# xxxupeng/stereo_toolbox

Hardware: AMD Instinct MI355X
Metric: stereo pairs/sec @ 540x960 D=192 (GwcNet_GC fwd+bwd) (higher is better)
Workload: dtype f32; 1 GPU; GwcNet_GC(maxdisp=192) train step: fwd+bwd+allreduce+Adam, 576x960 pairs (reference pad_to_2x shape), batch 1/GPU, fp32, synthetic randn inputs, deterministic filler weights; global_batch=1, parallelism=dp1, grad_sync=none (single rank: flat fp32 buffer packed, no collective), launch=eager, optimizer=torch.optim.Adam(fused=True)

## Files before the change

include/stx_hip.h:

```cpp
#ifndef STX_HIP_H
#define STX_HIP_H
#ifdef __cplusplus
extern "C" {
#endif

const char* stx_last_error(void);
const char* stx_build_info(void);
int stx_get_tuning(const char* name);
int stx_set_tuning(const char* name, int value);

int stx_cost_volume_fwd(const float* Lg, const float* Rg, int Cg, int G, const float* Lc, const float* Rc, int Cc,
                        const float* scale, float* vol, int B, int H, int W, int D, int mask_left, void* stream);
int stx_group_normalize_fwd(const float* x, float* y, int B, int C, int G, int HW, float out_scale, void* stream);
int stx_group_normalize_bwd(const float* x, const float* gy, float* gx, int B, int C, int G, int HW, float out_scale, void* stream);
int stx_cost_volume_bwd(const float* gvol, const float* Lg, const float* Rg, int Cg, int G, int Cc, float* gLg,
                        float* gRg, float* gLc, float* gRc, int B, int H, int W, int D, int mask_left, void* stream);

int stx_head_fwd(const float* cost, float* disp, float* stats, int B, int Dc, int Hc, int Wc, int D, int H, int W,
                 void* stream);
long long stx_head_bwd_workspace_floats(int B, int Dc, int H, int W);
int stx_head_bwd(const float* gdisp, const float* cost, const float* disp, const float* stats, float* gcost,
                 float* workspace, int B, int Dc, int Hc, int Wc, int D, int H, int W, void* stream);
int stx_head_fwd2(const float* cost, float* disp, float* stats, int B, int Dc, int Hc, int Wc, int D, int H, int W,
                  int align_corners, void* stream);
int stx_head_bwd2(const float* gdisp, const float* cost, const float* disp, const float* stats, float* gcost,
                  float* workspace, int B, int Dc, int Hc, int Wc, int D, int H, int W, int align_corners, void* stream);
int stx_softargmax_fwd(const float* x, float* out, int B, int D, int HW, void* stream);
int stx_argmax_fwd(const float* x, long long* out, int B, int D, int HW, void* stream);
int stx_unimodal_fwd(const float* x, float* out, int B, int D, int HW, void* stream);
int stx_dominant_modal_fwd(const float* x, float* out, int B, int D, int HW, void* stream);
int stx_modal_fwd(const float* x, float* out, float* aux, int B, int D, int HW, int kind, void* stream);
int stx_modal_bwd(const float* g, const float* out, const float* aux, float* gx, int B, int D, int HW, void* stream);
int stx_split_mode(const float* x, float* mode, unsigned char* mask, int B, int D, int HW, void* stream);
int stx_softmax_d_fwd(const float* x, float* y, int B, int D, int HW, void* stream);

long long stx_conv3d_packed_floats(int K, int N, int T);
int stx_conv3d_pack_weight(const float* w, float* wp, int A, int B, int T, int mode, void* stream);
int stx_conv3d_fwd_blocks(int Do, int Ho, int Wo);
long long stx_conv3d_fwd_stat_rows(int B, int Di, int Hi, int Wi, int Cin, int Cout, int ks, int stride);
int stx_conv3d_fwd(const float* x, const float* wp, float* out, const float* scale, const float* bias,
                   const float* residual, float* stats, int B, int Di, int Hi, int Wi, int Cin, int Cout, int ks,
                   int stride, int relu, void* stream);
int stx_deconv3d_fwd_blocks(int Di, int Hi, int Wi);
int stx_deconv3d_fwd(const float* x, const float* wp, float* out, const float* scale, const float* bias,
                     const float* residual, float* stats, int B, int Di, int Hi, int Wi, int Cin, int Cout, int Do,
                     int Ho, int Wo, int relu, void* stream);
long long stx_conv3d_wgrad_workspace_floats(int B, int Dc, int Hc, int Wc, int CF, int CC, int ks, int stride);
int stx_conv3d_wgrad(const float* fine, const float* coarse, float* dw, float* workspace, int B, int Df, int Hf, int Wf,
                     int CF, int Dc, int Hc, int Wc, int CC, int ks, int stride, void* stream);

int stx_conv3d_wgrad_bn_supported(int B, int D, int H, int W, int CF, int CC);
int stx_conv3d_wgrad_bn(const float* x, const float* gy, const float* z, const float* scale, const float* shift, const float* mean,
                        const float* invstd, const float* gamma, const float* sums, float inv_n, int act, float* dz, float* dw,
                        float* workspace, int B, int D, int H, int W, int CF, int CC, void* stream);

int stx_conv3d_axial_supported(int Cin, int Cout, int kd, int kh, int kw);
long long stx_conv3d_axial_packed_floats(int K, int N, int kd, int kh, int kw);
int stx_conv3d_axial_pack_weight(const float* w, float* wp, int A, int B, int kd, int kh, int kw, int mode, void* stream);
long long stx_conv3d_axial_fwd_stat_rows(int B, int D, int H, int W, int Cin, int Cout, int kd, int kh, int kw);
int stx_conv3d_axial_fwd(const float* x, const float* wp, float* out, const float* scale, const float* bias,
                         const float* residual, float* stats, int B, int D, int H, int W, int Cin, int Cout, int kd, int kh,
                         int kw, int act, void* stream);
long long stx_conv3d_axial_wgrad_workspace_floats(int B, int D, int H, int W, int CF, int CC, int kd, int kh, int kw);
int stx_conv3d_axial_wgrad(const float* x, const float* gz, float* dw, float* workspace, int B, int D, int H, int W, int CF,
                           int CC, int kd, int kh, int kw, void* stream);

int stx_convgru_supported(int hidden, int nx, int cx0, int cx1, int cx2, int ksize);
long long stx_convgru_packed_floats(int K, int N);
int stx_convgru_pack_weight(const float* w0, const float* w1, float* wp, int A, int Bd, int mode, void* stream);
int stx_convgru_gemm(const float* s0, int c0, int p0, const float* s1, int c1, int p1, const float* s2, int c2, int p2,
                     const float* s3, int c3, int p3, const float* wp, int N, int epi, int split, const float* bias0,
                     const float* bias1, const float* add0, int add0_pitch, const float* add1, int add1_pitch, const float* h,
                     int h_pitch, const float* z, float* out0, float* out1, float* out2, int out_pitch, int B, int H, int W,
                     void* stream);
int stx_convgru_gate_rows(long long P, int hidden);
int stx_convgru_gate_bwd(const float* g, int g_pitch, const float* z, const float* q, const float* h, int h_pitch, float* gq,
                         float* gz, float* rows, long long P, int hidden, void* stream);
int stx_convgru_reset_bwd(float* buf, int buf_pitch, const float* g, int g_pitch, const float* z, const float* r, const float* h,
                          int h_pitch, float* gr, float* rows, long long P, int hidden, void* stream);
int stx_convgru_row_sum(const float* rows, float* out, int nrows, int n, void* stream);
long long stx_convgru_wgrad_workspace_floats(int B, int H, int W, int K, int CC);
int stx_convgru_wgrad(const float* s0, int c0, int p0, const float* s1, int c1, int p1, const float* s2, int c2, int p2,
                      const float* s3, int c3, int p3, const float* g0, const float* g1, int CG, float* dw, float* workspace,
                      int B, int H, int W, void* stream);

int stx_conv2d_supported(int Cin, int Cout);
long long stx_conv2d_stat_rows(int groups);
int stx_conv2d_fwd(const float* x, const float* w, float* out, float* stats, int B, int H, int W, int Cin, int Cout, int dgrad,
                   int groups, void* stream);

int stx_conv3d_c1_fwd(const float* x, const float* w, const float* residual, float* out, int B, int D, int H, int W,
                      int Cin, void* stream);
long long stx_conv3d_c1_wgrad_workspace_floats(int Cin);
int stx_conv3d_c1_wgrad(const float* x, const float* gy, float* dw, float* workspace, int B, int D, int H, int W,
                        int Cin, void* stream);
int stx_conv3d_c1_dgrad(const float* gy, const float* w, float* gx, int B, int D, int H, int W, int Cin, void* stream);

int stx_mish_fwd(const float* x, float* y, long long n, void* stream);
int stx_mish_bwd(const float* gy, const float* x, float* gx, long long n, void* stream);
int stx_depth_to_space(const float* y, float* out, int B, int D, int H, int W, int C, int inverse, void* stream);
int stx_gate_fwd(const float* cv, const float* att, float* out, int B, int D, long long HW, int C, void* stream);
int stx_gate_bwd(const float* g, const float* cv, const float* att, float* gcv, float* gatt, int B, int D, long long HW,
                 int C, void* stream);

int stx_concat_channels(const float* in0, const float* in1, const float* in2, const float* in3, int C0, int C1, int C2, int C3,
                        float* out, long long nvox, void* stream);
int stx_split_channels(const float* in, float* out0, float* out1, float* out2, float* out3, int C0, int C1, int C2, int C3,
                       long long nvox, void* stream);
int stx_transpose(const float* in, float* out, int N, int rows, int cols, void* stream);

int stx_dwconv_hw_fwd(const float* x, const float* w, const int* dil, float* out, int B, int D, int H, int W, int C,
                      int flip, void* stream);
long long stx_dwconv_hw_wgrad_workspace_floats(int C);
int stx_dwconv_hw_wgrad(const float* x, const float* gy, const int* dil, float* dw, float* workspace, int B, int D,
                        int H, int W, int C, void* stream);
int stx_cost_volume_scale_bwd(const float* gvol, const float* Lc, const float* Rc, float* gscale, int B, int Cc, int H,
                              int W, int D, int mask_left, void* stream);
int stx_scale_channels(const float* x, const float* s, float* out, long long nvox, int C, void* stream);
int stx_ac_volume_bwd(const float* gvol, const float* Lc, const float* Rc, const float* prob, float* gL, float* gR,
                      float* gprob, int B, int Cc, int H, int W, int D, int mask_left, void* stream);

int stx_bn_reduce_blocks(void);
int stx_bn_stats_rows(long long nvox, int C);
int stx_bn_stats(const float* z, float* partials, long long nvox, int C, int groups, void* stream);
int stx_bn_finalize(const float* partials, int nrows, int C, double count, const float* gamma, const float* beta,
                    float* running_mean, float* running_var, float momentum, float eps, float* scale, float* shift,
                    float* mean, float* invstd, void* stream);
int stx_bn_finalize_groups(const float* partials, int nrows, int C, double count, const float* gamma, const float* beta,
                           float* running_mean, float* running_var, float momentum, float eps, float* out, int groups,
                           void* stream);
int stx_bn_apply(const float* z1, const float* scale1, const float* shift1, const float* z2, const float* scale2,
                 const float* shift2, float* out, long long nvox, int C, int relu, int groups, void* stream);
int stx_bn_bwd_reduce(const float* gy, const float* y, const float* z1, const float* mean1, const float* invstd1,
                      const float* z2, const float* mean2, const float* invstd2, float* partials, float* sums,
                      long long nvox, int C, int relu, void* stream);
int stx_bn_bwd_apply(const float* gy, const float* y, const float* z1, const float* mean1, const float* invstd1,
                     const float* gamma1, const float* z2, const float* mean2, const float* invstd2,
                     const float* gamma2, const float* sums, float* dz1, float* dz2, float* gout, long long nvox, int C,
                     int relu, void* stream);
int stx_bn_bwd_reduce2(const float* gy, const float* y, const float* z1, const float* mean1, const float* invstd1,
                       const float* z2, const float* mean2, const float* invstd2, const float* scale1,
                       const float* shift1, const float* scale2, const float* shift2, float* partials, float* sums,
                       long long nvox, int C, int relu, int groups, void* stream);
int stx_bn_bwd_apply2(const float* gy, const float* y, const float* z1, const float* mean1, const float* invstd1,
                      const float* gamma1, const float* z2, const float* mean2, const float* invstd2,
                      const float* gamma2, const float* scale1, const float* shift1, const float* scale2,
                      const float* shift2, const float* sums, float* dz1, float* dz2, float* gout, long long nvox,
                      int C, int relu, int groups, void* stream);

int stx_pad_normalize_u8(const unsigned char* img, float* out, int B, int H, int W, int Hp, int Wp, int top,
                         const float* mean3, const float* std3, void* stream);

int stx_sampled_volume_fwd(const float* Lg, const float* Rg, int Cg, int G, const float* Lc, const float* Rc, int Cc,
                           const float* samples, float* vol, int B, int H, int W, int S, int CTp, void* stream);
int stx_sampled_volume_bwd(const float* gvol, const float* Lg, const float* Rg, int Cg, int G, int Cc,
                           const float* samples, float* gLg, float* gRg, float* gLc, float* gRc, int B, int H, int W,
                           int S, int CTp, void* stream);

int stx_warp_fwd(const float* x, const float* disp, float* out, int B, int C, int H, int W, void* stream);
int stx_warp_bwd(const float* gout, const float* x, const float* disp, float* gx, float* gdisp, int B, int C, int H, int W,
                 void* stream);
int stx_corr_volume_fwd(const float* ref, const float* tgt, float* vol, int B, int C, int H, int W, int maxdisp, int groups,
                        void* stream);
int stx_corr_volume_bwd(const float* gvol, const float* ref, const float* tgt, float* gref, float* gtgt, int B, int C, int H,
                        int W, int maxdisp, int groups, void* stream);
int stx_disparity_variance_fwd(const float* x, const float* disp, const float* samples, float* out, int B, int D, int HW,
                               void* stream);
int stx_disparity_variance_bwd(const float* g, const float* x, const float* disp, const float* samples, float* gx, float* gdisp,
                               float* gsamples, int B, int D, int HW, void* stream);

long long stx_geo_pyramid_floats(long long rows, int len, int C, int levels);
int stx_geo_corr_fwd(const float* fmap1, const float* fmap2, float* cpyr, int B, int C, int H, int W1, int W2, int levels,
                     void* stream);
int stx_geo_corr_bwd(const float* gcpyr, const float* fmap1, const float* fmap2, float* gfmap1, float* gfmap2, int B, int C, int H,
                     int W1, int W2, int levels, void* stream);
int stx_geo_pyramid_fwd(const float* vol, float* gpyr, int B, int D, int H, int W, int C, int levels, void* stream);
int stx_geo_pyramid_bwd(const float* ggpyr, float* gvol, int B, int D, int H, int W, int C, int levels, void* stream);
int stx_geo_lookup_fwd(const float* gpyr, const float* cpyr, const float* disp, const float* coords, float* out, int B, int H,
                       int W, int D, int C, int W2, int levels, int radius, void* stream);
int stx_geo_lookup_bwd(const float* gout, const float* disp, const float* coords, float* ggpyr, float* gcpyr, int B, int H, int W,
                       int D, int C, int W2, int levels, int radius, void* stream);
int stx_context_upsample_fwd(const float* disp_low, const float* up_weights, float* out, int B, int h, int w, void* stream);
int stx_context_upsample_bwd(const float* g, const float* disp_low, const float* up_weights, float* gdisp, float* gweights, int B,
                             int h, int w, void* stream);

long long stx_corr1d_pyramid_floats(long long rows, int W2, int levels);
int stx_corr1d_pyramid_fwd(const float* fmap1, const float* fmap2, float* cpyr, int B, int C, int H, int W1, int W2, int levels,
                           float scale, void* stream);
int stx_corr1d_pyramid_bwd(const float* gcpyr, const float* fmap1, const float* fmap2, float* gfmap1, float* gfmap2, int B, int C,
                           int H, int W1, int W2, int levels, float scale, void* stream);
int stx_corr1d_lookup_fwd(const float* cpyr, const float* base, const float* disp, const float* jobs, int njobs, float* out, int B,
                          int H, int W1, int W2, int levels, void* stream);
int stx_corr1d_lookup_bwd(const float* gout, const float* base, const float* disp, const float* jobs, int njobs, float* gcpyr,
                          int B, int H, int W1, int W2, int levels, void* stream);

int stx_allpairs_estimates_fwd(const float* vol, int which, float* disp_l, float* conf_l, float* disp_r, float* conf_r, float* stats,
                               int B, int H, int W1, int W2, void* stream);
int stx_allpairs_estimates_bwd(const float* g_disp_l, const float* g_conf_l, const float* g_disp_r, const float* g_conf_r,
                               const float* vol, const float* stats, float* gvol, int B, int H, int W1, int W2, void* stream);
int stx_corr1d_volume_pyramid_fwd(const float* vol, const float* tdisp, const float* tconf, float atten, float* cpyr, int B, int H,
                                  int W1, int W2, int levels, void* stream);
int stx_corr1d_volume_pyramid_bwd(const float* gcpyr, const float* tdisp, const float* tconf, float atten, float* gvol, int B, int H,
                                  int W1, int W2, int levels, void* stream);
int stx_truncate_mask_fwd(const float* disp, const float* conf, int has_th, float conf_th, float atten, float* mask, int B, int H,
                          int W, void* stream);

int stx_generate_masks_fwd(const float* mde, void* masks, int B, int N, int H, int W, void* stream);
int stx_masked_volume_fwd(const float* vol, const float* mde_l, const float* mde_r, float* out, int B, int N, int H, int W2, int W3,
                          void* stream);
int stx_masked_volume_bwd(const float* g, const float* mde_l, const float* mde_r, float* gvol, int B, int N, int H, int W2, int W3,
                          void* stream);
int stx_softlrc_fwd(const float* disp2, const float* disp3, float lrc_th, float* out2, float* out3, int B, int H, int W,
                    void* stream);
long long stx_softlrc_bwd_workspace_floats(int B, int H, int W);
int stx_softlrc_bwd(const float* g2, const float* g3, const float* disp2, const float* disp3, float lrc_th, void* workspace,
                    float* gdisp2, float* gdisp3, int B, int H, int W, void* stream);
int stx_weighted_lsq_fwd(const float* mde, const float* disp, const float* conf, float min_quantile, float max_quantile, float* scale,
                         float* shift, void* stats, int B, long long n, void* stream);
int stx_weighted_lsq_bwd(const float* g_scale, const float* g_shift, const float* mde, const float* disp, const float* conf,
                         const void* stats, float* g_mde, float* g_disp, float* g_conf, int B, long long n, void* stream);
int stx_mirror_detector_fwd(const float* stereo_disp, const float* mono_disp, const float* stereo_conf, const float* mono_conf,
                            float conf_th, float step_gain, float* out, long long n, void* stream);
int stx_mirror_detector_bwd(const float* g_out, const float* stereo_disp, const float* mono_disp, const float* stereo_conf,
                            const float* mono_conf, float conf_th, float step_gain, float* g_stereo_disp, float* g_mono_disp,
                            float* g_stereo_conf, float* g_mono_conf, long long n, void* stream);

int stx_photo_warp_fwd(const float* right, const float* disp, float* warped, float* valid, int B, int C, int H, int W, void* stream);
int stx_photo_warp_bwd(const float* gwarped, const float* right, const float* disp, float* gdisp, int B, int C, int H, int W,
                       void* stream);
int stx_ssim_fwd(const float* x, const float* y, float* out, int B, int C, int H, int W, int window, void* stream);
long long stx_ssim_bwd_workspace_floats(int B, int C, int H, int W);
int stx_ssim_bwd(const float* g_out, const float* x, const float* y, float* gx, float* gy, float* workspace, int B, int C, int H, int W,
                 int window, void* stream);
int stx_photometric_fwd(const float* left, const float* right, const float* disp, double ssim_weight, int enable_mask, float* loss,
                        int B, int C, int H, int W, void* stream);
long long stx_photometric_bwd_workspace_floats(int B, int C, int H, int W);
int stx_photometric_bwd(const float* gloss, const float* left, const float* right, const float* disp, double ssim_weight,
                        int enable_mask, float* gdisp, float* workspace, int B, int C, int H, int W, void* stream);
int stx_auto_mask_fwd(const float* left, const float* right, const float* disp, int denorm, unsigned char* mask, int B, int C, int H,
                      int W, void* stream);
long long stx_smoothness_workspace_floats(int B, int H, int W);
int stx_smoothness_fwd(const float* disp, const float* img, float* out, float* stats, float* workspace, int B, int C, int H, int W,
                       void* stream);
int stx_smoothness_bwd(const float* gout, const float* disp, const float* img, const float* stats, float* gdisp, int B, int C, int H,
                       int W, void* stream);

int stx_sttr_head_fwd(const float* attn, const float* phi, int mode, int iters, float log_one, float log_bin, float log_2w,
                      const unsigned char* occ_mask, const float* target, float* disp, float* occ, float* norm, int* arg,
                      float* gt_response, float* bin_left, float* bin_right, double* us, double* vs, int N, int H, int W, void* stream);
int stx_sttr_head_bwd(const float* g_disp, const float* g_occ, const float* g_gt, const float* g_bin_left, const float* g_bin_right,
                      const float* attn, const float* phi, int mode, int iters, float log_one, float log_bin, float log_2w,
                      const float* target, const float* disp, const float* norm, const int* arg, const double* us, const double* vs,
                      float* g_attn, double* phi_partials, float* g_phi, int N, int H, int W, void* stream);
int stx_sttr_transport_fwd(const float* attn, const float* phi, int mode, int iters, float log_one, float log_bin, float log_2w,
                           float* P, double* us, double* vs, int N, int H, int W, void* stream);
int stx_sttr_transport_bwd(const float* G, const float* attn, const float* phi, int mode, int iters, float log_one, float log_bin,
                           float log_2w, const double* us, const double* vs, float* g_attn, double* phi_partials, float* g_phi, int N,
                           int H, int W, void* stream);

int stx_sttr_attn_fwd(const float* q, const float* k, const float* v, const float* Qr, const float* Kr, int causal, float* o,
                      float* raw, float* avg, float* stats, int W, int B, int E, int head_dim, void* stream);
int stx_sttr_attn_bwd(const float* dO, const float* dRaw, const float* q, const float* k, const float* v, const float* Qr,
                      const float* Kr, const float* o, const float* stats, int causal, float* dq, float* dk, float* dv, float* dQr,
                      float* dKr, float* scratch, long long scratch_floats, int nb, int W, int B, int E, int head_dim, void* stream);

int stx_disp_attention_supported(int L, int C, int nhead, int F, int layers);
int stx_disp_attention_fwd(const float* x, const float* pe, const float* const* params, float* y, float* saved, const long long* seed,
                           float p, float eps, int N, int L, int C, int nhead, int F, int layers, int hw, long long sb, long long sp,
                           long long st, void* stream);
long long stx_disp_attention_bwd_workspace_floats(int N, int L, int C, int F);
int stx_disp_attention_bwd(const float* gy, const float* saved, const float* const* params, float* const* gparams, float* gx, float* gbuf,
                           float* workspace, long long workspace_floats, const long long* seed, float p, float eps, int N, int L, int C,
                           int nhead, int F, int layers, int hw, long long sb, long long sp, long long st, void* stream);
int stx_disp_attention_masks(const long long* seed, float p, unsigned char* masks, int N, int L, int C, int F, int layers, void* stream);

int stx_convex_upsample_fwd(const float* flow, const float* mask, float* out, int N, int D, int H, int W, int mask_channels, int f,
                            float scale, void* stream);
long long stx_convex_upsample_bwd_workspace_floats(int N, int D, int H, int W);
int stx_convex_upsample_bwd(const float* g, const float* flow, const float* mask, float* gflow, float* gmask, float* workspace, int N,
                            int D, int H, int W, int mask_channels, int f, float scale, void* stream);
int stx_softmax_context_upsample_fwd(const float* disp_low, const float* logits, float* out, int B, int h, int w, float scale,
                                     void* stream);
int stx_softmax_context_upsample_bwd(const float* g, const float* disp_low, const float* logits, float* gdisp, float* glogits,
                                     float* workspace, int B, int h, int w, float scale, void* stream);
int stx_sequence_loss_max_predictions(void);
long long stx_sequence_loss_workspace_floats(long long n);
int stx_sequence_loss_fwd(const float* const* preds, const double* weights, int K, const float* gt, float maxdisp, float* loss,
                          int* count, float* workspace, long long n, void* stream);
int stx_sequence_loss_bwd(const float* gloss, const float* const* preds, const double* weights, int K, const float* gt, float maxdisp,
                          const int* count, float* const* gpreds, long long n, void* stream);

int stx_monster_flaw_fwd(const float* left, const float* right, const float* disp_a, const float* disp_b, int zeros_pad, float* out_a,
                         float* out_b, float* valid, int B, int C, int H, int W, void* stream);
int stx_monster_flaw_bwd(const float* g_a, const float* g_b, const float* right, const float* disp_a, const float* disp_b, int zeros_pad,
                         float* g_left, float* g_right, float* g_disp_a, float* g_disp_b, int B, int C, int H, int W, void* stream);
int stx_monster_scale_shift(const float* mono, const float* gt, const unsigned char* mask, long long k, float* out, void* stats, int B,
                            long long n, void* stream);
int stx_monster_apply_scale_shift(const float* x, const float* scale_shift, int with_shift, float* out, int B, long long n,
                                  void* stream);

#ifdef __cplusplus
}
#endif
#endif
```

stereo_toolbox_amd/_capi.py:

```python
import ctypes
import os
import threading

import torch

_P = ctypes.c_void_p
_I = ctypes.c_int
_F = ctypes.c_float
_L = ctypes.c_longlong

SIGNATURES = {
    "stx_get_tuning": [ctypes.c_char_p],
    "stx_set_tuning": [ctypes.c_char_p, _I],
    "stx_cost_volume_fwd": [_P, _P, _I, _I, _P, _P, _I, _P, _P, _I, _I, _I, _I, _I, _P],
    "stx_cost_volume_bwd": [_P, _P, _P, _I, _I, _I, _P, _P, _P, _P, _I, _I, _I, _I, _I, _P],
    "stx_group_normalize_fwd": [_P, _P, _I, _I, _I, _I, _F, _P],
    "stx_group_normalize_bwd": [_P, _P, _P, _I, _I, _I, _I, _F, _P],
    "stx_head_fwd": [_P, _P, _P, _I, _I, _I, _I, _I, _I, _I, _P],
    "stx_head_bwd_workspace_floats": [_I, _I, _I, _I],
    "stx_head_bwd": [_P, _P, _P, _P, _P, _P, _I, _I, _I, _I, _I, _I, _I, _P],
    "stx_head_fwd2": [_P, _P, _P, _I, _I, _I, _I, _I, _I, _I, _I, _P],
    "stx_head_bwd2": [_P, _P, _P, _P, _P, _P, _I, _I, _I, _I, _I, _I, _I, _I, _P],
    "stx_softargmax_fwd": [_P, _P, _I, _I, _I, _P],
    "stx_argmax_fwd": [_P, _P, _I, _I, _I, _P],
    "stx_softmax_d_fwd": [_P, _P, _I, _I, _I, _P],
    "stx_unimodal_fwd": [_P, _P, _I, _I, _I, _P],
    "stx_dominant_modal_fwd": [_P, _P, _I, _I, _I, _P],
    "stx_modal_fwd": [_P, _P, _P, _I, _I, _I, _I, _P],
    "stx_modal_bwd": [_P, _P, _P, _P, _I, _I, _I, _P],
    "stx_split_mode": [_P, _P, _P, _I, _I, _I, _P],
    "stx_conv3d_packed_floats": [_I, _I, _I],
    "stx_conv3d_pack_weight": [_P, _P, _I, _I, _I, _I, _P],
    "stx_conv3d_fwd_blocks": [_I, _I, _I],
    "stx_conv3d_fwd_stat_rows": [_I, _I, _I, _I, _I, _I, _I, _I],
    "stx_deconv3d_fwd_blocks": [_I, _I, _I],
    "stx_conv3d_fwd": [_P, _P, _P, _P, _P, _P, _P, _I, _I, _I, _I, _I, _I, _I, _I, _I, _P],
    "stx_deconv3d_fwd": [_P, _P, _P, _P, _P, _P, _P, _I, _I, _I, _I, _I, _I, _I, _I, _I, _I, _P],
    "stx_conv3d_wgrad_workspace_floats": [_I, _I, _I, _I, _I, _I, _I, _I],
    "stx_conv3d_wgrad": [_P, _P, _P, _P, _I, _I, _I, _I, _I, _I, _I, _I, _I, _I, _I, _P],
    "stx_conv3d_wgrad_bn_supported": [_I, _I, _I, _I, _I, _I],
    "stx_conv3d_wgrad_bn": [_P] * 9 + [_F, _I, _P, _P, _P, _I, _I, _I, _I, _I, _I, _P],
    "stx_conv3d_axial_supported": [_I, _I, _I, _I, _I],
    "stx_conv3d_axial_packed_floats": [_I, _I, _I, _I, _I],
    "stx_conv3d_axial_pack_weight": [_P, _P, _I, _I, _I, _I, _I, _I, _P],
    "stx_conv3d_axial_fwd_stat_rows": [_I] * 9,
    "stx_conv3d_axial_fwd": [_P] * 7 + [_I] * 10 + [_P],
    "stx_conv3d_axial_wgrad_workspace_floats": [_I] * 9,
    "stx_conv3d_axial_wgrad": [_P, _P, _P, _P] + [_I] * 9 + [_P],
    "stx_convgru_supported": [_I] * 6,
    "stx_convgru_packed_floats": [_I, _I],
    "stx_convgru_pack_weight": [_P, _P, _P, _I, _I, _I, _P],
    "stx_convgru_gemm": [_P, _I, _I] * 4 + [_P, _I, _I, _I, _P, _P, _P, _I, _P, _I, _P, _I, _P, _P, _P, _P, _I, _I, _I, _I, _P],
    "stx_convgru_gate_rows": [_L, _I],
    "stx_convgru_gate_bwd": [_P, _I, _P, _P, _P, _I, _P, _P, _P, _L, _I, _P],
    "stx_convgru_reset_bwd": [_P, _I, _P, _I, _P, _P, _P, _I, _P, _P, _L, _I, _P],
    "stx_convgru_row_sum": [_P, _P, _I, _I, _P],
    "stx_convgru_wgrad_workspace_floats": [_I] * 5,
    "stx_convgru_wgrad": [_P, _I, _I] * 4 + [_P, _P, _I, _P, _P, _I, _I, _I, _P],
    "stx_conv2d_supported": [_I, _I],
    "stx_conv2d_stat_rows": [_I],
    "stx_conv2d_fwd": [_P, _P, _P, _P, _I, _I, _I, _I, _I, _I, _I, _P],
    "stx_conv3d_c1_fwd": [_P, _P, _P, _P, _I, _I, _I, _I, _I, _P],
    "stx_conv3d_c1_wgrad_workspace_floats": [_I],
    "stx_conv3d_c1_wgrad": [_P, _P, _P, _P, _I, _I, _I, _I, _I, _P],
    "stx_conv3d_c1_dgrad": [_P, _P, _P, _I, _I, _I, _I, _I, _P],
    "stx_mish_fwd": [_P, _P, _L, _P],
    "stx_mish_bwd": [_P, _P, _P, _L, _P],
    "stx_depth_to_space": [_P, _P, _I, _I, _I, _I, _I, _I, _P],
    "stx_gate_fwd": [_P, _P, _P, _I, _I, _L, _I, _P],
    "stx_gate_bwd": [_P, _P, _P, _P, _P, _I, _I, _L, _I, _P],
    "stx_concat_channels": [_P, _P, _P, _P, _I, _I, _I, _I, _P, _L, _P],
    "stx_split_channels": [_P, _P, _P, _P, _P, _I, _I, _I, _I, _L, _P],
    "stx_transpose": [_P, _P, _I, _I, _I, _P],
    "stx_dwconv_hw_fwd": [_P, _P, _P, _P, _I, _I, _I, _I, _I, _I, _P],
    "stx_dwconv_hw_wgrad_workspace_floats": [_I],
    "stx_dwconv_hw_wgrad": [_P, _P, _P, _P, _P, _I, _I, _I, _I, _I, _P],
    "stx_cost_volume_scale_bwd": [_P, _P, _P, _P, _I, _I, _I, _I, _I, _I, _P],
    "stx_scale_channels": [_P, _P, _P, _L, _I, _P],
    "stx_ac_volume_bwd": [_P, _P, _P, _P, _P, _P, _P, _I, _I, _I, _I, _I, _I, _P],
    "stx_pad_normalize_u8": [_P, _P, _I, _I, _I, _I, _I, _I, _P, _P, _P],
    "stx_warp_fwd": [_P, _P, _P, _I, _I, _I, _I, _P],
    "stx_warp_bwd": [_P, _P, _P, _P, _P, _I, _I, _I, _I, _P],
    "stx_corr_volume_fwd": [_P, _P, _P, _I, _I, _I, _I, _I, _I, _P],
    "stx_corr_volume_bwd": [_P, _P, _P, _P, _P, _I, _I, _I, _I, _I, _I, _P],
    "stx_disparity_variance_fwd": [_P, _P, _P, _P, _I, _I, _I, _P],
    "stx_disparity_variance_bwd": [_P, _P, _P, _P, _P, _P, _P, _I, _I, _I, _P],
    "stx_sampled_volume_fwd": [_P, _P, _I, _I, _P, _P, _I, _P, _P, _I, _I, _I, _I, _I, _P],
    "stx_sampled_volume_bwd": [_P, _P, _P, _I, _I, _I, _P, _P, _P, _P, _P, _I, _I, _I, _I, _I, _P],
    "stx_geo_pyramid_floats": [_L, _I, _I, _I],
    "stx_geo_corr_fwd": [_P, _P, _P, _I, _I, _I, _I, _I, _I, _P],
    "stx_geo_corr_bwd": [_P, _P, _P, _P, _P, _I, _I, _I, _I, _I, _I, _P],
    "stx_geo_pyramid_fwd": [_P, _P, _I, _I, _I, _I, _I, _I, _P],
    "stx_geo_pyramid_bwd": [_P, _P, _I, _I, _I, _I, _I, _I, _P],
    "stx_geo_lookup_fwd": [_P, _P, _P, _P, _P, _I, _I, _I, _I, _I, _I, _I, _I, _P],
    "stx_geo_lookup_bwd": [_P, _P, _P, _P, _P, _I, _I, _I, _I, _I, _I, _I, _I, _P],
    "stx_context_upsample_fwd": [_P, _P, _P, _I, _I, _I, _P],
    "stx_context_upsample_bwd": [_P, _P, _P, _P, _P, _I, _I, _I, _P],
    "stx_corr1d_pyramid_floats": [_L, _I, _I],
    "stx_corr1d_pyramid_fwd": [_P, _P, _P, _I, _I, _I, _I, _I, _I, _F, _P],
    "stx_corr1d_pyramid_bwd": [_P, _P, _P, _P, _P, _I, _I, _I, _I, _I, _I, _F, _P],
    "stx_corr1d_lookup_fwd": [_P, _P, _P, _P, _I, _P, _I, _I, _I, _I, _I, _P],
    "stx_corr1d_lookup_bwd": [_P, _P, _P, _P, _I, _P, _I, _I, _I, _I, _I, _P],
    "stx_allpairs_estimates_fwd": [_P, _I, _P, _P, _P, _P, _P, _I, _I, _I, _I, _P],
    "stx_allpairs_estimates_bwd": [_P, _P, _P, _P, _P, _P, _P, _I, _I, _I, _I, _P],
    "stx_corr1d_volume_pyramid_fwd": [_P, _P, _P, _F, _P, _I, _I, _I, _I, _I, _P],
    "stx_corr1d_volume_pyramid_bwd": [_P, _P, _P, _F, _P, _I, _I, _I, _I, _I, _P],
    "stx_truncate_mask_fwd": [_P, _P, _I, _F, _F, _P, _I, _I, _I, _P],
    "stx_generate_masks_fwd": [_P, _P, _I, _I, _I, _I, _P],
    "stx_masked_volume_fwd": [_P, _P, _P, _P, _I, _I, _I, _I, _I, _P],
    "stx_masked_volume_bwd": [_P, _P, _P, _P, _I, _I, _I, _I, _I, _P],
    "stx_softlrc_fwd": [_P, _P, _F, _P, _P, _I, _I, _I, _P],
    "stx_softlrc_bwd_workspace_floats": [_I, _I, _I],
    "stx_softlrc_bwd": [_P, _P, _P, _P, _F, _P, _P, _P, _I, _I, _I, _P],
    "stx_weighted_lsq_fwd": [_P, _P, _P, _F, _F, _P, _P, _P, _I, _L, _P],
    "stx_weighted_lsq_bwd": [_P, _P, _P, _P, _P, _P, _P, _P, _P, _I, _L, _P],
    "stx_mirror_detector_fwd": [_P, _P, _P, _P, _F, _F, _P, _L, _P],
    "stx_mirror_detector_bwd": [_P, _P, _P, _P, _P, _F, _F, _P, _P, _P, _P, _L, _P],
    "stx_photo_warp_fwd": [_P, _P, _P, _P, _I, _I, _I, _I, _P],
    "stx_photo_warp_bwd": [_P, _P, _P, _P, _I, _I, _I, _I, _P],
    "stx_ssim_fwd": [_P, _P, _P, _I, _I, _I, _I, _I, _P],
    "stx_ssim_bwd_workspace_floats": [_I, _I, _I, _I],
    "stx_ssim_bwd": [_P, _P, _P, _P, _P, _P, _I, _I, _I, _I, _I, _P],
    "stx_photometric_fwd": [_P, _P, _P, ctypes.c_double, _I, _P, _I, _I, _I, _I, _P],
    "stx_photometric_bwd_workspace_floats": [_I, _I, _I, _I],
    "stx_photometric_bwd": [_P, _P, _P, _P, ctypes.c_double, _I, _P, _P, _I, _I, _I, _I, _P],
    "stx_auto_mask_fwd": [_P, _P, _P, _I, _P, _I, _I, _I, _I, _P],
    "stx_smoothness_workspace_floats": [_I, _I, _I],
    "stx_smoothness_fwd": [_P, _P, _P, _P, _P, _I, _I, _I, _I, _P],
    "stx_smoothness_bwd": [_P, _P, _P, _P, _P, _I, _I, _I, _I, _P],
    "stx_sttr_head_fwd": [_P, _P, _I, _I, _F, _F, _F] + [_P] * 11 + [_I, _I, _I, _P],
    "stx_sttr_head_bwd": [_P] * 7 + [_I, _I, _F, _F, _F] + [_P] * 9 + [_I, _I, _I, _P],
    "stx_sttr_transport_fwd": [_P, _P, _I, _I, _F, _F, _F, _P, _P, _P, _I, _I, _I, _P],
    "stx_sttr_transport_bwd": [_P, _P, _P, _I, _I, _F, _F, _F, _P, _P, _P, _P, _P, _I, _I, _I, _P],
    "stx_sttr_attn_fwd": [_P] * 5 + [_I] + [_P] * 4 + [_I, _I, _I, _I, _P],
    "stx_sttr_attn_bwd": [_P] * 9 + [_I] + [_P] * 6 + [_L, _I, _I, _I, _I, _I, _P],
    "stx_disp_attention_supported": [_I] * 5,
    "stx_disp_attention_fwd": [_P] * 6 + [_F, _F] + [_I] * 7 + [_L, _L, _L, _P],
    "stx_disp_attention_bwd_workspace_floats": [_I] * 4,
    "stx_disp_attention_bwd": [_P] * 7 + [_L, _P, _F, _F] + [_I] * 7 + [_L, _L, _L, _P],
    "stx_disp_attention_masks": [_P, _F, _P, _I, _I, _I, _I, _I, _P],
    "stx_convex_upsample_fwd": [_P, _P, _P, _I, _I, _I, _I, _I, _I, _F, _P],
    "stx_convex_upsample_bwd_workspace_floats": [_I, _I, _I, _I],
    "stx_convex_upsample_bwd": [_P, _P, _P, _P, _P, _P, _I, _I, _I, _I, _I, _I, _F, _P],
    "stx_softmax_context_upsample_fwd": [_P, _P, _P, _I, _I, _I, _F, _P],
    "stx_softmax_context_upsample_bwd": [_P, _P, _P, _P, _P, _P, _I, _I, _I, _F, _P],
    "stx_sequence_loss_max_predictions": [],
    "stx_sequence_loss_workspace_floats": [_L],
    "stx_sequence_loss_fwd": [_P, _P, _I, _P, _F, _P, _P, _P, _L, _P],
    "stx_sequence_loss_bwd": [_P, _P, _P, _I, _P, _F, _P, _P, _L, _P],
    "stx_monster_flaw_fwd": [_P, _P, _P, _P, _I, _P, _P, _P, _I, _I, _I, _I, _P],
    "stx_monster_flaw_bwd": [_P, _P, _P, _P, _P, _I, _P, _P, _P, _P, _I, _I, _I, _I, _P],
    "stx_monster_scale_shift": [_P, _P, _P, _L, _P, _P, _I, _L, _P],
    "stx_monster_apply_scale_shift": [_P, _P, _I, _P, _I, _L, _P],
    "stx_bn_reduce_blocks": [],
    "stx_bn_stats_rows": [_L, _I],
    "stx_bn_stats": [_P, _P, _L, _I, _I, _P],
    "stx_bn_finalize": [_P, _I, _I, ctypes.c_double, _P, _P, _P, _P, _F, _F, _P, _P, _P, _P, _P],
    "stx_bn_finalize_groups": [_P, _I, _I, ctypes.c_double, _P, _P, _P, _P, _F, _F, _P, _I, _P],
    "stx_bn_apply": [_P, _P, _P, _P, _P, _P, _P, _L, _I, _I, _I, _P],
    "stx_bn_bwd_reduce": [_P, _P, _P, _P, _P, _P, _P, _P, _P, _P, _L, _I, _I, _P],
    "stx_bn_bwd_apply": [_P, _P, _P, _P, _P, _P, _P, _P, _P, _P, _P, _P, _P, _P, _L, _I, _I, _P],
    "stx_bn_bwd_reduce2": [_P] * 14 + [_L, _I, _I, _I, _P],
    "stx_bn_bwd_apply2": [_P] * 18 + [_L, _I, _I, _I, _P],
}
_RET_CHARP = ("stx_last_error", "stx_build_info")


class StxError(RuntimeError):
    pass


class StxLib:

    def __init__(self, path):
        if not os.path.exists(path):
            raise StxError(
                f"HIP library not found: {path}. Build it with `python -m stereo_toolbox_amd.build` "
                "(hipcc, gfx950). There is no CPU fallback for the cost-volume hot path.")
        self.path = path
        self._dll = ctypes.CDLL(path)
        for name in _RET_CHARP:
            fn = getattr(self._dll, name)
            fn.restype = ctypes.c_char_p
            fn.argtypes = []
        self._fns = {}
        for name, argtypes in SIGNATURES.items():
            fn = getattr(self._dll, name, None)
            if fn is None:
                continue
            fn.restype = ctypes.c_longlong if name.endswith(("_floats", "_stat_rows")) else _I
            fn.argtypes = argtypes
            self._fns[name] = fn

    def has(self, name):
        return name in self._fns

    def build_info(self):
        return self._dll.stx_build_info().decode()

    def get_tuning(self, name):
        return self._fns["stx_get_tuning"](name.encode())

    def set_tuning(self, name, value):
        old = self.get_tuning(name)
        if old < 0 or self._fns["stx_set_tuning"](name.encode(), int(value)) != 0:
            raise StxError(f"unknown tuning switch {name}")
        return old

    def raw(self, name):
        return self._fns[name]

    def call(self, name, *args):
        fn = self._fns.get(name)
        if fn is None:
            raise StxError(f"{self.path} does not export {name}")
        rc = fn(*args)
        if rc != 0:
            raise StxError(f"{name} failed ({rc}): {self._dll.stx_last_error().decode()}")


_LIB = None
_LOCK = threading.Lock()
LIB_PATH = os.environ.get("STX_HIP_LIB") or os.path.join(os.path.dirname(os.path.abspath(__file__)), "lib", "libstx_hip.so")


def get_lib():
    global _LIB
    if _LIB is None:
        with _LOCK:
            if _LIB is None:
                _LIB = StxLib(LIB_PATH)
    return _LIB
```

stereo_toolbox_amd/aggregation.py:

```python
import os
import threading

import torch
import torch.nn as nn

from . import ops


def _is_transposed(conv):
    return isinstance(conv, nn.ConvTranspose3d)


def _conv_cfg(conv):
    ks = conv.kernel_size[0]
    stride = conv.stride[0]
    if _is_transposed(conv):
        k3 = ks == 3 and stride == 2 and conv.padding[0] == 1 and conv.output_padding[0] == 1
        k4 = ks == 4 and stride == 2 and conv.padding[0] == 1 and conv.output_padding[0] == 0
        if not (k3 or k4) or len(set(conv.kernel_size)) != 1 or len(set(conv.stride)) != 1:
            raise ops.StxError("only ConvTranspose3d(k=3, s=2, p=1, op=1) and ConvTranspose3d(k=4, s=2, p=1) are on the hot path")
    else:
        if not ((ks == 3 and conv.padding[0] == 1 and stride in (1, 2)) or (ks == 1 and conv.padding[0] == 0 and stride == 1)):
            raise ops.StxError(f"unsupported Conv3d k={ks} s={stride} p={conv.padding}")
    if conv.bias is not None or conv.groups != 1:
        raise ops.StxError("hot-path convolutions are bias-free and dense")
    return ks, stride


def _fold(bn):
    key = (bn.weight._version, bn.bias._version, bn.running_mean._version, bn.running_var._version,
           bn.weight.data_ptr(), bn.bias.data_ptr(), bn.running_mean.data_ptr(), bn.running_var.data_ptr())
    hit = bn.__dict__.get("_stx_fold") if ops._CACHE_ENABLED else None
    if hit is not None and hit[0] == key:
        return hit[1], hit[2]
    with torch.no_grad():
        scale = (bn.weight * torch.rsqrt(bn.running_var + bn.eps)).contiguous()
        bias = (bn.bias - bn.running_mean * scale).contiguous()
    if ops._CACHE_ENABLED:
        bn.__dict__["_stx_fold"] = (key, scale, bias)
    return scale, bias


def _needs_grad(*tensors_and_modules):
    if not torch.is_grad_enabled():
        return False
    for t in tensors_and_modules:
        if t is None:
            continue
        if isinstance(t, torch.Tensor):
            if t.requires_grad:
                return True
        else:
            if any(p.requires_grad for p in t.parameters()):
                return True
    return False


def _infer_conv(x, conv, scale, bias, residual, relu):
    ks, stride = _conv_cfg(conv)
    if _is_transposed(conv) and ks == 4:
        if residual is not None:
            raise ops.StxError("ConvTranspose3d(k4) with a fused residual is not wired (no model uses it)")
        return ops.deconv4_forward(x, conv.weight.detach(), scale, bias, int(relu), owner=conv.weight)
    if _is_transposed(conv):
        wp = ops.pack_weight(conv.weight.detach(), 2, owner=conv.weight)
        return ops.deconv3d_forward(x, wp, conv.weight.shape[1], scale=scale, bias=bias, residual=residual, relu=relu)[0]
    if ops._is_c1(conv.weight, ks, stride, False) and scale is None and bias is None and not relu:
        return ops.conv3d_c1_forward(x, conv.weight.detach().contiguous(), residual)
    if x.shape[-1] != conv.weight.shape[1]:
        if x.shape[-1] != (conv.weight.shape[1] + 7) // 8 * 8:
            raise ops.StxError(f"conv: input has {x.shape[-1]} channels, weight expects {conv.weight.shape[1]}")
        wpad = ops.pad_weight_channels(conv.weight.detach(), x.shape[-1])
        return ops.conv3d_forward(x, ops.pack_weight(wpad, 0), conv.weight.shape[0], ks, stride, scale, bias, residual, relu)[0]
    if x.shape[-1] % 8 != 0:
        xp, wpad = ops.pad_input_channels(x, conv.weight.detach())
        return ops.conv3d_forward(xp, ops.pack_weight(wpad, 0), conv.weight.shape[0], ks, stride, scale, bias, residual, relu)[0]
    wp = ops.pack_weight(conv.weight.detach(), 0, owner=conv.weight)
    return ops.conv3d_forward(x, wp, conv.weight.shape[0], ks, stride, scale, bias, residual, relu)[0]


class deferred_bn_counters:
    _tls = threading.local()

    @staticmethod
    def _state():
        st = deferred_bn_counters._tls
        if not hasattr(st, "active"):
            st.active, st.pending = 0, []
        return st

    def __enter__(self):
        self._state().active += 1
        ops.bn_defer_reset_if_stale()
        return self

    def __exit__(self, *exc):
        st = self._state()
        st.active -= 1
        if st.active == 0 and st.pending:
            pend, st.pending = st.pending, []
            by_dev = {}
            for t in pend:
                d = by_dev.setdefault(t.device, {})
                ent = d.setdefault(id(t), [t, 0])
                ent[1] += 1
            for d in by_dev.values():
                torch._foreach_add_([e[0] for e in d.values()], [e[1] for e in d.values()])
        return False


def _bn_state(bn, partials, count, steps=1):
    training = bn.training
    sync = None
    if training and isinstance(bn, nn.SyncBatchNorm):
        import torch.distributed as dist
        if dist.is_available() and dist.is_initialized() and dist.get_world_size(bn.process_group) > 1:
            sync = (bn.process_group, dist.get_world_size(bn.process_group))
    if training:
        bn.__dict__.pop("_stx_fold", None)
    if training and bn.track_running_stats and bn.num_batches_tracked is not None:
        st = deferred_bn_counters._state()
        if st.active and bn.momentum is not None:
            st.pending.extend([bn.num_batches_tracked] * steps)
        else:
            bn.num_batches_tracked.add_(steps)
    if bn.momentum is not None:
        momentum = bn.momentum
    elif training and bn.track_running_stats and bn.num_batches_tracked is not None:
        momentum = 1.0 / float(bn.num_batches_tracked.item())
    else:
        momentum = 0.0
    return {"training": training, "partials": partials, "count": count, "running_mean": bn.running_mean,
            "running_var": bn.running_var, "momentum": momentum, "eps": bn.eps, "sync": sync}


def _raw_conv(x, conv, want):
    ks, stride = _conv_cfg(conv)
    if _is_transposed(conv) and ks == 4:
        return ops.deconv4_raw(x, conv.weight, want)
    return ops.ConvRawFn.apply(x, conv.weight, ks, stride, _is_transposed(conv), want)


@ops.fp32_region
def shared_input_convs(x, blocks):
    cfgs, ws = [], []
    for seq in blocks:
        conv, bn = seq[0], seq[1]
        if _is_transposed(conv) or not bn.training or conv.weight.shape[1] != x.shape[-1] or conv.weight.shape[1] % 8 \
                or conv.weight.shape[0] % 8:
            return None
        ks, stride = _conv_cfg(conv)
        cfgs.append((ks, stride, True))
        ws.append(conv.weight)
    if not _needs_grad(x, *[m for seq in blocks for m in (seq[0], seq[1])]):
        return None
    outs = ops.SharedInputConvsFn.apply(x, tuple(cfgs), *ws)
    return [(outs[2 * k], outs[2 * k + 1]) for k in range(len(blocks))]


@ops.fp32_region
def conv_block(x, conv, bn=None, relu=False, second=None, residual=None, mish=False, leaky=False, raw=None, second_raw=None):
    if (mish and relu) or (leaky and (relu or mish)):
        raise ops.StxError("conv_block: relu, mish and leaky are mutually exclusive")
    if second is not None and residual is not None:
        raise ops.StxError("conv_block: `second` and `residual` are mutually exclusive")
    mods = [conv, bn] + ([second[1], second[2]] if second is not None else [])
    grad = (raw is not None or second_raw is not None
            or _needs_grad(x, residual, *(m for m in mods if m is not None), *([second[0]] if second else [])))
    train_bn = (bn is not None and bn.training) or (second is not None and second[2].training)
    if mish and (grad or train_bn) and (bn is None or residual is not None):
        return ops.mish(conv_block(x, conv, bn, relu=False, second=second, residual=residual))
    if mish:
        relu = 2
    if leaky:
        relu = 3

    if not grad and not train_bn:
        if second is not None:
            s2, b2 = _fold(second[2])
            residual = _infer_conv(second[0], second[1], s2, b2, None, False)
        if bn is not None:
            s1, b1 = _fold(bn)
        else:
            s1 = b1 = None
        return _infer_conv(x, conv, s1, b1, residual, relu)

    want = bn is not None and bn.training
    z1, part1 = raw if raw is not None else _raw_conv(x, conv, want)
    if bn is None:
        y = z1
        if residual is not None:
            y = y + residual
        if relu == 3:
            return torch.nn.functional.leaky_relu(y, 0.01)
        return torch.relu(y) if relu else y
    count1 = z1.numel() // z1.shape[-1]
    st1 = _bn_state(bn, part1 if want else None, count1)
    if second is not None:
        x2, conv2, bn2 = second
        want2 = bn2.training
        z2, part2 = second_raw if second_raw is not None else _raw_conv(x2, conv2, want2)
        st2 = _bn_state(bn2, part2 if want2 else None, z2.numel() // z2.shape[-1])
        return ops.BnActFn.apply(z1, bn.weight, bn.bias, z2, bn2.weight, bn2.bias, None, relu, st1, st2)
    defer = (residual is None and want and relu in (0, 1, False, True) and not _is_transposed(conv) and _conv_cfg(conv) == (3, 1)
             and conv.weight.shape[0] % 32 == 0 and conv.weight.shape[1] % 32 == 0 and not st1.get("sync")
             and os.environ.get("STX_BN_BWD_IN_WGRAD", "1") != "0")
    if defer:
        ops.bn_defer_reset_if_stale()
    return ops.BnActFn.apply(z1, bn.weight, bn.bias, None, None, None, residual, relu, st1, None, 1, defer)


def _axial_cfg(conv):
    if not isinstance(conv, nn.Conv3d) or _is_transposed(conv):
        raise ops.StxError("axial_conv_block: expected an nn.Conv3d")
    kernel = ops._axial_kernel(conv.weight, "axial_conv_block")
    if tuple(conv.stride) != (1, 1, 1) or tuple(conv.dilation) != (1, 1, 1) or conv.groups != 1:
        raise ops.StxError(f"axial_conv_block: stride {tuple(conv.stride)} dilation {tuple(conv.dilation)} groups {conv.groups}: "
                           "only dense stride-1 convolutions are served")
    if tuple(conv.padding) != tuple(k // 2 for k in kernel) or conv.padding_mode != "zeros":
        raise ops.StxError(f"axial_conv_block: padding {conv.padding} ({conv.padding_mode}) is not the 'same' zero padding of kernel {kernel}")
    return kernel


def _fold_with_bias(conv, bn):
    scale, shift = _fold(bn)
    if conv.bias is None:
        return scale, shift
    hit = conv.__dict__.get("_stx_fold") if ops._CACHE_ENABLED else None
    key = (conv.bias._version, conv.bias.data_ptr())
    if hit is not None and hit[0] == key and hit[1] is shift:
        return scale, hit[2]
    with torch.no_grad():
        shift_b = torch.addcmul(shift, conv.bias, scale).contiguous()
    if ops._CACHE_ENABLED:
        conv.__dict__["_stx_fold"] = (key, shift, shift_b)
    return scale, shift_b


@ops.fp32_region
def axial_conv_block(x, conv, bn):
    kernel = _axial_cfg(conv)
    if not isinstance(bn, nn.modules.batchnorm._BatchNorm):
        raise ops.StxError(f"axial_conv_block: {type(bn).__name__} is not a BatchNorm")
    if not _needs_grad(x, conv, bn) and not bn.training:
        scale, shift = _fold_with_bias(conv, bn)
        xk, wk, _ = ops._axial_prepare(x, conv.weight.detach(), "axial_conv_block")
        wp = ops.pack_weight_axial(wk, 0, owner=conv.weight if wk.shape == conv.weight.shape else None)
        return ops.conv3d_axial_forward(xk, wp, conv.weight.shape[0], kernel, scale, shift, None, 1)[0]
    want = bn.training
    z, part = ops.AxialConvRawFn.apply(x, conv.weight, want)
    if conv.bias is not None:
        z = ops.ZeroGradBiasFn.apply(z, conv.bias) if want else z + conv.bias
    st = _bn_state(bn, part if want else None, z.numel() // z.shape[-1])
    y = ops.BnActFn.apply(z, bn.weight, bn.bias, None, None, None, None, 1, st, None)
    if want and conv.bias is not None and bn.track_running_stats and bn.running_mean is not None:
        with torch.no_grad():
            bn.running_mean.add_(conv.bias.detach(), alpha=float(st["momentum"]))
    return y


@ops.fp32_region
def convbn_block(x, seq, relu=False, second=None, residual=None, mish=False, raw=None, second_raw=None):
    sec = None
    if second is not None:
        sec = (second[0], second[1][0], second[1][1])
    return conv_block(x, seq[0], seq[1], relu=relu, second=sec, residual=residual, mish=mish, raw=raw, second_raw=second_raw)
```

stereo_toolbox_amd/csrc/conv_c1.hip:

```cpp
#include "stx_common.h"
#include <stdlib.h>

namespace {

constexpr int C1_THREADS = 256;
constexpr int C1_TD = 2, C1_TH = 4, C1_TW = 32;
constexpr int C1_ED = C1_TD + 2, C1_EH = C1_TH + 2, C1_EW = C1_TW + 2;
constexpr int C1_CK = 16, C1_VS = C1_CK + 4;

struct C1Args {
    const float* x;
    const float* w;
    const float* gy;
    const float* res;
    float* out;
    int B, D, H, W, Cin;
    int nDt, nHt, nWt, ntiles;
};

__device__ __forceinline__ void c1_stage(const C1Args& a, float* tile, int b, int d0, int h0, int w0, int c0, int tid) {
    for (int idx = tid; idx < C1_ED * C1_EH * C1_EW * (C1_CK / 4); idx += C1_THREADS) {
        const int v = idx / (C1_CK / 4), f = idx - v * (C1_CK / 4);
        const int wx = v % C1_EW, hy = (v / C1_EW) % C1_EH, dz = v / (C1_EW * C1_EH);
        const int gd = d0 - 1 + dz, gh = h0 - 1 + hy, gw = w0 - 1 + wx;
        float4 val = make_float4(0.f, 0.f, 0.f, 0.f);
        if (gd >= 0 && gd < a.D && gh >= 0 && gh < a.H && gw >= 0 && gw < a.W)
            val = stx_ld4(a.x + ((((size_t)b * a.D + gd) * a.H + gh) * a.W + gw) * a.Cin + c0 + 4 * f);
        stx_st4(tile + v * C1_VS + 4 * f, val);
    }
}

__global__ __launch_bounds__(C1_THREADS) void conv_c1_fwd_kernel(C1Args a) {
    STX_DYN_SMEM(smem);
    float* tile = reinterpret_cast<float*>(smem);
    const int tid = threadIdx.x;
    int r = blockIdx.x;
    const int wt = r % a.nWt; r /= a.nWt;
    const int ht = r % a.nHt; r /= a.nHt;
    const int dt = r % a.nDt;
    const int b = r / a.nDt;
    const int d0 = dt * C1_TD, h0 = ht * C1_TH, w0 = wt * C1_TW;
    const int lw = tid % C1_TW, lh = (tid / C1_TW) % C1_TH, ld = tid / (C1_TW * C1_TH);
    const int base = ((ld * C1_EH + lh) * C1_EW + lw) * C1_VS;
    float acc = 0.f;
    for (int c0 = 0; c0 < a.Cin; c0 += C1_CK) {
        __syncthreads();
        c1_stage(a, tile, b, d0, h0, w0, c0, tid);
        __syncthreads();
        for (int tap = 0; tap < 27; ++tap) {
            const int kd = tap / 9, kh = (tap / 3) % 3, kw = tap % 3;
            const float* p = tile + base + ((kd * C1_EH + kh) * C1_EW + kw) * C1_VS;
#pragma unroll
            for (int f = 0; f < C1_CK / 4; ++f) {
                const float4 v = stx_ld4(p + 4 * f);
                const float* wp = a.w + (size_t)(c0 + 4 * f) * 27 + tap;
                acc = fmaf(v.x, wp[0], acc);
                acc = fmaf(v.y, wp[27], acc);
                acc = fmaf(v.z, wp[54], acc);
                acc = fmaf(v.w, wp[81], acc);
            }
        }
    }
    const int od = d0 + ld, oh = h0 + lh, ow = w0 + lw;
    if (od < a.D && oh < a.H && ow < a.W) {
        const size_t o = (((size_t)b * a.D + od) * a.H + oh) * a.W + ow;
        a.out[o] = a.res ? acc + a.res[o] : acc;
    }
}

__global__ __launch_bounds__(C1_THREADS) void conv_c1_wgrad_kernel(C1Args a) {
    STX_DYN_SMEM(smem);
    float* tile = reinterpret_cast<float*>(smem);
    float* gys = tile + C1_ED * C1_EH * C1_EW * C1_VS;
    const int tid = threadIdx.x;
    const int cl = tid & 15, tg = tid >> 4;
    const int nchunk = a.Cin / C1_CK;
    float acc[4][2];
#pragma unroll
    for (int i = 0; i < 4; ++i) { acc[i][0] = 0.f; acc[i][1] = 0.f; }
    const int tapA = tg, tapB = tg + 16;
    const int offA = (((tapA / 9) * C1_EH + (tapA / 3) % 3) * C1_EW + tapA % 3) * C1_VS + cl;
    const int tB = tapB < 27 ? tapB : 0;
    const int offB = (((tB / 9) * C1_EH + (tB / 3) % 3) * C1_EW + tB % 3) * C1_VS + cl;

    for (int t = blockIdx.x; t < a.ntiles; t += gridDim.x) {
        int r = t;
        const int wt = r % a.nWt; r /= a.nWt;
        const int ht = r % a.nHt; r /= a.nHt;
        const int dt = r % a.nDt;
        const int b = r / a.nDt;
        const int d0 = dt * C1_TD, h0 = ht * C1_TH, w0 = wt * C1_TW;
#pragma unroll
        for (int ck = 0; ck < 4; ++ck) {
            if (ck < nchunk) {
                __syncthreads();
                c1_stage(a, tile, b, d0, h0, w0, ck * C1_CK, tid);
                if (ck == 0) {
                    const int lw = tid % C1_TW, lh = (tid / C1_TW) % C1_TH, ld = tid / (C1_TW * C1_TH);
                    const int od = d0 + ld, oh = h0 + lh, ow = w0 + lw;
                    gys[tid] = (od < a.D && oh < a.H && ow < a.W)
                                   ? a.gy[(((size_t)b * a.D + od) * a.H + oh) * a.W + ow] : 0.f;
                }
                __syncthreads();
                float sA = 0.f, sB = 0.f;
                for (int v = 0; v < C1_TD * C1_TH * C1_TW; ++v) {
                    const int lw = v % C1_TW, lh = (v / C1_TW) % C1_TH, ld = v / (C1_TW * C1_TH);
                    const int vb = ((ld * C1_EH + lh) * C1_EW + lw) * C1_VS;
                    const float g = gys[v];
                    sA = fmaf(tile[vb + offA], g, sA);
                    sB = fmaf(tile[vb + offB], g, sB);
                }
                acc[ck][0] += sA;
                acc[ck][1] += sB;
            }
        }
    }
    float* dst = a.out + (size_t)blockIdx.x * a.Cin * 27;
#pragma unroll
    for (int ck = 0; ck < 4; ++ck) {
        if (ck < nchunk) {
            dst[(ck * C1_CK + cl) * 27 + tapA] = acc[ck][0];
            if (tapB < 27) dst[(ck * C1_CK + cl) * 27 + tapB] = acc[ck][1];
        }
    }
}

__global__ __launch_bounds__(C1_THREADS) void c1_colsum_kernel(const float* __restrict__ partials, int nrows, int M,
                                                               float* __restrict__ sums) {
    __shared__ double red[C1_THREADS];
    const int m = blockIdx.x, tid = threadIdx.x;
    double s = 0.0;
    for (int r = tid; r < nrows; r += C1_THREADS) s += (double)partials[(size_t)r * M + m];
    red[tid] = s;
    __syncthreads();
    for (int k = C1_THREADS / 2; k > 0; k >>= 1) {
        if (tid < k) red[tid] += red[tid + k];
        __syncthreads();
    }
    if (tid == 0) sums[m] = (float)red[0];
}

constexpr size_t C1_TILE_BYTES = (size_t)C1_ED * C1_EH * C1_EW * C1_VS * 4;
constexpr int C1_WGRAD_BLOCKS = 512;


constexpr int C1D_TH = 4, C1D_TW = 32;
constexpr int C1D_EH = C1D_TH + 2, C1D_EW = C1D_TW + 2;

__global__ __launch_bounds__(C1_THREADS) void conv_c1_dgrad_kernel(const float* __restrict__ gy,
                                                                   const float* __restrict__ w, float* __restrict__ gx,
                                                                   int B, int D, int H, int W, int Cin, int nHt, int nWt) {
    __shared__ float gys[3 * C1D_EH * C1D_EW];
    __shared__ float ws[27 * 64];
    const int tid = threadIdx.x;
    int r = blockIdx.x;
    const int wt = r % nWt; r /= nWt;
    const int ht = r % nHt; r /= nHt;
    const int d = r % D;
    const int b = r / D;
    const int h0 = ht * C1D_TH, w0 = wt * C1D_TW;
    for (int idx = tid; idx < 3 * C1D_EH * C1D_EW; idx += C1_THREADS) {
        const int wx = idx % C1D_EW, hy = (idx / C1D_EW) % C1D_EH, dz = idx / (C1D_EW * C1D_EH);
        const int gd = d - 1 + dz, gh = h0 - 1 + hy, gw = w0 - 1 + wx;
        gys[idx] = (gd >= 0 && gd < D && gh >= 0 && gh < H && gw >= 0 && gw < W)
                       ? gy[(((size_t)b * D + gd) * H + gh) * W + gw] : 0.f;
    }
    for (int idx = tid; idx < 27 * Cin; idx += C1_THREADS) {
        const int c = idx % Cin, tap = idx / Cin;
        ws[tap * Cin + c] = w[(size_t)c * 27 + tap];
    }
    __syncthreads();
    const int CQ = Cin >> 2;
    for (int item = tid; item < CQ * (C1D_TH * C1D_TW / 4); item += C1_THREADS) {
        const int q = item % CQ, grp = item / CQ;
        const int lw = (grp % (C1D_TW / 4)) * 4, lh = grp / (C1D_TW / 4);
        float4 acc[4];
#pragma unroll
        for (int j = 0; j < 4; ++j) acc[j] = make_float4(0.f, 0.f, 0.f, 0.f);
#pragma unroll
        for (int kd = 0; kd < 3; ++kd)
#pragma unroll
            for (int kh = 0; kh < 3; ++kh) {
                const float* gp = gys + (((2 - kd) * C1D_EH) + (lh + 2 - kh)) * C1D_EW + lw;
                float g6[6];
#pragma unroll
                for (int j = 0; j < 6; ++j) g6[j] = gp[j];
#pragma unroll
                for (int kw = 0; kw < 3; ++kw) {
                    const float4 wv = stx_ld4(ws + ((kd * 3 + kh) * 3 + kw) * Cin + 4 * q);
#pragma unroll
                    for (int j = 0; j < 4; ++j) {
                        const float g = g6[j + 2 - kw];
                        acc[j].x = fmaf(g, wv.x, acc[j].x);
                        acc[j].y = fmaf(g, wv.y, acc[j].y);
                        acc[j].z = fmaf(g, wv.z, acc[j].z);
                        acc[j].w = fmaf(g, wv.w, acc[j].w);
                    }
                }
            }
        const int oh = h0 + lh;
        if (oh < H) {
            float* o = gx + ((((size_t)b * D + d) * H + oh) * W + w0 + lw) * Cin + 4 * q;
#pragma unroll
            for (int j = 0; j < 4; ++j)
                if (w0 + lw + j < W) stx_st4(o + (size_t)j * Cin, acc[j]);
        }
    }
}


__global__ __launch_bounds__(C1_THREADS) void conv_c1_dgrad_mfma_kernel(const float* __restrict__ gy,
                                                                        const float* __restrict__ w, float* __restrict__ gx,
                                                                        int B, int D, int H, int W, int nHt, int nWt, int ntiles) {
    __shared__ float gys[3 * C1D_EH * C1D_EW];
    const int tid = threadIdx.x, lane = tid & 63, wave = tid >> 6;
    const int i = lane & 31, half = lane >> 5;
    float wreg[14];
    int aoff[14];
#pragma unroll
    for (int j = 0; j < 14; ++j) {
        const int tap = 2 * j + half;
        const int tp = tap < 27 ? tap : 26;
        const int kd = tp / 9, kh = (tp / 3) % 3, kw = tp % 3;
        wreg[j] = tap < 27 ? w[(size_t)i * 27 + tap] : 0.f;
        aoff[j] = ((2 - kd) * C1D_EH + (wave + 2 - kh)) * C1D_EW + i + 2 - kw;
    }
    const unsigned plane_bytes = (unsigned)H * (unsigned)W * 128u;
    for (int tile = blockIdx.x; tile < ntiles; tile += gridDim.x) {
        int r_ = tile;
        const int wt = r_ % nWt; r_ /= nWt;
        const int ht = r_ % nHt; r_ /= nHt;
        const int d = r_ % D;
        const int b = r_ / D;
        const int h0 = ht * C1D_TH, w0 = wt * C1D_TW;
        __syncthreads();
        for (int idx = tid; idx < 3 * C1D_EH * C1D_EW; idx += C1_THREADS) {
            const int wx = idx % C1D_EW, hy = (idx / C1D_EW) % C1D_EH, dz = idx / (C1D_EW * C1D_EH);
            const int gd = d - 1 + dz, gh = h0 - 1 + hy, gw = w0 - 1 + wx;
            gys[idx] = (gd >= 0 && gd < D && gh >= 0 && gh < H && gw >= 0 && gw < W)
                           ? gy[(((size_t)b * D + gd) * H + gh) * W + gw] : 0.f;
        }
        __syncthreads();
        f32x16 acc;
#pragma unroll
        for (int r = 0; r < 16; ++r) acc[r] = 0.f;
        float av[14];
#pragma unroll
        for (int j = 0; j < 14; ++j) av[j] = gys[aoff[j]];
#pragma unroll
        for (int j = 0; j < 14; ++j) acc = __builtin_amdgcn_mfma_f32_32x32x2f32(av[j], wreg[j], acc, 0, 0, 0);
        const int oh = h0 + wave;
        const stx_bufrsrc ors = stx_make_rsrc(gx + ((size_t)b * D + d) * H * W * 32, plane_bytes);
        const unsigned vbase = (unsigned)((((oh < H ? oh : 0) * W + w0 + 4 * half) * 32 + i) * 4);
#pragma unroll
        for (int r = 0; r < 16; ++r) {
            const int m = (r & 3) + 8 * (r >> 2);
            const bool ok = oh < H && w0 + 4 * half + m < W;
            stx_buf_st1(ors, ok ? vbase : STX_BUF_OOB, (unsigned)(m * 128), acc[r]);
        }
    }
}


constexpr int C1M_TD = 2, C1M_TH = 8, C1M_TW = 32;
constexpr int C1M_ED = C1M_TD + 2, C1M_EH = C1M_TH + 2, C1M_EW = C1M_TW + 2;
constexpr int C1M_BLOCKS = 1024;

__global__ __launch_bounds__(C1_THREADS) void conv_c1_wgrad_mfma_kernel(const float* __restrict__ x,
                                                                        const float* __restrict__ gy,
                                                                        float* __restrict__ slab, int B, int D, int H,
                                                                        int W, int Cin, int nDt, int nHt, int nWt,
                                                                        int ntiles) {
    __shared__ float gys[C1M_ED * C1M_EH * C1M_EW];
    __shared__ float red[4][1024];
    const int tid = threadIdx.x, lane = tid & 63, wave = tid >> 6;
    const int i = lane & 31, half = lane >> 5;
    const int cb = blockIdx.y;
    const int kd = i / 9, kh = (i / 3) % 3, kw = i % 3;
    const int toff = (i < 27) ? ((2 - kd) * C1M_EH + (2 - kh)) * C1M_EW + (2 - kw) + half : half;
    f32x16 acc;
#pragma unroll
    for (int r = 0; r < 16; ++r) acc[r] = 0.f;
    for (int t = blockIdx.x; t < ntiles; t += gridDim.x) {
        int r = t;
        const int wt = r % nWt; r /= nWt;
        const int ht = r % nHt; r /= nHt;
        const int dt = r % nDt;
        const int b = r / nDt;
        const int d0 = dt * C1M_TD, h0 = ht * C1M_TH, w0 = wt * C1M_TW;
        __syncthreads();
        for (int idx = tid; idx < C1M_ED * C1M_EH * C1M_EW; idx += C1_THREADS) {
            const int wx = idx % C1M_EW, hy = (idx / C1M_EW) % C1M_EH, dz = idx / (C1M_EW * C1M_EH);
            const int gd = d0 - 1 + dz, gh = h0 - 1 + hy, gw = w0 - 1 + wx;
            gys[idx] = (gd >= 0 && gd < D && gh >= 0 && gh < H && gw >= 0 && gw < W)
                           ? gy[(((size_t)b * D + gd) * H + gh) * W + gw] : 0.f;
        }
        __syncthreads();
#pragma unroll 1
        for (int k = 0; k < 4; ++k) {
            const int row = wave * 4 + k;
            const int ld = row / C1M_TH, lh = row % C1M_TH;
            const int gd = d0 + ld, gh = h0 + lh;
            const bool rowok = gd < D && gh < H;
            const float* xr = x + ((((size_t)b * D + gd) * H + gh) * W + w0 + half) * Cin + cb * 32 + i;
            float av[16];
#pragma unroll
            for (int p = 0; p < 16; ++p)
                av[p] = (rowok && w0 + 2 * p + half < W) ? xr[(size_t)(2 * p) * Cin] : 0.f;
            const float* gp = gys + (ld * C1M_EH + lh) * C1M_EW + toff;
#pragma unroll
            for (int p = 0; p < 16; ++p) {
                float bv = gp[2 * p];
                bv = (i < 27) ? bv : 0.f;
                acc = __builtin_amdgcn_mfma_f32_32x32x2f32(av[p], bv, acc, 0, 0, 0);
            }
        }
    }
#pragma unroll
    for (int r = 0; r < 16; ++r) red[wave][((r & 3) + 8 * (r >> 2) + 4 * half) * 32 + i] = acc[r];
    __syncthreads();
    float* dst = slab + ((size_t)cb * gridDim.x + blockIdx.x) * 1024;
    for (int idx = tid; idx < 1024; idx += C1_THREADS)
        dst[idx] = (red[0][idx] + red[1][idx]) + (red[2][idx] + red[3][idx]);
}

__global__ __launch_bounds__(C1_THREADS) void c1m_reduce_kernel(const float* __restrict__ slab, int nrows,
                                                                float* __restrict__ dw) {
    __shared__ double red[C1_THREADS];
    const int m = blockIdx.x, tid = threadIdx.x;
    const int tap = m % 27, cfull = m / 27, cb = cfull >> 5, c = cfull & 31;
    const float* p = slab + (size_t)cb * nrows * 1024 + c * 32 + tap;
    double s = 0.0;
    for (int r = tid; r < nrows; r += C1_THREADS) s += (double)p[(size_t)r * 1024];
    red[tid] = s;
    __syncthreads();
    for (int k = C1_THREADS / 2; k > 0; k >>= 1) {
        if (tid < k) red[tid] += red[tid + k];
        __syncthreads();
    }
    if (tid == 0) dw[m] = (float)red[0];
}


constexpr int C1F_TH = 8, C1F_TW = 32;
constexpr int C1F_EH = C1F_TH + 2, C1F_EW = C1F_TW + 2, C1F_NV = C1F_EH * C1F_EW;
constexpr int C1F_MT = (C1F_NV + 31) / 32;
constexpr int C1F_WGS = 512;

__global__ __launch_bounds__(C1_THREADS) void conv_c1_fwd_mfma_kernel(const float* __restrict__ x,
                                                                      const float* __restrict__ w,
                                                                      const float* __restrict__ res,
                                                                      float* __restrict__ out, int B, int D, int H, int W,
                                                                      int nHt, int nWt, int ncols) {
    STX_DYN_SMEM(smem);
    float* Ps = reinterpret_cast<float*>(smem);
    const int tid = threadIdx.x, lane = tid & 63, wave = __builtin_amdgcn_readfirstlane(tid >> 6);
    const int i = lane & 31, half = lane >> 5;
    float wreg[16];
#pragma unroll
    for (int s_ = 0; s_ < 16; ++s_) wreg[s_] = (i < 27) ? w[(size_t)(16 * half + s_) * 27 + i] : 0.f;
    const int lh = tid / C1F_TW, lw = tid % C1F_TW;

    constexpr int MTW = (C1F_MT + 3) / 4;
    const long long units = (long long)ncols * D;
    int u = __builtin_amdgcn_readfirstlane((int)(units * blockIdx.x / gridDim.x));
    const int u_end = __builtin_amdgcn_readfirstlane((int)(units * (blockIdx.x + 1) / gridDim.x));
    const unsigned plane_bytes = (unsigned)H * (unsigned)W * 32u * 4u;
    while (u < u_end) {
        const int col = u / D;
        const int d_lo = u - col * D;
        const int left = u_end - u;
        const int d_hi = (D - d_lo < left) ? D : d_lo + left;
        u += d_hi - d_lo;
        const int wt = col % nWt, ht = (col / nWt) % nHt, b = col / (nWt * nHt);
        const int h0 = ht * C1F_TH, w0 = wt * C1F_TW;
        const int oh = h0 + lh, ow = w0 + lw;
        const bool ook = oh < H && ow < W;
        unsigned voff[MTW];
#pragma unroll
        for (int t = 0; t < MTW; ++t) {
            const int hv = (wave + 4 * t) * 32 + i;
            const int hy = hv / C1F_EW, wx = hv - hy * C1F_EW;
            const int gh = h0 - 1 + hy, gw = w0 - 1 + wx;
            const bool ok = wave + 4 * t < C1F_MT && hv < C1F_NV && gh >= 0 && gh < H && gw >= 0 && gw < W;
            voff[t] = ok ? (unsigned)(((gh * W + gw) * 32 + 16 * half) * 4) : STX_BUF_OOB;
        }
        float4 nxt[MTW][4];
        auto load_plane = [&](int p) {
            const bool in = p >= 0 && p < D && p <= d_hi;
            const stx_bufrsrc rs = stx_make_rsrc(x + ((size_t)b * D + (in ? p : 0)) * H * W * 32, in ? plane_bytes : 0u);
#pragma unroll
            for (int t = 0; t < MTW; ++t)
#pragma unroll
                for (int q = 0; q < 4; ++q) nxt[t][q] = stx_buf_ld4(rs, voff[t], 16u * q);
        };
        float accA = 0.f, accB = 0.f;
        load_plane(d_lo - 1);
        __syncthreads();
        for (int p = d_lo - 1; p <= d_hi; ++p) {
            float* Pb = Ps + ((p + 2) & 1) * (C1F_NV * 27);
            const bool pin = p >= 0 && p < D;
            float4 cur[MTW][4];
#pragma unroll
            for (int t = 0; t < MTW; ++t)
#pragma unroll
                for (int q = 0; q < 4; ++q) cur[t][q] = nxt[t][q];
            load_plane(p + 1);
            if (pin) {
#pragma unroll
                for (int t = 0; t < MTW; ++t) {
                    const int m = wave + 4 * t;
                    if (m < C1F_MT) {
                        f32x16 acc;
#pragma unroll
                        for (int r = 0; r < 16; ++r) acc[r] = 0.f;
#pragma unroll
                        for (int q = 0; q < 4; ++q) {
                            acc = __builtin_amdgcn_mfma_f32_32x32x2f32(cur[t][q].x, wreg[4 * q + 0], acc, 0, 0, 0);
                            acc = __builtin_amdgcn_mfma_f32_32x32x2f32(cur[t][q].y, wreg[4 * q + 1], acc, 0, 0, 0);
                            acc = __builtin_amdgcn_mfma_f32_32x32x2f32(cur[t][q].z, wreg[4 * q + 2], acc, 0, 0, 0);
                            acc = __builtin_amdgcn_mfma_f32_32x32x2f32(cur[t][q].w, wreg[4 * q + 3], acc, 0, 0, 0);
                        }
                        if (i < 27) {
#pragma unroll
                            for (int r = 0; r < 16; ++r) {
                                const int v = m * 32 + (r & 3) + 8 * (r >> 2) + 4 * half;
                                if (v < C1F_NV) Pb[v * 27 + i] = acc[r];
                            }
                        }
                    }
                }
            }
            __syncthreads();
            float s0 = 0.f, s1 = 0.f, s2 = 0.f;
            if (pin) {
#pragma unroll
                for (int kh = 0; kh < 3; ++kh)
#pragma unroll
                    for (int kw = 0; kw < 3; ++kw) {
                        const float* pp = Pb + ((lh + kh) * C1F_EW + lw + kw) * 27 + kh * 3 + kw;
                        s0 += pp[0];
                        s1 += pp[9];
                        s2 += pp[18];
                    }
            }
            const float done = accA + s2;
            const int od = p - 1;
            if (od >= d_lo && od < d_hi && ook) {
                const size_t o = (((size_t)b * D + od) * H + oh) * W + ow;
                out[o] = res ? done + res[o] : done;
            }
            accA = accB + s1;
            accB = s0;
        }
    }
}

}

extern "C" int stx_conv3d_c1_fwd(const float* x, const float* w, const float* residual, float* out, int B, int D,
                                 int H, int W, int Cin, void* stream) {
    stx_begin();
    STX_REQUIRE(x && w && out && B > 0 && D > 0 && H > 0 && W > 0, "conv3d_c1_fwd: bad shape");
    STX_REQUIRE(Cin % C1_CK == 0, "conv3d_c1_fwd: Cin=%d must be a multiple of %d", Cin, C1_CK);
    if (Cin == 32 && (long long)H * W * 128 < (1ll << 31)) {
        const int nHt = stx_cdiv(H, C1F_TH), nWt = stx_cdiv(W, C1F_TW);
        const long long ncols = (long long)B * nHt * nWt, units = ncols * D;
        STX_REQUIRE(units < (1ll << 31), "conv3d_c1_fwd: volume too large");
        long long g = C1F_WGS;
        if (g > units / 4) g = units / 4 > 0 ? units / 4 : 1;
        const size_t lds = (size_t)2 * C1F_NV * 27 * 4;
        if (int rc = stx_lds_require((const void*)conv_c1_fwd_mfma_kernel, lds, "conv3d_c1_fwd(mfma)")) return rc;
        hipLaunchKernelGGL(conv_c1_fwd_mfma_kernel, dim3((unsigned)g), dim3(C1_THREADS), lds, (hipStream_t)stream, x, w,
                           residual, out, B, D, H, W, nHt, nWt, (int)ncols);
        return stx_check_launch("conv3d_c1_fwd(mfma)");
    }
    C1Args a;
    a.x = x; a.w = w; a.gy = nullptr; a.res = residual; a.out = out;
    a.B = B; a.D = D; a.H = H; a.W = W; a.Cin = Cin;
    a.nDt = stx_cdiv(D, C1_TD); a.nHt = stx_cdiv(H, C1_TH); a.nWt = stx_cdiv(W, C1_TW);
    a.ntiles = B * a.nDt * a.nHt * a.nWt;
    if (int rc = stx_lds_require((const void*)conv_c1_fwd_kernel, C1_TILE_BYTES, "conv3d_c1_fwd")) return rc;
    hipLaunchKernelGGL(conv_c1_fwd_kernel, dim3(a.ntiles), dim3(C1_THREADS), C1_TILE_BYTES, (hipStream_t)stream, a);
    return stx_check_launch("conv3d_c1_fwd");
}

extern "C" long long stx_conv3d_c1_wgrad_workspace_floats(int Cin) {
    const long long valu = (long long)C1_WGRAD_BLOCKS * Cin * 27;
    const long long mfma = (long long)C1M_BLOCKS * 1024 * ((Cin + 31) / 32);
    return valu > mfma ? valu : mfma;
}

extern "C" int stx_conv3d_c1_wgrad(const float* x, const float* gy, float* dw, float* workspace, int B, int D, int H,
                                   int W, int Cin, void* stream) {
    stx_begin();
    STX_REQUIRE(x && gy && dw && workspace && B > 0, "conv3d_c1_wgrad: null operand");
    STX_REQUIRE(Cin % C1_CK == 0 && Cin <= 4 * C1_CK, "conv3d_c1_wgrad: Cin=%d must be 16..64 in steps of 16", Cin);
    if (Cin % 32 == 0) {
        const int nDt = stx_cdiv(D, C1M_TD), nHt = stx_cdiv(H, C1M_TH), nWt = stx_cdiv(W, C1M_TW);
        const long long nt = (long long)B * nDt * nHt * nWt;
        STX_REQUIRE(nt < (1ll << 31), "conv3d_c1_wgrad: volume too large");
        const int nblk = nt < C1M_BLOCKS ? (int)nt : C1M_BLOCKS;
        hipStream_t st = (hipStream_t)stream;
        hipLaunchKernelGGL(conv_c1_wgrad_mfma_kernel, dim3(nblk, Cin / 32), dim3(C1_THREADS), 0, st, x, gy, workspace, B,
                           D, H, W, Cin, nDt, nHt, nWt, (int)nt);
        int rc = stx_check_launch("conv3d_c1_wgrad(mfma)");
        if (rc) return rc;
        hipLaunchKernelGGL(c1m_reduce_kernel, dim3(Cin * 27), dim3(C1_THREADS), 0, st, workspace, nblk, dw);
        return stx_check_launch("conv3d_c1_wgrad(reduce)");
    }
    C1Args a;
    a.x = x; a.w = nullptr; a.gy = gy; a.res = nullptr; a.out = workspace;
    a.B = B; a.D = D; a.H = H; a.W = W; a.Cin = Cin;
    a.nDt = stx_cdiv(D, C1_TD); a.nHt = stx_cdiv(H, C1_TH); a.nWt = stx_cdiv(W, C1_TW);
    a.ntiles = B * a.nDt * a.nHt * a.nWt;
    const int nblk = a.ntiles < C1_WGRAD_BLOCKS ? a.ntiles : C1_WGRAD_BLOCKS;
    const size_t lds = C1_TILE_BYTES + 256 * 4;
    hipStream_t st = (hipStream_t)stream;
    if (int rc = stx_lds_require((const void*)conv_c1_wgrad_kernel, lds, "conv3d_c1_wgrad")) return rc;
    hipLaunchKernelGGL(conv_c1_wgrad_kernel, dim3(nblk), dim3(C1_THREADS), lds, st, a);
    if (int rc = stx_check_launch("conv3d_c1_wgrad")) return rc;
    hipLaunchKernelGGL(c1_colsum_kernel, dim3(Cin * 27), dim3(C1_THREADS), 0, st, workspace, nblk, Cin * 27, dw);
    return stx_check_launch("conv3d_c1_colsum");
}

extern "C" int stx_conv3d_c1_dgrad(const float* gy, const float* w, float* gx, int B, int D, int H, int W, int Cin,
                                   void* stream) {
    stx_begin();
    STX_REQUIRE(gy && w && gx && B > 0 && D > 0 && H > 0 && W > 0, "conv3d_c1_dgrad: bad shape");
    STX_REQUIRE(Cin % 4 == 0 && Cin <= 64, "conv3d_c1_dgrad: Cin=%d must be a multiple of 4, <= 64", Cin);
    const int nHt = stx_cdiv(H, C1D_TH), nWt = stx_cdiv(W, C1D_TW);
    const long long nt = (long long)B * D * nHt * nWt;
    if (Cin == 32 && (long long)H * W * 128 < (1ll << 31) && nt < (1ll << 31)) {
        const long long g = nt < 256 * 8 ? nt : 256 * 8;
        hipLaunchKernelGGL(conv_c1_dgrad_mfma_kernel, dim3((unsigned)g), dim3(C1_THREADS), 0, (hipStream_t)stream, gy, w, gx, B, D,
                           H, W, nHt, nWt, (int)nt);
        return stx_check_launch("conv3d_c1_dgrad(mfma)");
    }
    hipLaunchKernelGGL(conv_c1_dgrad_kernel, dim3((unsigned)((size_t)B * D * nHt * nWt)), dim3(C1_THREADS), 0,
                       (hipStream_t)stream, gy, w, gx, B, D, H, W, Cin, nHt, nWt);
    return stx_check_launch("conv3d_c1_dgrad");
}
```

stereo_toolbox_amd/models/GwcNet/gwcnet.py:

```python
import torch
import torch.nn as nn

from ... import ops
from ...aggregation import conv_block, convbn_block, deferred_bn_counters, shared_input_convs
from ..features2d import ResTrunk, cat_features, channels_last_weights_, convbn, init_reference_style, run_head2d, run_pair
from .submodule import convbn_3d


class feature_extraction(ResTrunk):
    fused_everywhere = True

    def __init__(self, concat_feature=False, concat_feature_channel=12):
        super().__init__()
        self.concat_feature = concat_feature
        if concat_feature:
            self.lastconv = nn.Sequential(convbn(320, 128, 3, 1, 1, 1), nn.ReLU(inplace=True),
                                          nn.Conv2d(128, concat_feature_channel, 1, bias=False))

    def forward(self, x):
        gwc = cat_features(self.trunk(x))
        if not self.concat_feature:
            return {"gwc_feature": gwc}
        return {"gwc_feature": gwc, "concat_feature": run_head2d(self.lastconv, gwc)}


class hourglass(nn.Module):

    def __init__(self, c):
        super().__init__()
        self.conv1 = nn.Sequential(convbn_3d(c, c * 2, 3, 2, 1), nn.ReLU(inplace=True))
        self.conv2 = nn.Sequential(convbn_3d(c * 2, c * 2, 3, 1, 1), nn.ReLU(inplace=True))
        self.conv3 = nn.Sequential(convbn_3d(c * 2, c * 4, 3, 2, 1), nn.ReLU(inplace=True))
        self.conv4 = nn.Sequential(convbn_3d(c * 4, c * 4, 3, 1, 1), nn.ReLU(inplace=True))
        self.conv5 = nn.Sequential(nn.ConvTranspose3d(c * 4, c * 2, 3, padding=1, output_padding=1, stride=2, bias=False),
                                   nn.BatchNorm3d(c * 2))
        self.conv6 = nn.Sequential(nn.ConvTranspose3d(c * 2, c, 3, padding=1, output_padding=1, stride=2, bias=False),
                                   nn.BatchNorm3d(c))
        self.redir1 = convbn_3d(c, c, kernel_size=1, stride=1, pad=0)
        self.redir2 = convbn_3d(c * 2, c * 2, kernel_size=1, stride=1, pad=0)

    def forward(self, x, mid=None, also=None):
        rx = shared_input_convs(x, [self.conv1[0], self.redir1] + ([also] if also is not None else []))
        rx = rx or [None, None, None]
        c1 = convbn_block(x, self.conv1[0], relu=True, raw=rx[0])
        c2 = convbn_block(c1, self.conv2[0], relu=True)
        r2 = shared_input_convs(c2, [self.conv3[0], self.redir2]) or [None, None]
        c3 = convbn_block(c2, self.conv3[0], relu=True, raw=r2[0])
        c4 = convbn_block(c3, self.conv4[0], relu=True)
        if mid is not None:
            c4 = mid(c4)
        c5 = convbn_block(c4, self.conv5, relu=True, second=(c2, self.redir2), second_raw=r2[1])
        out = convbn_block(c5, self.conv6, relu=True, second=(x, self.redir1), second_raw=rx[1])
        return (out, rx[2]) if also is not None else out


def classifier(c):
    return nn.Sequential(convbn_3d(c, c, 3, 1, 1), nn.ReLU(inplace=True),
                         nn.Conv3d(c, 1, kernel_size=3, padding=1, stride=1, bias=False))


def run_classifier(seq, x, add=None, raw=None):
    h = convbn_block(x, seq[0], relu=True, raw=raw)
    cost = conv_block(h, seq[2], residual=None if add is None else add.unsqueeze(-1))
    return cost.squeeze(-1)


class GwcNet(nn.Module):
    def __init__(self, maxdisp, use_concat_volume=False):
        super().__init__()
        self.maxdisp = maxdisp
        self.use_concat_volume = use_concat_volume
        self.num_groups = 40
        if use_concat_volume:
            self.concat_channels = 12
            self.feature_extraction = feature_extraction(True, self.concat_channels)
        else:
            self.concat_channels = 0
            self.feature_extraction = feature_extraction(False)
        self.dres0 = nn.Sequential(convbn_3d(self.num_groups + self.concat_channels * 2, 32, 3, 1, 1),
                                   nn.ReLU(inplace=True), convbn_3d(32, 32, 3, 1, 1), nn.ReLU(inplace=True))
        self.dres1 = nn.Sequential(convbn_3d(32, 32, 3, 1, 1), nn.ReLU(inplace=True), convbn_3d(32, 32, 3, 1, 1))
        self.dres2 = hourglass(32)
        self.dres3 = hourglass(32)
        self.dres4 = hourglass(32)
        self.classif0 = classifier(32)
        self.classif1 = classifier(32)
        self.classif2 = classifier(32)
        self.classif3 = classifier(32)
        init_reference_style(self)
        channels_last_weights_(self.feature_extraction)

    def forward(self, left, right):
        with deferred_bn_counters():
            fl, fr = run_pair(self.feature_extraction, left, right, self.training)
            return self.aggregate(fl, fr, left.shape[2], left.shape[3])

    @ops.fp32_region
    def aggregate(self, fl, fr, H, W):
        vol = ops.cost_volume(fl["gwc_feature"], fr["gwc_feature"], fl.get("concat_feature"),
                              fr.get("concat_feature"), self.maxdisp // 4, self.num_groups, mask_left=True)
        cost0 = convbn_block(vol, self.dres0[0], relu=True)
        cost0 = convbn_block(cost0, self.dres0[2], relu=True)
        t = convbn_block(cost0, self.dres1[0], relu=True)
        cost0 = convbn_block(t, self.dres1[2], relu=False, residual=cost0)
        if self.training:
            out1, r0 = self.dres2(cost0, also=self.classif0[0])
            out2, r1 = self.dres3(out1, also=self.classif1[0])
            out3, r2 = self.dres4(out2, also=self.classif2[0])
            return [ops.regression_head(run_classifier(c, o, raw=r), self.maxdisp, H, W)
                    for c, o, r in ((self.classif0, cost0, r0), (self.classif1, out1, r1), (self.classif2, out2, r2),
                                    (self.classif3, out3, None))]
        out1 = self.dres2(cost0)
        out2 = self.dres3(out1)
        out3 = self.dres4(out2)
        return ops.regression_head(run_classifier(self.classif3, out3), self.maxdisp, H, W)


def GwcNet_G(d=192):
    return GwcNet(d, use_concat_volume=False)


def GwcNet_GC(d=192):
    return GwcNet(d, use_concat_volume=True)
```

stereo_toolbox_amd/models/PSMNet/stackhourglass.py:

```python
import torch.nn as nn

from ... import ops
from ...aggregation import conv_block, convbn_block, deferred_bn_counters
from ..features2d import channels_last_weights_, init_reference_style, run_pair
from .submodule import convbn_3d, feature_extraction


class hourglass(nn.Module):

    def __init__(self, inplanes):
        super().__init__()
        c = inplanes
        self.conv1 = nn.Sequential(convbn_3d(c, c * 2, kernel_size=3, stride=2, pad=1), nn.ReLU(inplace=True))
        self.conv2 = convbn_3d(c * 2, c * 2, kernel_size=3, stride=1, pad=1)
        self.conv3 = nn.Sequential(convbn_3d(c * 2, c * 2, kernel_size=3, stride=2, pad=1), nn.ReLU(inplace=True))
        self.conv4 = nn.Sequential(convbn_3d(c * 2, c * 2, kernel_size=3, stride=1, pad=1), nn.ReLU(inplace=True))
        self.conv5 = nn.Sequential(nn.ConvTranspose3d(c * 2, c * 2, kernel_size=3, padding=1, output_padding=1,
                                                      stride=2, bias=False), nn.BatchNorm3d(c * 2))
        self.conv6 = nn.Sequential(nn.ConvTranspose3d(c * 2, c, kernel_size=3, padding=1, output_padding=1,
                                                      stride=2, bias=False), nn.BatchNorm3d(c))

    def forward(self, x, presqu, postsqu, skip=None):
        out = convbn_block(x, self.conv1[0], relu=True)
        pre = convbn_block(out, self.conv2, relu=True, residual=postsqu)
        out = convbn_block(pre, self.conv3[0], relu=True)
        out = convbn_block(out, self.conv4[0], relu=True)
        post = convbn_block(out, self.conv5, relu=True, residual=presqu if presqu is not None else pre)
        out = convbn_block(post, self.conv6, relu=False, residual=skip)
        return out, pre, post


def _classifier():
    return nn.Sequential(convbn_3d(32, 32, 3, 1, 1), nn.ReLU(inplace=True),
                         nn.Conv3d(32, 1, kernel_size=3, padding=1, stride=1, bias=False))


def _run_classifier(seq, x, add=None):
    h = convbn_block(x, seq[0], relu=True)
    cost = conv_block(h, seq[2], residual=None if add is None else add.unsqueeze(-1))
    return cost.squeeze(-1)


class PSMNet(nn.Module):
    def __init__(self, maxdisp=192):
        super().__init__()
        self.maxdisp = maxdisp
        self.feature_extraction = feature_extraction()
        self.dres0 = nn.Sequential(convbn_3d(64, 32, 3, 1, 1), nn.ReLU(inplace=True),
                                   convbn_3d(32, 32, 3, 1, 1), nn.ReLU(inplace=True))
        self.dres1 = nn.Sequential(convbn_3d(32, 32, 3, 1, 1), nn.ReLU(inplace=True), convbn_3d(32, 32, 3, 1, 1))
        self.dres2 = hourglass(32)
        self.dres3 = hourglass(32)
        self.dres4 = hourglass(32)
        self.classif1 = _classifier()
        self.classif2 = _classifier()
        self.classif3 = _classifier()
        init_reference_style(self)
        channels_last_weights_(self.feature_extraction)

    def forward(self, left, right):
        with deferred_bn_counters():
            fl, fr = run_pair(self.feature_extraction, left, right, self.training)
            return self.aggregate(fl, fr, left.shape[2], left.shape[3])

    @ops.fp32_region
    def aggregate(self, fl, fr, H, W):
        cost = ops.cost_volume(None, None, fl, fr, self.maxdisp // 4, 0, mask_left=True)
        cost0 = convbn_block(cost, self.dres0[0], relu=True)
        cost0 = convbn_block(cost0, self.dres0[2], relu=True)
        t = convbn_block(cost0, self.dres1[0], relu=True)
        cost0 = convbn_block(t, self.dres1[2], relu=False, residual=cost0)
        out1, pre1, post1 = self.dres2(cost0, None, None, skip=cost0)
        out2, pre2, post2 = self.dres3(out1, pre1, post1, skip=cost0)
        out3, pre3, post3 = self.dres4(out2, pre1, post2, skip=cost0)
        cost1 = _run_classifier(self.classif1, out1)
        cost2 = _run_classifier(self.classif2, out2, add=cost1)
        cost3 = _run_classifier(self.classif3, out3, add=cost2)
        pred3 = ops.regression_head(cost3, self.maxdisp, H, W).unsqueeze(1)
        if self.training:
            pred1 = ops.regression_head(cost1, self.maxdisp, H, W).unsqueeze(1)
            pred2 = ops.regression_head(cost2, self.maxdisp, H, W).unsqueeze(1)
            return [pred1, pred2, pred3]
        return pred3
```

stereo_toolbox_amd/ops.py:

```python
import ctypes

import torch

from ._capi import StxError, get_lib

_P = ctypes.c_void_p


class _DevPtr(ctypes.c_void_p):
    """A device pointer that remembers the device of the tensor it came from: _call() reads the launch device off its
    own arguments, so nothing survives between launches (an exception between building the arguments and the launch
    cannot leak state into the next one)."""


def _stream(dev=None):
    return _P(torch.cuda.current_stream(dev).cuda_stream)


def _p(t):
    if t is None:
        return None
    p = _DevPtr(t.data_ptr())
    p.dev = t.device
    return p


def on_device(t):
    return t.is_cuda


def _chk(t, name, dims=None):
    if t is None:
        return
    if not t.is_cuda:
        raise StxError(f"{name}: expected a ROCm device tensor, got {t.device} -- the cost-volume hot path has "
                       "no CPU fallback (the CPU oracle lives in oracle/ and is test-only)")
    if t.dtype != torch.float32:
        raise StxError(f"{name}: expected float32, got {t.dtype}")
    if not t.is_contiguous():
        raise StxError(f"{name}: expected a dense contiguous tensor, strides {t.stride()}")
    if dims is not None and t.dim() != dims:
        raise StxError(f"{name}: expected {dims} dims, got shape {tuple(t.shape)}")


def _call(name, *args):
    dev = None
    for a in args:
        if isinstance(a, _DevPtr):
            if dev is None:
                dev = a.dev
            elif a.dev != dev:
                raise StxError(f"{name}: operands live on different devices ({dev} and {a.dev})")
    if dev is not None and dev.type == "cuda" and dev.index != torch.cuda.current_device():
        with torch.cuda.device(dev):
            get_lib().call(name, *args, _stream(dev))
    else:
        get_lib().call(name, *args, _stream(dev))


_LOW = (torch.float16, torch.bfloat16)


def _to_fp32(v):
    if isinstance(v, torch.Tensor):
        return v.float() if v.dtype in _LOW else v
    if isinstance(v, dict):
        return {k: _to_fp32(x) for k, x in v.items()}
    if isinstance(v, (list, tuple)):
        return type(v)(_to_fp32(x) for x in v)
    return v


def autocast_active():
    return torch.is_autocast_enabled("cuda") or torch.is_autocast_enabled("cpu")


def fp32_region(fn):
    import functools

    @functools.wraps(fn)
    def wrapped(*args, **kwargs):
        if not autocast_active():
            return fn(*args, **kwargs)
        with torch.autocast("cuda", enabled=False), torch.autocast("cpu", enabled=False):
            return fn(*_to_fp32(args), **_to_fp32(kwargs))
    return wrapped


def to_ncdhw(x):
    return x.permute(0, 4, 1, 2, 3)


def to_ndhwc(x):
    return x.permute(0, 2, 3, 4, 1).contiguous()


class _Workspace:

    def __init__(self):
        self.bufs = {}

    def get(self, tag, nfloats, device):
        sid = torch.cuda.current_stream(device).cuda_stream if device.type == "cuda" else 0
        key = (device.index, sid, tag)
        b = self.bufs.get(key)
        if b is None or b.numel() < nfloats:
            b = torch.empty(int(nfloats), dtype=torch.float32, device=device)
            self.bufs[key] = b
        return b


_WS = _Workspace()


_CACHE_ENABLED = True


def set_weight_cache(enabled):
    global _CACHE_ENABLED
    _CACHE_ENABLED = bool(enabled)


def invalidate_caches(model):
    for m in model.modules():
        m.__dict__.pop("_stx_fold", None)
    for p in model.parameters():
        p.__dict__.pop("_stx_packed", None)


def pack_weight(w, mode, owner=None):
    _chk(w, "weight", 5)
    if owner is not None and _CACHE_ENABLED:
        cache = owner.__dict__.setdefault("_stx_packed", {})
        hit = cache.get(mode)
        if hit is not None and hit[0] == (owner._version, owner.data_ptr()):
            return hit[1]
    A, Bd = w.shape[0], w.shape[1]
    T = w.shape[2] * w.shape[3] * w.shape[4]
    K, N = (Bd, A) if mode == 0 else (A, Bd)
    n = get_lib().raw("stx_conv3d_packed_floats")(K, N, T)
    wp = torch.empty(n, dtype=torch.float32, device=w.device)
    _call("stx_conv3d_pack_weight", _p(w), _p(wp), A, Bd, T, mode)
    if owner is not None and _CACHE_ENABLED:
        cache[mode] = ((owner._version, owner.data_ptr()), wp)
    return wp


def _pad_channels(t, C):
    if t.shape[-1] == C:
        return t
    out = t.new_zeros(*t.shape[:-1], C)
    out[..., : t.shape[-1]] = t
    return out


def pad_input_channels(x, w):
    Cin = x.shape[-1]
    Cp = (Cin + 7) // 8 * 8
    if Cp == Cin:
        return x, w
    wp = w.new_zeros(w.shape[0], Cp, *w.shape[2:])
    wp[:, :Cin] = w
    return _pad_channels(x, Cp), wp


def pad_weight_channels(w, Cp):
    if w.shape[1] == Cp:
        return w
    wp = w.new_zeros(w.shape[0], Cp, *w.shape[2:])
    wp[:, : w.shape[1]] = w
    return wp


def conv_out_dims(D, H, W, ks, stride):
    pad = ks // 2
    return tuple((d + 2 * pad - ks) // stride + 1 for d in (D, H, W))


def conv3d_forward(x, wp, Cout, ks, stride, scale=None, bias=None, residual=None, relu=False, want_stats=False):
    _chk(x, "x", 5)
    B, D, H, W, Cin = x.shape
    Do, Ho, Wo = conv_out_dims(D, H, W, ks, stride)
    out = torch.empty(B, Do, Ho, Wo, Cout, dtype=torch.float32, device=x.device)
    stats = None
    if want_stats:
        rows = get_lib().raw("stx_conv3d_fwd_stat_rows")(B, D, H, W, Cin, Cout, ks, stride)
        stats = torch.empty(rows, 2, Cout, dtype=torch.float32, device=x.device)
    _call("stx_conv3d_fwd", _p(x), _p(wp), _p(out), _p(scale), _p(bias), _p(residual), _p(stats), B, D, H, W, Cin,
          Cout, ks, stride, int(relu))
    return out, stats


def deconv3d_forward(x, wp, Cout, out_dims=None, scale=None, bias=None, residual=None, relu=False, want_stats=False):
    _chk(x, "x", 5)
    B, D, H, W, Cin = x.shape
    Do, Ho, Wo = out_dims if out_dims is not None else (2 * D, 2 * H, 2 * W)
    if Cout > 64:
        if Cout % 64 != 0:
            raise StxError(f"deconv3d_forward: Cout={Cout} > 64 must be a multiple of 64")
        nt = Cout // 32
        wv = wp.view(-1, Cin // 8, nt, 256)
        outs, sts = [], []
        for h in range(Cout // 64):
            sl = slice(64 * h, 64 * h + 64)
            o, st_ = deconv3d_forward(x, wv[:, :, 2 * h:2 * h + 2].contiguous(), 64, (Do, Ho, Wo),
                                      None if scale is None else scale[sl].contiguous(),
                                      None if bias is None else bias[sl].contiguous(),
                                      None if residual is None else residual[..., sl].contiguous(), relu, want_stats)
            outs.append(o)
            sts.append(st_)
        return torch.cat(outs, -1), (torch.cat(sts, -1) if want_stats else None)
    out = torch.empty(B, Do, Ho, Wo, Cout, dtype=torch.float32, device=x.device)
    stats = None
    if want_stats:
        nb = get_lib().raw("stx_deconv3d_fwd_blocks")(D, H, W)
        stats = torch.empty(B * nb, 2, Cout, dtype=torch.float32, device=x.device)
    _call("stx_deconv3d_fwd", _p(x), _p(wp), _p(out), _p(scale), _p(bias), _p(residual), _p(stats), B, D, H, W, Cin,
          Cout, Do, Ho, Wo, int(relu))
    return out, stats


def conv3d_wgrad(fine, coarse, ks, stride):
    B, Df, Hf, Wf, CF = fine.shape
    _, Dc, Hc, Wc, CC = coarse.shape
    n = get_lib().raw("stx_conv3d_wgrad_workspace_floats")(B, Dc, Hc, Wc, CF, CC, ks, stride)
    ws = _WS.get("wgrad", n, fine.device)
    dw = torch.empty(CC, CF, ks ** 3, dtype=torch.float32, device=fine.device)
    _call("stx_conv3d_wgrad", _p(fine), _p(coarse), _p(dw), _p(ws), B, Df, Hf, Wf, CF, Dc, Hc, Wc, CC, ks, stride)
    return dw


def conv3d_wgrad_bn(x, gy, pend):
    B, D, H, W, CF = x.shape
    CC = gy.shape[-1]
    n = get_lib().raw("stx_conv3d_wgrad_workspace_floats")(B, D, H, W, CF, CC, 3, 1)
    ws = _WS.get("wgrad", n, x.device)
    dw = torch.empty(CC, CF, 27, dtype=torch.float32, device=x.device)
    dz = torch.empty_like(gy)
    _call("stx_conv3d_wgrad_bn", _p(x), _p(gy), _p(pend.z), _p(pend.scale), _p(pend.shift), _p(pend.mean), _p(pend.invstd),
          _p(pend.gamma), _p(pend.sums), float(pend.inv_n), int(pend.act), _p(dz), _p(dw), _p(ws), B, D, H, W, CF, CC)
    return dw, dz


class _PendingBn:
    __slots__ = ("g", "z", "scale", "shift", "mean", "invstd", "gamma", "sums", "inv_n", "act")

    def materialize(self):
        C = self.z.shape[-1]
        nvox = self.z.numel() // C
        dz = torch.empty_like(self.z)
        _call("stx_bn_bwd_apply2", _p(self.g), None, _p(self.z), _p(self.mean), _p(self.invstd), _p(self.gamma), None, None,
              None, None, _p(self.scale), _p(self.shift), None, None, _p(self.sums), _p(dz), None, None, nvox, C, int(self.act), 1)
        return dz


_BN_DEFER = {"outstanding": 0, "armed": False}


def _bn_defer_check():
    n, _BN_DEFER["outstanding"], _BN_DEFER["armed"] = _BN_DEFER["outstanding"], 0, False
    if n:
        raise StxError(f"{n} deferred BatchNorm-backward record(s) were not consumed by their convolution's backward node: "
                       "the gradients of this backward pass are wrong (set STX_BN_BWD_IN_WGRAD=0 and report)")


def _defer_pending_bn(g, pend):
    g._stx_pending_bn = pend
    _BN_DEFER["outstanding"] += 1
    if not _BN_DEFER["armed"]:
        _BN_DEFER["armed"] = True
        torch.autograd.Variable._execution_engine.queue_callback(_bn_defer_check)


def bn_defer_reset_if_stale():
    if not _BN_DEFER["armed"]:
        return
    task_id = getattr(torch._C, "_current_graph_task_id", None)
    if task_id is None or task_id() == -1:
        _BN_DEFER["outstanding"], _BN_DEFER["armed"] = 0, False


def _take_pending_bn(g):
    pend = getattr(g, "_stx_pending_bn", None) if g is not None else None
    if pend is not None:
        del g._stx_pending_bn
        _BN_DEFER["outstanding"] -= 1
        if pend.g is not g:
            raise StxError("deferred BatchNorm backward: record attached to a different gradient tensor")
    return pend


def _is_c1(w, ks, stride, transposed):
    return (not transposed) and ks == 3 and stride == 1 and w.shape[0] == 1 and w.shape[1] % 16 == 0 and w.shape[1] <= 64


def conv3d_c1_forward(x, w, residual=None):
    _chk(x, "x", 5)
    _chk(w, "weight", 5)
    B, D, H, W, Cin = x.shape
    out = torch.empty(B, D, H, W, 1, dtype=torch.float32, device=x.device)
    _call("stx_conv3d_c1_fwd", _p(x), _p(w), _p(residual), _p(out), B, D, H, W, Cin)
    return out


def conv3d_c1_wgrad(x, gy):
    B, D, H, W, Cin = x.shape
    ws = _WS.get("c1wgrad", get_lib().raw("stx_conv3d_c1_wgrad_workspace_floats")(Cin), x.device)
    dw = torch.empty(1, Cin, 3, 3, 3, dtype=torch.float32, device=x.device)
    _call("stx_conv3d_c1_wgrad", _p(x), _p(gy), _p(dw), _p(ws), B, D, H, W, Cin)
    return dw


def conv3d_c1_dgrad(gy, w, Cin):
    B, D, H, W, _ = gy.shape
    gx = torch.empty(B, D, H, W, Cin, dtype=torch.float32, device=gy.device)
    _call("stx_conv3d_c1_dgrad", _p(gy), _p(w), _p(gx), B, D, H, W, Cin)
    return gx


class ConvRawFn(torch.autograd.Function):

    @staticmethod
    def forward(ctx, x, w, ks, stride, transposed, want_stats):
        _chk(x, "x", 5)
        ctx.cin_true = None
        ctx.x_prepadded = False
        if not transposed and x.shape[-1] != w.shape[1]:
            if x.shape[-1] != (w.shape[1] + 7) // 8 * 8:
                raise StxError(f"conv: input has {x.shape[-1]} channels, weight expects {w.shape[1]}")
            ctx.cin_true, ctx.x_prepadded = w.shape[1], True
            w = pad_weight_channels(w, x.shape[-1])
        elif not transposed and x.shape[-1] % 8 != 0:
            ctx.cin_true = x.shape[-1]
            x, w = pad_input_channels(x, w)
        if _is_c1(w, ks, stride, transposed) and not want_stats:
            z, stats = conv3d_c1_forward(x, w.contiguous()), None
        elif transposed:
            Cout = w.shape[1]
            z, stats = deconv3d_forward(x, pack_weight(w, 2), Cout, want_stats=want_stats)
        else:
            Cout = w.shape[0]
            z, stats = conv3d_forward(x, pack_weight(w, 0), Cout, ks, stride, want_stats=want_stats)
        ctx.save_for_backward(x, w)
        ctx.cfg = (ks, stride, transposed)
        if stats is None:
            stats = x.new_empty(0)
        ctx.mark_non_differentiable(stats)
        return z, stats

    @staticmethod
    def backward(ctx, gz, _gstats):
        x, w = ctx.saved_tensors
        ks, stride, transposed = ctx.cfg
        pend = _take_pending_bn(gz)
        gx = gw = None
        B, D, H, W, Cin = x.shape
        if pend is not None:
            if (ctx.needs_input_grad[1] and not transposed and ks == 3 and stride == 1 and ctx.cin_true is None
                    and get_lib().raw("stx_conv3d_wgrad_bn_supported")(B, D, H, W, Cin, w.shape[0])):
                gw_pre, gz = conv3d_wgrad_bn(x, gz, pend)
                gw_pre = gw_pre.reshape(w.shape)
            else:
                gw_pre, gz = None, pend.materialize()
        else:
            gw_pre = None
        gz = gz.contiguous()
        if transposed:
            Ci, Co = w.shape[0], w.shape[1]
            if ctx.needs_input_grad[0]:
                gx, _ = conv3d_forward(gz, pack_weight(w, 0), Ci, 3, 2)
            if ctx.needs_input_grad[1]:
                gz_w = gz if Co % 32 == 0 else _pad_channels(gz, (Co + 31) // 32 * 32)
                x_w = x if Ci % 32 == 0 else _pad_channels(x, (Ci + 31) // 32 * 32)
                gw = conv3d_wgrad(gz_w, x_w, 3, 2)[:Ci, :Co].reshape(w.shape)
        else:
            Co, Ci = w.shape[0], w.shape[1]
            c1 = _is_c1(w, ks, stride, transposed)
            gz_k, w_k = gz, w
            if Co % 8 != 0 and not c1:
                Cp = (Co + 7) // 8 * 8
                gz_k = _pad_channels(gz, Cp)
                w_k = w.new_zeros(Cp, *w.shape[1:])
                w_k[:Co] = w
            if ctx.needs_input_grad[0]:
                if c1:
                    gx = conv3d_c1_dgrad(gz, w.contiguous(), Ci)
                elif stride == 1 and Ci > 128:
                    parts = []
                    for lo in range(0, Ci, 128):
                        hi = min(Ci, lo + 128)
                        g, _ = conv3d_forward(gz_k, pack_weight(w_k[:, lo:hi].contiguous(), 1), hi - lo, ks, 1)
                        parts.append(g)
                    gx = torch.cat(parts, -1)
                elif stride == 1:
                    gx, _ = conv3d_forward(gz_k, pack_weight(w_k, 1), Ci, ks, 1)
                else:
                    if Co % 32:
                        Cp = (Co + 31) // 32 * 32
                        gz_k = _pad_channels(gz, Cp)
                        w_k = w.new_zeros(Cp, *w.shape[1:])
                        w_k[:Co] = w
                    gx, _ = deconv3d_forward(gz_k, pack_weight(w_k, 2), Ci, out_dims=(D, H, W))
            if gw_pre is not None:
                gw = gw_pre
            elif ctx.needs_input_grad[1]:
                if c1:
                    gw = conv3d_c1_wgrad(x, gz)
                else:
                    gz_w = gz if Co % 32 == 0 else _pad_channels(gz, (Co + 31) // 32 * 32)
                    x_w = x if Ci % 32 == 0 else _pad_channels(x, (Ci + 31) // 32 * 32)
                    gw = conv3d_wgrad(x_w, gz_w, ks, stride)[:Co, :Ci].reshape(w.shape)
        if ctx.cin_true is not None:
            if gx is not None and not ctx.x_prepadded:
                gx = gx[..., :ctx.cin_true].contiguous()
            if gw is not None:
                gw = gw[:, :ctx.cin_true].contiguous()
        return gx, gw, None, None, None, None


AXIAL_MAX_CHANNELS = 192
AXIAL_MAX_TAPS = 17


def _axial_kernel(w, who):
    if w.dim() != 5:
        raise StxError(f"{who}: expected a weight [Cout, Cin, kd, kh, kw], got shape {tuple(w.shape)}")
    kd, kh, kw = (int(k) for k in w.shape[2:])
    planar = (kd, kh, kw) == (1, 3, 3)
    axial = kh == 1 and kw == 1 and kd % 2 == 1 and 3 <= kd <= AXIAL_MAX_TAPS
    if not (planar or axial):
        raise StxError(f"{who}: kernel {(kd, kh, kw)} is not served -- (1,3,3) or (kd,1,1) with kd odd, 3 <= kd <= {AXIAL_MAX_TAPS}")
    if w.shape[0] > AXIAL_MAX_CHANNELS or w.shape[1] > AXIAL_MAX_CHANNELS:
        raise StxError(f"{who}: {w.shape[1]} -> {w.shape[0]} channels, at most {AXIAL_MAX_CHANNELS} are served")
    return kd, kh, kw


def pack_weight_axial(w, mode, owner=None):
    _chk(w, "weight", 5)
    kd, kh, kw = _axial_kernel(w, "pack_weight_axial")
    if owner is not None and _CACHE_ENABLED:
        cache = owner.__dict__.setdefault("_stx_packed", {})
        hit = cache.get(("axial", mode))
        if hit is not None and hit[0] == (owner._version, owner.data_ptr()):
            return hit[1]
    A, Bd = w.shape[0], w.shape[1]
    K, N = (Bd, A) if mode == 0 else (A, Bd)
    n = get_lib().raw("stx_conv3d_axial_packed_floats")(K, N, kd, kh, kw)
    if n <= 0:
        raise StxError(f"pack_weight_axial: GEMM-K {K} (a multiple of 4), N {N}, kernel {(kd, kh, kw)} unsupported")
    wp = torch.empty(n, dtype=torch.float32, device=w.device)
    _call("stx_conv3d_axial_pack_weight", _p(w), _p(wp), A, Bd, kd, kh, kw, mode)
    if owner is not None and _CACHE_ENABLED:
        cache[("axial", mode)] = ((owner._version, owner.data_ptr()), wp)
    return wp


def conv3d_axial_forward(x, wp, Cout, kernel, scale=None, bias=None, residual=None, act=0, want_stats=False):
    _chk(x, "x", 5)
    B, D, H, W, Cin = x.shape
    kd, kh, kw = kernel
    out = torch.empty(B, D, H, W, Cout, dtype=torch.float32, device=x.device)
    stats = None
    if want_stats:
        rows = get_lib().raw("stx_conv3d_axial_fwd_stat_rows")(B, D, H, W, Cin, Cout, kd, kh, kw)
        stats = torch.empty(rows, 2, Cout, dtype=torch.float32, device=x.device)
    _call("stx_conv3d_axial_fwd", _p(x), _p(wp), _p(out), _p(scale), _p(bias), _p(residual), _p(stats), B, D, H, W, Cin, Cout,
          kd, kh, kw, int(act))
    return out, stats


def conv3d_axial_wgrad(x, gz, kernel):
    B, D, H, W, CF = x.shape
    CC = gz.shape[-1]
    kd, kh, kw = kernel
    n = get_lib().raw("stx_conv3d_axial_wgrad_workspace_floats")(B, D, H, W, CF, CC, kd, kh, kw)
    if n <= 0:
        raise StxError(f"conv3d_axial_wgrad: {CF} x {CC} channels, kernel {kernel} unsupported")
    ws = _WS.get("axwgrad", n, x.device)
    dw = torch.empty(CC, CF, kd * kh * kw, dtype=torch.float32, device=x.device)
    _call("stx_conv3d_axial_wgrad", _p(x), _p(gz), _p(dw), _p(ws), B, D, H, W, CF, CC, kd, kh, kw)
    return dw


def _pad4(C):
    return (C + 3) // 4 * 4


def _axial_prepare(x, w, who):
    _chk(x, "x", 5)
    _chk(w, "weight", 5)
    kernel = _axial_kernel(w, who)
    if x.shape[-1] != w.shape[1]:
        raise StxError(f"{who}: input has {x.shape[-1]} channels, weight expects {w.shape[1]}")
    Cp = _pad4(w.shape[1])
    if Cp != w.shape[1]:
        x, w = _pad_channels(x, Cp), pad_weight_channels(w, Cp)
    return x, w, kernel


def _axial_backward(x, w, kernel, gz, cin_true, need_x, need_w):
    gz = gz.contiguous()
    Co, Ci = w.shape[0], w.shape[1]
    gz_k, w_k = gz, w
    if Co % 4:
        Cp = _pad4(Co)
        gz_k = _pad_channels(gz, Cp)
        w_k = w.new_zeros(Cp, *w.shape[1:])
        w_k[:Co] = w
    gx = gw = None
    if need_x:
        gx, _ = conv3d_axial_forward(gz_k, pack_weight_axial(w_k, 1), Ci, kernel)
        if Ci != cin_true:
            gx = gx[..., :cin_true].contiguous()
    if need_w:
        gw = conv3d_axial_wgrad(x, gz_k, kernel)[:Co, :cin_true].reshape(Co, cin_true, *kernel)
        if not gw.is_contiguous():
            gw = gw.contiguous()
    return gx, gw


class AxialConvRawFn(torch.autograd.Function):

    @staticmethod
    def forward(ctx, x, w, want_stats):
        ctx.cin_true = w.shape[1]
        x, w, kernel = _axial_prepare(x, w, "AxialConvRawFn")
        z, stats = conv3d_axial_forward(x, pack_weight_axial(w, 0), w.shape[0], kernel, want_stats=want_stats)
        ctx.save_for_backward(x, w)
        ctx.kernel = kernel
        if stats is None:
            stats = x.new_empty(0)
        ctx.mark_non_differentiable(stats)
        return z, stats

    @staticmethod
    def backward(ctx, gz, _gstats):
        x, w = ctx.saved_tensors
        gx, gw = _axial_backward(x, w, ctx.kernel, gz, ctx.cin_true, ctx.needs_input_grad[0], ctx.needs_input_grad[1])
        return gx, gw, None


class _AxialConvBiasFn(torch.autograd.Function):

    @staticmethod
    def forward(ctx, x, w, bias):
        ctx.cin_true = w.shape[1]
        x, w, kernel = _axial_prepare(x, w, "conv3d_axial")
        z, _ = conv3d_axial_forward(x, pack_weight_axial(w, 0), w.shape[0], kernel, bias=bias.contiguous())
        ctx.save_for_backward(x, w)
        ctx.kernel = kernel
        return z

    @staticmethod
    def backward(ctx, gz):
        x, w = ctx.saved_tensors
        gx, gw = _axial_backward(x, w, ctx.kernel, gz, ctx.cin_true, ctx.needs_input_grad[0], ctx.needs_input_grad[1])
        gb = gz.sum((0, 1, 2, 3)) if ctx.needs_input_grad[2] else None
        return gx, gw, gb


class ZeroGradBiasFn(torch.autograd.Function):

    @staticmethod
    def forward(ctx, z, bias):
        ctx.save_for_backward(bias)
        return z.view_as(z)

    @staticmethod
    def backward(ctx, gz):
        (bias,) = ctx.saved_tensors
        return gz, torch.zeros_like(bias)


@fp32_region
def conv3d_axial(x, weight, bias=None):
    _chk(x, "x", 5)
    _chk(weight, "weight", 5)
    _chk(bias, "bias", 1)
    _axial_kernel(weight, "conv3d_axial")
    if bias is not None and bias.shape[0] != weight.shape[0]:
        raise StxError(f"conv3d_axial: bias of {bias.shape[0]} for {weight.shape[0]} output channels")
    if torch.is_grad_enabled() and any(t is not None and t.requires_grad for t in (x, weight, bias)):
        if bias is None:
            return AxialConvRawFn.apply(x, weight, False)[0]
        return _AxialConvBiasFn.apply(x, weight, bias)
    xk, wk, kernel = _axial_prepare(x, weight.detach(), "conv3d_axial")
    return conv3d_axial_forward(xk, pack_weight_axial(wk, 0), weight.shape[0], kernel, bias=None if bias is None else bias.detach())[0]


CONVGRU_MAX_HIDDEN = 128
CONVGRU_MAX_K = 512
CONVGRU_MAX_X = 3
CONVGRU_PACKS = 0


def _cl_pitch(t):
    B, C, H, W = t.shape
    sb, sc, sh, sw = t.stride()
    if C > 1 and sc != 1:
        return None
    pitch = sw if W > 1 else (sh if H > 1 else (sb if B > 1 else C))
    if pitch < C or pitch % 4 or t.data_ptr() % 16:
        return None
    if (W > 1 and sw != pitch) or (H > 1 and sh != W * pitch) or (B > 1 and sb != H * W * pitch):
        return None
    return pitch


def _cl_source(t):
    pitch = _cl_pitch(t)
    if pitch is None:
        t = t.contiguous(memory_format=torch.channels_last)
        pitch = _cl_pitch(t)
        if pitch is None:
            t = t.permute(0, 2, 3, 1).contiguous().permute(0, 3, 1, 2)
            pitch = t.shape[1]
    return t, pitch


def _convgru_chk(t, name, like=None, channels=None):
    if t is None:
        return
    if not on_device(t):
        raise StxError(f"convgru: {name}: expected a ROCm device tensor, got {t.device} -- the cell has no CPU fallback")
    if t.dtype != torch.float32:
        raise StxError(f"convgru: {name}: expected float32, got {t.dtype}")
    if like is not None:
        if t.dim() != 4 or t.shape[0] != like.shape[0] or tuple(t.shape[2:]) != tuple(like.shape[2:]):
            raise StxError(f"convgru: {name} has shape {tuple(t.shape)}, h has {tuple(like.shape)} (batch, H and W must agree)")
        if channels is not None and t.shape[1] != channels:
            raise StxError(f"convgru: {name} has {t.shape[1]} channels, expected {channels}")


def _convgru_pack(w0, w1, mode):
    global CONVGRU_PACKS
    key = tuple(v for w in (w0, w1) if w is not None for v in (w._version, w.data_ptr()))
    tag = ("convgru", mode, w1 is not None)
    if _CACHE_ENABLED:
        cache = w0.__dict__.setdefault("_stx_packed", {})
        hit = cache.get(tag)
        if hit is not None and hit[0] == key:
            return hit[1]
    A, Bd = w0.shape[0], w0.shape[1]
    nw = 1 if w1 is None else 2
    K, N = (Bd, nw * A) if mode == 0 else (nw * A, Bd)
    n = get_lib().raw("stx_convgru_packed_floats")(K, N)
    if n <= 0:
        raise StxError(f"convgru: GEMM-K {K} (a multiple of 4, <= {CONVGRU_MAX_K}) x N {N} unsupported")
    wp = torch.empty(n, dtype=torch.float32, device=w0.device)
    w0c, w1c = w0.detach().contiguous(), None if w1 is None else w1.detach().contiguous()
    _call("stx_convgru_pack_weight", _p(w0c), _p(w1c), _p(wp), A, Bd, mode)
    CONVGRU_PACKS += 1
    if _CACHE_ENABLED:
        cache[tag] = (key, wp)
    return wp


def _src_args(srcs):
    out = []
    for t, pitch in srcs:
        out += [_p(t), t.shape[1], pitch]
    for _ in range(4 - len(srcs)):
        out += [None, 0, 0]
    return out


def convgru_gemm(srcs, wp, N, B, H, W, epi=0, split=0, bias0=None, bias1=None, add0=None, add1=None, h=None, z=None, out0=None,
                 out1=None, out2=None, out_pitch=0):
    a0, a0p = add0 if add0 is not None else (None, 0)
    a1, a1p = add1 if add1 is not None else (None, 0)
    ht, hp = h if h is not None else (None, 0)
    _call("stx_convgru_gemm", *_src_args(srcs), _p(wp), N, epi, split, _p(bias0), _p(bias1), _p(a0), a0p, _p(a1), a1p, _p(ht), hp,
          _p(z), _p(out0), _p(out1), _p(out2), out_pitch, B, H, W)


def _nchw(t):
    return t.permute(0, 3, 1, 2)


class ConvGRUFn(torch.autograd.Function):

    @staticmethod
    def forward(ctx, h, cz, cr, cq, wz, bz, wr, br, wq, bq, *xs):
        B, hidden, H, W = h.shape
        dev = h.device
        need = any(ctx.needs_input_grad)
        hs = _cl_source(h.detach())
        xsrc = [_cl_source(x.detach()) for x in xs]
        cs = [None if c is None else _cl_source(c.detach()) for c in (cz, cr, cq)]
        new = lambda: torch.empty(B, H, W, hidden, dtype=torch.float32, device=dev)
        z, rh, hn = new(), new(), new()
        r = new() if need else None
        q = new() if need else None
        bzc, brc, bqc = (None if b is None else b.detach().contiguous() for b in (bz, br, bq))
        convgru_gemm([hs] + xsrc, _convgru_pack(wz, wr, 0), 2 * hidden, B, H, W, epi=1, split=hidden, bias0=bzc, bias1=brc,
                     add0=cs[0], add1=cs[1], h=hs, out0=z, out1=rh, out2=r)
        convgru_gemm([(_nchw(rh), hidden)] + xsrc, _convgru_pack(wq, None, 0), hidden, B, H, W, epi=2, split=hidden, bias0=bqc,
                     add0=cs[2], h=hs, z=z, out0=hn, out1=q)
        if need:
            ctx.save_for_backward(hs[0], z, r, q, rh, wz, wr, wq, *[t for t, _ in xsrc])
            ctx.pitches = (hs[1], [p for _, p in xsrc])
            ctx.has_c = [c is not None for c in (cz, cr, cq)]
            ctx.has_b = [b is not None for b in (bz, br, bq)]
        return _nchw(hn)

    @staticmethod
    def backward(ctx, g):
        h, z, r, q, rh, wz, wr, wq, *xt = ctx.saved_tensors
        hp, xp = ctx.pitches
        B, hidden, H, W = h.shape
        dev = h.device
        P = B * H * W
        need = ctx.needs_input_grad
        need_x = any(need[10:])
        need_w = any(need[i] for i in (4, 6, 8))
        need_b = any(need[i] for i in (5, 7, 9)) and any(ctx.has_b)
        cx = [t.shape[1] for t in xt]
        K = hidden + sum(cx)
        Ndg = K if need_x else hidden
        gt, gp = _cl_source(g)
# ... 145 lines not shown
        if ctx.needs_input_grad[0]:
            rank = lambda k: (0 if ctx.cfgs[k][0] == 3 and ctx.cfgs[k][1] == 1 else (1 if ctx.cfgs[k][1] == 2 else 2))
            for k in sorted((k for k in range(len(ws)) if gzs[k] is not None), key=rank):
                (ks, stride, _), w, gz = ctx.cfgs[k], ws[k], gzs[k]
                if stride == 1:
                    gx, _ = conv3d_forward(gz, pack_weight(w, 1), Ci, ks, 1, residual=gx)
                else:
                    Co = w.shape[0]
                    gz_k, w_k = gz, w
                    if Co % 32:
                        Cp = (Co + 31) // 32 * 32
                        gz_k = _pad_channels(gz, Cp)
                        w_k = w.new_zeros(Cp, *w.shape[1:])
                        w_k[:Co] = w
                    gx, _ = deconv3d_forward(gz_k, pack_weight(w_k, 2), Ci, out_dims=(D, H, W), residual=gx)
        for k, (w, gz) in enumerate(zip(ws, gzs)):
            if gz is None or not ctx.needs_input_grad[2 + k] or gws[k] is not None:
                continue
            ks, stride, _ = ctx.cfgs[k]
            Co = w.shape[0]
            gz_w = gz if Co % 32 == 0 else _pad_channels(gz, (Co + 31) // 32 * 32)
            x_w = x if Ci % 32 == 0 else _pad_channels(x, (Ci + 31) // 32 * 32)
            gws[k] = conv3d_wgrad(x_w, gz_w, ks, stride)[:Co, :Ci].reshape(w.shape)
        return (gx, None, *gws)


_D4_SEL = ((3, 1, 4), (4, 2, 0))


def embed_deconv4_weight(w):
    Ci, Co = w.shape[0], w.shape[1]
    wz = torch.cat((w, w.new_zeros(Ci, Co, 1, 4, 4)), 2)
    wz = torch.cat((wz, wz.new_zeros(Ci, Co, 5, 1, 4)), 3)
    wz = torch.cat((wz, wz.new_zeros(Ci, Co, 5, 5, 1)), 4)
    parts = []
    for pd in (0, 1):
        for ph in (0, 1):
            for pw in (0, 1):
                sel = wz[:, :, list(_D4_SEL[pd])][:, :, :, list(_D4_SEL[ph])][:, :, :, :, list(_D4_SEL[pw])]
                parts.append(sel.transpose(0, 1))
    return torch.cat(parts, 0).contiguous()


class DepthToSpaceFn(torch.autograd.Function):

    @staticmethod
    def forward(ctx, y):
        y = y.contiguous()
        _chk(y, "y", 5)
        B, D, H, W, C8 = y.shape
        C = C8 // 8
        out = torch.empty(B, 2 * D, 2 * H, 2 * W, C, dtype=torch.float32, device=y.device)
        _call("stx_depth_to_space", _p(y), _p(out), B, D, H, W, C, 0)
        return out

    @staticmethod
    def backward(ctx, g):
        g = g.contiguous()
        B, D2, H2, W2, C = g.shape
        gy = torch.empty(B, D2 // 2, H2 // 2, W2 // 2, 8 * C, dtype=torch.float32, device=g.device)
        _call("stx_depth_to_space", _p(g), _p(gy), B, D2 // 2, H2 // 2, W2 // 2, C, 1)
        return gy


def _d4_chunks(Co):
    per = max(1, min(8, 128 // Co))
    return [(c0, min(8, c0 + per)) for c0 in range(0, 8, per)]


def deconv4_raw(x, w, want_stats):
    Co = w.shape[1]
    if Co % 4:
        raise StxError(f"ConvTranspose3d(k4): {Co} output channels (need a multiple of 4)")
    w3 = embed_deconv4_weight(w)
    ys = [ConvRawFn.apply(x, w3[c0 * Co:c1 * Co], 3, 1, False, False)[0] for c0, c1 in _d4_chunks(Co)]
    z = DepthToSpaceFn.apply(ys[0] if len(ys) == 1 else torch.cat(ys, -1))
    return z, (bn_stats(z.detach()) if want_stats else z.new_empty(0))


@fp32_region
def deconv4_forward(x, w, scale=None, bias=None, relu=0, owner=None):
    _chk(x, "x", 5)
    Co = w.shape[1]
    if Co % 4:
        raise StxError(f"ConvTranspose3d(k4): {Co} output channels (need a multiple of 4)")
    cache = owner.__dict__.setdefault("_stx_packed", {}) if (owner is not None and _CACHE_ENABLED) else None
    key = (owner._version, owner.data_ptr()) if owner is not None else None
    hit = cache.get("d4") if cache is not None else None
    if hit is not None and hit[0] == key:
        packed = hit[1]
    else:
        w3 = embed_deconv4_weight(w)
        packed = [pack_weight(w3[c0 * Co:c1 * Co].contiguous(), 0) for c0, c1 in _d4_chunks(Co)]
        if cache is not None:
            cache["d4"] = (key, packed)
    ys = []
    for (c0, c1), wp in zip(_d4_chunks(Co), packed):
        n = c1 - c0
        ys.append(conv3d_forward(x, wp, n * Co, 3, 1, None if scale is None else scale.repeat(n),
                                 None if bias is None else bias.repeat(n), None, relu)[0])
    B, D, H, W, _ = x.shape
    y = ys[0] if len(ys) == 1 else torch.cat(ys, -1)
    out = torch.empty(B, 2 * D, 2 * H, 2 * W, Co, dtype=torch.float32, device=x.device)
    _call("stx_depth_to_space", _p(y), _p(out), B, D, H, W, Co, 0)
    return out


class GateFn(torch.autograd.Function):

    @staticmethod
    def forward(ctx, cv, att):
        out = gate(cv.detach(), att.detach())
        ctx.save_for_backward(cv, att)
        return out

    @staticmethod
    def backward(ctx, g):
        cv, att = ctx.saved_tensors
        g = g.contiguous()
        B, D, H, W, C = cv.shape
        gcv = torch.empty_like(cv) if ctx.needs_input_grad[0] else None
        gatt = torch.empty_like(att) if ctx.needs_input_grad[1] else None
        if gcv is not None or gatt is not None:
            _call("stx_gate_bwd", _p(g), _p(cv), _p(att), _p(gcv), _p(gatt), B, D, H * W, C)
        return gcv, gatt


@fp32_region
def gate(cv, att):
    if torch.is_grad_enabled() and (cv.requires_grad or att.requires_grad):
        return GateFn.apply(cv.contiguous(), att.contiguous())
    cv, att = cv.contiguous(), att.contiguous()
    _chk(cv, "cv", 5)
    _chk(att, "att", 4)
    B, D, H, W, C = cv.shape
    if att.shape != (B, H, W, C) or C % 4:
        raise StxError(f"gate: volume {tuple(cv.shape)} vs gate {tuple(att.shape)} (need [B,H,W,C], C % 4 == 0)")
    out = torch.empty_like(cv)
    _call("stx_gate_fwd", _p(cv), _p(att), _p(out), B, D, H * W, C)
    return out


class ChannelMajorFn(torch.autograd.Function):

    @staticmethod
    def forward(ctx, x):
        B, C, H, W = x.shape
        out = torch.empty((B, C, H, W), dtype=x.dtype, device=x.device)
        _call("stx_transpose", _p(x.permute(0, 2, 3, 1)), _p(out), B, H * W, C)
        return out

    @staticmethod
    def backward(ctx, g):
        g = g.contiguous()
        B, C, H, W = g.shape
        gx = torch.empty((B, H, W, C), dtype=g.dtype, device=g.device)
        _call("stx_transpose", _p(g), _p(gx), B, C, H * W)
        return gx.permute(0, 3, 1, 2)


@fp32_region
def channel_major(x):
    if x.is_contiguous():
        return x
    if (x.dim() == 4 and x.dtype == torch.float32 and on_device(x) and x.is_contiguous(memory_format=torch.channels_last)
            and x.shape[1] % 4 == 0 and (x.shape[2] * x.shape[3]) % 4 == 0):
        return ChannelMajorFn.apply(x)
    return x.contiguous()


class CatChannelsFn(torch.autograd.Function):

    @staticmethod
    def forward(ctx, *parts):
        ctx.cs = [int(p.shape[-1]) for p in parts]
        nvox = parts[0].numel() // ctx.cs[0]
        out = parts[0].new_empty(*parts[0].shape[:-1], sum(ctx.cs))
        ptrs = [_p(p) for p in parts] + [None] * (4 - len(parts))
        cs = ctx.cs + [0] * (4 - len(parts))
        _call("stx_concat_channels", *ptrs, *cs, _p(out), nvox)
        return out

    @staticmethod
    def backward(ctx, g):
        g = g.contiguous()
        nvox = g.numel() // g.shape[-1]
        outs = [g.new_empty(*g.shape[:-1], c) if need else None for c, need in zip(ctx.cs, ctx.needs_input_grad)]
        if any(o is not None for o in outs):
            dst = [o if o is not None else g.new_empty(*g.shape[:-1], c) for o, c in zip(outs, ctx.cs)]
            ptrs = [_p(o) for o in dst] + [None] * (4 - len(dst))
            cs = ctx.cs + [0] * (4 - len(dst))
            _call("stx_split_channels", _p(g), *ptrs, *cs, nvox)
        return tuple(outs)


@fp32_region
def cat_channels(parts):
    parts = [p.contiguous() for p in parts]
    if not 2 <= len(parts) <= 4:
        raise StxError(f"cat_channels: {len(parts)} parts (2 to 4)")
    lead = parts[0].shape[:-1]
    for p in parts:
        if p.shape[:-1] != lead or p.shape[-1] % 4 or p.dtype != torch.float32 or p.device != parts[0].device:
            raise StxError(f"cat_channels: parts {[tuple(q.shape) for q in parts]} (equal leading shape, fp32, widths % 4 == 0)")
    return CatChannelsFn.apply(*parts)


def conv2d_supported(conv):
    return (conv.kernel_size == (3, 3) and conv.stride == (1, 1) and conv.padding == (1, 1) and conv.dilation == (1, 1)
            and conv.groups == 1 and conv.bias is None and conv.in_channels in (32, 64) and conv.out_channels in (32, 64))


def _ohwi(w):
    v = w.permute(0, 2, 3, 1)
    return v if v.is_contiguous() else v.contiguous()


def conv2d_forward(x, w, dgrad=False, groups=1, want_stats=False):
    _chk(x, "x", 4)
    wo = _ohwi(w)
    _chk(wo, "weight", 4)
    B, H, W, Cin = x.shape
    Co, Ci = w.shape[0], w.shape[1]
    Kin, Nout = (Co, Ci) if dgrad else (Ci, Co)
    if Cin != Kin or B % groups:
        raise StxError(f"conv2d: input {tuple(x.shape)} against weight {tuple(w.shape)} (dgrad={dgrad}, groups={groups})")
    out = torch.empty(B, H, W, Nout, dtype=torch.float32, device=x.device)
    part = None
    if want_stats:
        rows = int(get_lib().raw("stx_conv2d_stat_rows")(groups))
        part = torch.empty(rows, 2, Nout, dtype=torch.float32, device=x.device)
    _call("stx_conv2d_fwd", _p(x), _p(wo), _p(out), _p(part), B, H, W, Kin, Nout, int(dgrad), groups)
    if part is not None and groups > 1:
        part = part.view(groups, rows // groups, 2, Nout)
    return out, part


class Conv2dFn(torch.autograd.Function):

    @staticmethod
    def forward(ctx, x, w, groups):
        xl = x.permute(0, 2, 3, 1)
        if not xl.is_contiguous():
            xl = xl.contiguous()
        z, part = conv2d_forward(xl, w, False, groups, True)
        ctx.save_for_backward(x, w)
        ctx.mark_non_differentiable(part)
        return z, part

    @staticmethod
    def backward(ctx, gz, _gpart):
        x, w = ctx.saved_tensors
        gz = gz.contiguous()
        gx = gw = None
        if ctx.needs_input_grad[0]:
            gx = conv2d_forward(gz, w, True)[0].permute(0, 3, 1, 2)
        if ctx.needs_input_grad[1]:
            gw = torch.ops.aten.convolution_backward(gz.permute(0, 3, 1, 2), x, w, None, (1, 1), (1, 1), (1, 1), False, (0, 0), 1,
                                                     (False, True, False))[1]
        return gx, gw, None


def bn_finalize(partials, count, gamma, beta, running_mean, running_var, momentum, eps, groups=1):
    C = partials.shape[-1]
    out = torch.empty(4, groups, C, dtype=torch.float32, device=partials.device)
    _call("stx_bn_finalize_groups", _p(partials), partials.shape[-3], C, float(count), _p(gamma), _p(beta),
          _p(running_mean), _p(running_var), float(momentum), float(eps), _p(out), groups)
    return list(out.unbind(0)) if groups > 1 else list(out[:, 0].unbind(0))


@fp32_region
def bn_stats(z, groups=1):
    _chk(z, "z")
    C = z.shape[-1]
    nvox = z.numel() // C // groups
    if groups < 1 or z.shape[0] % groups:
        raise StxError(f"bn_stats: leading axis {z.shape[0]} does not split into {groups} groups")
    rows = get_lib().raw("stx_bn_stats_rows")(nvox, C)
    if rows <= 0:
        raise StxError(f"bn_stats: C={C} unsupported")
    part = torch.empty(groups, rows, 2, C, dtype=torch.float32, device=z.device)
    _call("stx_bn_stats", _p(z), _p(part), nvox, C, groups)
    return part if groups > 1 else part[0]


def _sync_bn_partials(partials, count, group, world):
    import torch.distributed as dist
    tot = partials.double().sum(0)
    dist.all_reduce(tot, group=group)
    hi = tot.float()
    lo = (tot - hi.double()).float()
    return torch.stack((hi, lo)).contiguous(), count * world


@fp32_region
def bn_apply(z1, scale1, shift1, z2=None, scale2=None, shift2=None, relu=False, groups=1):
    out = torch.empty_like(z1)
    C = z1.shape[-1]
    _call("stx_bn_apply", _p(z1), _p(scale1), _p(shift1), _p(z2), _p(scale2), _p(shift2), _p(out),
          z1.numel() // C // groups, C, int(relu), groups)
    return out


class BnActFn(torch.autograd.Function):

    @staticmethod
    def forward(ctx, z1, gamma1, beta1, z2, gamma2, beta2, residual, relu, bn1, bn2, groups=1, defer=False):
        G = int(groups)
        ctx.defer = bool(defer)

        def affine(gamma, beta, bn):
            if bn["training"]:
                partials, count = bn["partials"], bn["count"]
                if bn.get("sync"):
                    if G > 1:
                        raise StxError("BnActFn: SyncBatchNorm with groups is not wired (SyncBN runs the views separately)")
                    partials, count = _sync_bn_partials(partials, count, *bn["sync"])
                return bn_finalize(partials, count, gamma, beta, bn["running_mean"], bn["running_var"], bn["momentum"],
                                   bn["eps"], G)
            invstd = torch.rsqrt(bn["running_var"] + bn["eps"])
            scale = gamma * invstd
            res = (scale, beta - bn["running_mean"] * scale, bn["running_mean"].clone(), invstd)
            return res if G == 1 else [t.unsqueeze(0).expand(G, -1).contiguous() for t in res]

        relu = int(relu)
        if relu == 2 and residual is not None:
            raise StxError("BnActFn: Mish with a plain residual is not wired (no model of the family uses it)")
        if G < 1 or z1.shape[0] % G:
            raise StxError(f"BnActFn: leading axis {z1.shape[0]} does not split into {G} groups")
        sc1, sh1, m1, i1 = affine(gamma1, beta1, bn1)
        two = z2 is not None
        if two:
            sc2, sh2, m2, i2 = affine(gamma2, beta2, bn2)
            y = bn_apply(z1, sc1, sh1, z2, sc2, sh2, relu, G)
        else:
            sc2 = sh2 = m2 = i2 = None
            y = bn_apply(z1, sc1, sh1, residual, None, None, relu, G)
        ctx.relu, ctx.two, ctx.has_res, ctx.groups = relu, two, residual is not None, G
        ctx.train1 = bn1["training"]
        ctx.train2 = bn2["training"] if two else False
        ctx.sync = bn1.get("sync") or (bn2.get("sync") if two else None)
        ctx.remask = bool(relu) and residual is None
        keep_y = y if (relu and not ctx.remask) else None
        ctx.save_for_backward(z1, gamma1, m1, i1, z2, gamma2, m2, i2, keep_y, sc1 if ctx.remask else None,
                              sh1 if ctx.remask else None, sc2 if (ctx.remask and two) else None,
                              sh2 if (ctx.remask and two) else None)
        return y

    @staticmethod
    def backward(ctx, gy):
        z1, gamma1, m1, i1, z2, gamma2, m2, i2, y, sc1, sh1, sc2, sh2 = ctx.saved_tensors
        gy = gy.contiguous()
        G = ctx.groups
        C = z1.shape[-1]
        nvox = z1.numel() // C // G
        lib = get_lib()
        NB = lib.raw("stx_bn_reduce_blocks")()
        part = _WS.get("bnred", G * NB * 3 * C, z1.device)
        sums_all = torch.empty(G + (1 if G > 1 else 0), 3, C, dtype=torch.float32, device=z1.device)
        sums = sums_all[:G]
        _call("stx_bn_bwd_reduce2", _p(gy), _p(y), _p(z1), _p(m1), _p(i1), _p(z2) if ctx.two else None,
              _p(m2) if ctx.two else None, _p(i2) if ctx.two else None, _p(sc1), _p(sh1), _p(sc2), _p(sh2), _p(part),
              _p(sums_all), nvox, C, int(ctx.relu), G)
        if not ctx.needs_input_grad[0] and not ctx.two and not ctx.has_res:
            tot = sums_all[G] if G > 1 else sums_all[0]
            return (None, tot[1], tot[0], None, None, None, None, None, None, None, None, None)
        if (ctx.defer and not ctx.two and not ctx.has_res and ctx.relu in (0, 1) and ctx.train1 and not ctx.sync and G == 1
                and (not ctx.relu or ctx.remask)):
            alias = gy.view_as(gy)
            pend = _PendingBn()
            pend.g, pend.z, pend.scale, pend.shift, pend.mean, pend.invstd = alias, z1, sc1, sh1, m1, i1
            pend.gamma, pend.sums, pend.inv_n, pend.act = gamma1, sums, 1.0 / nvox, int(ctx.relu)
            if pend.scale is None:
                pend.scale = pend.shift = m1
            _defer_pending_bn(alias, pend)
            tot = sums_all[0]
            return (alias, tot[1], tot[0], None, None, None, None, None, None, None, None, None)
        dz1 = torch.empty_like(z1)
        dz2 = torch.empty_like(z2) if ctx.two else None
        gres = torch.empty_like(z1) if (ctx.has_res and ctx.relu) else None
        use = sums
        if ctx.sync:
            import torch.distributed as dist
            use = sums.clone()
            dist.all_reduce(use, group=ctx.sync[0])
            use /= ctx.sync[1]
        if not ctx.train1 or (ctx.two and not ctx.train2):
            use = torch.zeros_like(sums)
        _call("stx_bn_bwd_apply2", _p(gy), _p(y), _p(z1), _p(m1), _p(i1), _p(gamma1), _p(z2) if ctx.two else None,
              _p(m2) if ctx.two else None, _p(i2) if ctx.two else None, _p(gamma2) if ctx.two else None, _p(sc1), _p(sh1),
              _p(sc2), _p(sh2), _p(use), _p(dz1), _p(dz2), _p(gres), nvox, C, int(ctx.relu), G)
        if ctx.has_res and not ctx.relu:
            gres = gy
        tot = sums_all[G] if G > 1 else sums_all[0]
        return (dz1, tot[1], tot[0], dz2, tot[2] if ctx.two else None, tot[0].clone() if ctx.two else None, gres,
                None, None, None, None, None)


class MishFn(torch.autograd.Function):

    @staticmethod
    def forward(ctx, x):
        x = x.contiguous()
        _chk(x, "x")
        y = torch.empty_like(x)
        _call("stx_mish_fwd", _p(x), _p(y), x.numel())
        ctx.save_for_backward(x)
        return y

    @staticmethod
    def backward(ctx, gy):
        (x,) = ctx.saved_tensors
        gy = gy.contiguous()
        gx = torch.empty_like(x)
        _call("stx_mish_bwd", _p(gy), _p(x), _p(gx), x.numel())
        return gx


@fp32_region
def mish(x):
    if torch.is_grad_enabled() and x.requires_grad:
        return MishFn.apply(x)
    x = x.contiguous()
    _chk(x, "x")
    y = torch.empty_like(x)
    _call("stx_mish_fwd", _p(x), _p(y), x.numel())
    return y


def _cv_shapes(Lg, Lc, num_groups):
    ref = Lg if Lg is not None else Lc
    B, _, H, W = ref.shape
    Cg = Lg.shape[1] if Lg is not None else 0
    Cc = Lc.shape[1] if Lc is not None else 0
    G = num_groups if Lg is not None else 0
    return B, H, W, Cg, G, Cc


@fp32_region
def cost_volume_forward(Lg, Rg, Lc, Rc, maxdisp, num_groups, mask_left=True, scale=None):
    for n, t in (("ref gwc", Lg), ("tgt gwc", Rg), ("ref concat", Lc), ("tgt concat", Rc)):
        _chk(t, n, 4)
    B, H, W, Cg, G, Cc = _cv_shapes(Lg, Lc, num_groups)
    if G:
        assert Cg % G == 0
    vol = torch.empty(B, maxdisp, H, W, G + 2 * Cc, dtype=torch.float32, device=(Lg if Lg is not None else Lc).device)
    _call("stx_cost_volume_fwd", _p(Lg), _p(Rg), Cg, G, _p(Lc), _p(Rc), Cc, _p(scale), _p(vol), B, H, W, maxdisp,
          int(mask_left))
    return vol


class CostVolumeFn(torch.autograd.Function):

    @staticmethod
    def forward(ctx, Lg, Rg, Lc, Rc, maxdisp, num_groups, mask_left):
        ctx.save_for_backward(Lg, Rg)
        ctx.cfg = (maxdisp, num_groups, mask_left, None if Lc is None else Lc.shape)
        return cost_volume_forward(Lg, Rg, Lc, Rc, maxdisp, num_groups, mask_left)

    @staticmethod
    def backward(ctx, gvol):
        Lg, Rg = ctx.saved_tensors
        maxdisp, num_groups, mask_left, cshape = ctx.cfg
        gvol = gvol.contiguous()
        B, D, H, W, CT = gvol.shape
        Cg = Lg.shape[1] if Lg is not None else 0
        G = num_groups if Lg is not None else 0
        Cc = cshape[1] if cshape is not None else 0
        gLg = torch.empty_like(Lg) if G else None
        gRg = torch.empty_like(Rg) if G else None
        gLc = gvol.new_empty(cshape) if Cc else None
        gRc = gvol.new_empty(cshape) if Cc else None
        _call("stx_cost_volume_bwd", _p(gvol), _p(Lg), _p(Rg), Cg, G, Cc, _p(gLg), _p(gRg), _p(gLc), _p(gRc), B, H, W,
              D, int(mask_left))
        return gLg, gRg, gLc, gRc, None, None, None


class GroupNormalizeFn(torch.autograd.Function):

    @staticmethod
    def forward(ctx, x, num_groups, out_scale):
        x = x.contiguous()
        _chk(x, "x", 4)
        B, C, H, W = x.shape
        y = torch.empty_like(x)
        _call("stx_group_normalize_fwd", _p(x), _p(y), B, C, num_groups, H * W, float(out_scale))
        ctx.save_for_backward(x)
        ctx.cfg = (num_groups, float(out_scale))
        return y

    @staticmethod
    def backward(ctx, gy):
        (x,) = ctx.saved_tensors
        gy = gy.contiguous()
        B, C, H, W = x.shape
        gx = torch.empty_like(x)
        _call("stx_group_normalize_bwd", _p(x), _p(gy), _p(gx), B, C, ctx.cfg[0], H * W, ctx.cfg[1])
        return gx, None, None


@fp32_region
def group_normalize(x, num_groups, out_scale=1.0):
    assert x.dim() == 4 and x.shape[1] % num_groups == 0, f"C:{x.shape[1]}, num_groups:{num_groups}"
    return GroupNormalizeFn.apply(channel_major(x), num_groups, out_scale)


@fp32_region
def cost_volume(Lg, Rg, Lc, Rc, maxdisp, num_groups, mask_left=True, normalize=False):
    if normalize and Lg is not None:
        Lg = group_normalize(Lg, num_groups, float(Lg.shape[1] // num_groups))
        Rg = group_normalize(Rg, num_groups, 1.0)
    ts = [channel_major(t) if t is not None else None for t in (Lg, Rg, Lc, Rc)]
    if torch.is_grad_enabled() and any(t is not None and t.requires_grad for t in ts):
        return CostVolumeFn.apply(*ts, maxdisp, num_groups, mask_left)
    return cost_volume_forward(*ts, maxdisp, num_groups, mask_left)


class SampledVolumeFn(torch.autograd.Function):

    @staticmethod
    def forward(ctx, Lg, Rg, Lc, Rc, samples, num_groups):
        B, H, W, Cg, G, Cc = _cv_shapes(Lg, Lc, num_groups)
        S = samples.shape[1]
        CTp = (G + 2 * Cc + 1 + 7) // 8 * 8
        vol = torch.empty(B, S, H, W, CTp, dtype=torch.float32, device=samples.device)
        _call("stx_sampled_volume_fwd", _p(Lg), _p(Rg), Cg, G, _p(Lc), _p(Rc), Cc, _p(samples), _p(vol), B, H, W, S, CTp)
        ctx.save_for_backward(Lg, Rg, samples)
        ctx.cfg = (G, Cg, Cc, None if Lc is None else Lc.shape)
        return vol

    @staticmethod
    def backward(ctx, gvol):
        Lg, Rg, samples = ctx.saved_tensors
        G, Cg, Cc, cshape = ctx.cfg
        gvol = gvol.contiguous()
        B, S, H, W, CTp = gvol.shape
        gLg = torch.empty_like(Lg) if G else None
        gRg = torch.empty_like(Rg) if G else None
        gLc = gvol.new_empty(cshape) if Cc else None
        gRc = gvol.new_empty(cshape) if Cc else None
        _call("stx_sampled_volume_bwd", _p(gvol), _p(Lg), _p(Rg), Cg, G, Cc, _p(samples), _p(gLg), _p(gRg), _p(gLc),
              _p(gRc), B, H, W, S, CTp)
        return gLg, gRg, gLc, gRc, None, None


@fp32_region
def sampled_volume(Lg, Rg, Lc, Rc, samples, num_groups):
    ts = [channel_major(t) if t is not None else None for t in (Lg, Rg, Lc, Rc)]
    for n, t in (("ref gwc", ts[0]), ("tgt gwc", ts[1]), ("ref concat", ts[2]), ("tgt concat", ts[3])):
        _chk(t, n, 4)
    samples = samples.detach().contiguous()
    _chk(samples, "samples", 4)
    if ts[0] is not None:
        assert ts[0].shape[1] % num_groups == 0
    if torch.is_grad_enabled() and any(t is not None and t.requires_grad for t in ts):
        return SampledVolumeFn.apply(*ts, samples, num_groups)
    return SampledVolumeFn.forward(_NoCtx(), *ts, samples, num_groups)


class _NoCtx:

    def save_for_backward(self, *a):
        pass

    def mark_non_differentiable(self, *a):
        pass


class WarpFn(torch.autograd.Function):

    @staticmethod
    def forward(ctx, x, disp):
        B, C, H, W = x.shape
        out = torch.empty_like(x)
        _call("stx_warp_fwd", _p(x), _p(disp), _p(out), B, C, H, W)
        ctx.save_for_backward(x, disp)
        return out

    @staticmethod
    def backward(ctx, g):
        x, disp = ctx.saved_tensors
        B, C, H, W = x.shape
        g = g.contiguous()
        gx = torch.empty_like(x) if ctx.needs_input_grad[0] else None
        gd = torch.empty_like(disp) if ctx.needs_input_grad[1] else None
        _call("stx_warp_bwd", _p(g), _p(x), _p(disp), _p(gx), _p(gd), B, C, H, W)
        return gx, gd


@fp32_region
def warp(x, disp):
    x, disp = x.contiguous(), disp.contiguous()
    _chk(x, "x", 4)
    _chk(disp, "disp", 4)
    if disp.shape != (x.shape[0], 1, x.shape[2], x.shape[3]):
        raise StxError(f"warp: disp {tuple(disp.shape)} does not match x {tuple(x.shape)}")
    if torch.is_grad_enabled() and (x.requires_grad or disp.requires_grad):
        return WarpFn.apply(x, disp)
    return WarpFn.forward(_NoCtx(), x, disp)


class CorrVolumeFn(torch.autograd.Function):

    @staticmethod
    def forward(ctx, ref, tgt, maxdisp, groups):
        B, C, H, W = ref.shape
        vol = torch.empty(B, groups, 2 * maxdisp + 1, H, W, dtype=torch.float32, device=ref.device)
        _call("stx_corr_volume_fwd", _p(ref), _p(tgt), _p(vol), B, C, H, W, maxdisp, groups)
        ctx.save_for_backward(ref, tgt)
        ctx.cfg = (maxdisp, groups)
        return vol

    @staticmethod
    def backward(ctx, g):
        ref, tgt = ctx.saved_tensors
        B, C, H, W = ref.shape
        g = g.contiguous()
        gr = torch.empty_like(ref) if ctx.needs_input_grad[0] else None
        gt = torch.empty_like(tgt) if ctx.needs_input_grad[1] else None
        _call("stx_corr_volume_bwd", _p(g), _p(ref), _p(tgt), _p(gr), _p(gt), B, C, H, W, *ctx.cfg)
        return gr, gt, None, None


@fp32_region
def corr_volume(ref, tgt, maxdisp, groups):
    ref, tgt = ref.contiguous(), tgt.contiguous()
    _chk(ref, "ref", 4)
    _chk(tgt, "tgt", 4)
    if ref.shape != tgt.shape:
        raise StxError(f"corr_volume: ref {tuple(ref.shape)} vs tgt {tuple(tgt.shape)}")
    if torch.is_grad_enabled() and (ref.requires_grad or tgt.requires_grad):
        return CorrVolumeFn.apply(ref, tgt, int(maxdisp), int(groups))
    return CorrVolumeFn.forward(_NoCtx(), ref, tgt, int(maxdisp), int(groups))


class DisparityVarianceFn(torch.autograd.Function):

    @staticmethod
    def forward(ctx, x, disp, samples):
        B, D = x.shape[0], x.shape[1]
        HW = x.shape[2] * x.shape[3]
        out = torch.empty(B, 1, x.shape[2], x.shape[3], dtype=torch.float32, device=x.device)
        _call("stx_disparity_variance_fwd", _p(x), _p(disp), _p(samples), _p(out), B, D, HW)
        ctx.save_for_backward(x, disp, samples)
        return out

    @staticmethod
    def backward(ctx, g):
        x, disp, samples = ctx.saved_tensors
        B, D = x.shape[0], x.shape[1]
        HW = x.shape[2] * x.shape[3]
        g = g.contiguous()
        need = ctx.needs_input_grad
        gx = torch.empty_like(x) if need[0] else None
        gd = torch.empty_like(disp) if need[1] else None
        gs = torch.empty_like(samples) if (samples is not None and need[2]) else None
        if gx is None and gd is None and gs is None:
            return None, None, None
        _call("stx_disparity_variance_bwd", _p(g), _p(x), _p(disp), _p(samples), _p(gx), _p(gd), _p(gs), B, D, HW)
        return gx, gd, gs


@fp32_region
def disparity_variance(x, disp, samples=None):
    x, disp = x.contiguous(), disp.contiguous()
    _chk(x, "x", 4)
    _chk(disp, "disparity", 4)
    if disp.shape != (x.shape[0], 1, x.shape[2], x.shape[3]):
        raise StxError(f"disparity_variance: disparity {tuple(disp.shape)} does not match x {tuple(x.shape)}")
    if samples is not None:
        samples = samples.contiguous()
        _chk(samples, "samples", 4)
        if samples.shape != x.shape:
            raise StxError(f"disparity_variance: samples {tuple(samples.shape)} vs x {tuple(x.shape)}")
    if torch.is_grad_enabled() and any(t is not None and t.requires_grad for t in (x, disp, samples)):
        return DisparityVarianceFn.apply(x, disp, samples)
    return DisparityVarianceFn.forward(_NoCtx(), x, disp, samples)


class AcVolumeFn(torch.autograd.Function):

    @staticmethod
    def forward(ctx, Lc, Rc, prob, maxdisp):
        ctx.save_for_backward(Lc, Rc, prob)
        ctx.maxdisp = maxdisp
        return cost_volume_forward(None, None, Lc, Rc, maxdisp, 0, mask_left=False, scale=prob)

    @staticmethod
    def backward(ctx, gvol):
        Lc, Rc, prob = ctx.saved_tensors
        gvol = gvol.contiguous()
        B, D, H, W, CT = gvol.shape
        Cc = Lc.shape[1]
        gprob = torch.empty_like(prob)
        gL, gR = torch.empty_like(Lc), torch.empty_like(Rc)
        if D * W * 4 <= 150 * 1024:
            _call("stx_ac_volume_bwd", _p(gvol), _p(Lc), _p(Rc), _p(prob), _p(gL), _p(gR), _p(gprob), B, Cc, H, W, D, 0)
            return gL, gR, gprob, None
        _call("stx_cost_volume_scale_bwd", _p(gvol), _p(Lc), _p(Rc), _p(gprob), B, Cc, H, W, D, 0)
# ... 1783 lines not shown
```

Before: 0.1787 pairs/s.

## Fuse BN+ReLU into the Cout=1 classifier conv's input load, forward and wgrad

Adds BN-affine+ReLU-on-load variants of the single-output-channel 3D conv forward and weight-gradient MFMA kernels, plus a BnReluC1Fn autograd function and classifier_tail helper. The classifier's intermediate BN+ReLU activation no longer needs to be written out and re-read. The backward recomputes the activation inside the wgrad kernel and reuses the shared BN backward path. This adds template branches and per-element recompute, and depends on the model file (truncated here) routing its classifiers through classifier_tail.

```diff
diff --git a/include/stx_hip.h b/include/stx_hip.h
--- a/include/stx_hip.h
+++ b/include/stx_hip.h
@@ -95,6 +95,11 @@
 int stx_conv3d_c1_wgrad(const float* x, const float* gy, float* dw, float* workspace, int B, int D, int H, int W,
                         int Cin, void* stream);
 int stx_conv3d_c1_dgrad(const float* gy, const float* w, float* gx, int B, int D, int H, int W, int Cin, void* stream);
+int stx_conv3d_c1_bn_supported(int B, int D, int H, int W, int Cin);
+int stx_conv3d_c1_fwd_bn(const float* z, const float* scale, const float* shift, const float* w, const float* residual,
+                         float* out, int B, int D, int H, int W, int Cin, void* stream);
+int stx_conv3d_c1_wgrad_bn(const float* z, const float* scale, const float* shift, const float* gy, float* dw,
+                           float* workspace, int B, int D, int H, int W, int Cin, void* stream);
 
 int stx_mish_fwd(const float* x, float* y, long long n, void* stream);
 int stx_mish_bwd(const float* gy, const float* x, float* gx, long long n, void* stream);
diff --git a/stereo_toolbox_amd/_capi.py b/stereo_toolbox_amd/_capi.py
--- a/stereo_toolbox_amd/_capi.py
+++ b/stereo_toolbox_amd/_capi.py
@@ -64,6 +64,9 @@
     "stx_conv3d_c1_wgrad_workspace_floats": [_I],
     "stx_conv3d_c1_wgrad": [_P, _P, _P, _P, _I, _I, _I, _I, _I, _P],
     "stx_conv3d_c1_dgrad": [_P, _P, _P, _I, _I, _I, _I, _I, _P],
+    "stx_conv3d_c1_bn_supported": [_I, _I, _I, _I, _I],
+    "stx_conv3d_c1_fwd_bn": [_P, _P, _P, _P, _P, _P, _I, _I, _I, _I, _I, _P],
+    "stx_conv3d_c1_wgrad_bn": [_P, _P, _P, _P, _P, _P, _I, _I, _I, _I, _I, _P],
     "stx_mish_fwd": [_P, _P, _L, _P],
     "stx_mish_bwd": [_P, _P, _P, _L, _P],
     "stx_depth_to_space": [_P, _P, _I, _I, _I, _I, _I, _I, _P],
diff --git a/stereo_toolbox_amd/aggregation.py b/stereo_toolbox_amd/aggregation.py
--- a/stereo_toolbox_amd/aggregation.py
+++ b/stereo_toolbox_amd/aggregation.py
@@ -159,6 +159,17 @@
 
 
 @ops.fp32_region
+def skip_input_conv(x, seq):
+    conv, bn = seq[0], seq[1]
+    if (_is_transposed(conv) or not bn.training or _conv_cfg(conv) != (3, 1) or conv.weight.shape[1] != x.shape[-1]
+            or conv.weight.shape[1] % 8 or conv.weight.shape[0] % 8 or conv.weight.shape[1] > 128
+            or not x.requires_grad or not torch.is_grad_enabled()):
+        return None, x
+    z, part, x_skip = ops.ConvRawSkipFn.apply(x, conv.weight, True)
+    return (z, part), x_skip
+
+
+@ops.fp32_region
 def conv_block(x, conv, bn=None, relu=False, second=None, residual=None, mish=False, leaky=False, raw=None, second_raw=None):
     if (mish and relu) or (leaky and (relu or mish)):
         raise ops.StxError("conv_block: relu, mish and leaky are mutually exclusive")
@@ -202,12 +213,34 @@
         z2, part2 = second_raw if second_raw is not None else _raw_conv(x2, conv2, want2)
         st2 = _bn_state(bn2, part2 if want2 else None, z2.numel() // z2.shape[-1])
         return ops.BnActFn.apply(z1, bn.weight, bn.bias, z2, bn2.weight, bn2.bias, None, relu, st1, st2)
+    defer = _defers_bn_backward(conv, st1, want, relu, residual)
+    return ops.BnActFn.apply(z1, bn.weight, bn.bias, None, None, None, residual, relu, st1, None, 1, defer)
+
+
+def _defers_bn_backward(conv, st, want, relu, residual):
     defer = (residual is None and want and relu in (0, 1, False, True) and not _is_transposed(conv) and _conv_cfg(conv) == (3, 1)
-             and conv.weight.shape[0] % 32 == 0 and conv.weight.shape[1] % 32 == 0 and not st1.get("sync")
+             and conv.weight.shape[0] % 32 == 0 and conv.weight.shape[1] % 32 == 0 and not st.get("sync")
              and os.environ.get("STX_BN_BWD_IN_WGRAD", "1") != "0")
     if defer:
         ops.bn_defer_reset_if_stale()
-    return ops.BnActFn.apply(z1, bn.weight, bn.bias, None, None, None, residual, relu, st1, None, 1, defer)
+    return defer
+
+
+@ops.fp32_region
+def classifier_tail(x, seq, tail, add=None, raw=None):
+    conv, bn = seq[0], seq[1]
+    on_load = (os.environ.get("STX_C1_BN_ON_LOAD", "1") != "0" and bn.training and isinstance(tail, nn.Conv3d)
+               and not _is_transposed(conv) and _conv_cfg(conv) == (3, 1) and _conv_cfg(tail) == (3, 1)
+               and tuple(tail.weight.shape[:2]) == (1, conv.weight.shape[0])
+               and (raw is not None or _needs_grad(x, conv, bn, tail, add))
+               and ops.conv3d_c1_bn_supported(*x.shape[:4], conv.weight.shape[0]))
+    if not on_load:
+        h = conv_block(x, conv, bn, relu=True, raw=raw)
+        return conv_block(h, tail, residual=add)
+    z, part = raw if raw is not None else _raw_conv(x, conv, True)
+    st = _bn_state(bn, part, z.numel() // z.shape[-1])
+    defer = _defers_bn_backward(conv, st, True, True, None)
+    return ops.BnReluC1Fn.apply(z, bn.weight, bn.bias, tail.weight, add, st, defer)
 
 
 def _axial_cfg(conv):
diff --git a/stereo_toolbox_amd/csrc/conv_c1.hip b/stereo_toolbox_amd/csrc/conv_c1.hip
--- a/stereo_toolbox_amd/csrc/conv_c1.hip
+++ b/stereo_toolbox_amd/csrc/conv_c1.hip
@@ -266,11 +266,15 @@
 constexpr int C1M_ED = C1M_TD + 2, C1M_EH = C1M_TH + 2, C1M_EW = C1M_TW + 2;
 constexpr int C1M_BLOCKS = 1024;
 
+__device__ __forceinline__ float c1_bn_relu(float z, float sc, float sh) { return stx_act(fmaf(z, sc, sh), 1); }
+
+template <bool BN>
 __global__ __launch_bounds__(C1_THREADS) void conv_c1_wgrad_mfma_kernel(const float* __restrict__ x,
                                                                         const float* __restrict__ gy,
                                                                         float* __restrict__ slab, int B, int D, int H,
                                                                         int W, int Cin, int nDt, int nHt, int nWt,
-                                                                        int ntiles) {
+                                                                        int ntiles, const float* __restrict__ scale,
+                                                                        const float* __restrict__ shift) {
     __shared__ float gys[C1M_ED * C1M_EH * C1M_EW];
     __shared__ float red[4][1024];
     const int tid = threadIdx.x, lane = tid & 63, wave = tid >> 6;
@@ -281,6 +285,8 @@
     f32x16 acc;
 #pragma unroll
     for (int r = 0; r < 16; ++r) acc[r] = 0.f;
+    float sc = 0.f, sh = 0.f;
+    if constexpr (BN) { sc = scale[cb * 32 + i]; sh = shift[cb * 32 + i]; }
     for (int t = blockIdx.x; t < ntiles; t += gridDim.x) {
         int r = t;
         const int wt = r % nWt; r /= nWt;
@@ -307,6 +313,13 @@
 #pragma unroll
             for (int p = 0; p < 16; ++p)
                 av[p] = (rowok && w0 + 2 * p + half < W) ? xr[(size_t)(2 * p) * Cin] : 0.f;
+            if constexpr (BN) {
+#pragma unroll
+                for (int p = 0; p < 16; ++p) {
+                    const float t = c1_bn_relu(av[p], sc, sh);
+                    av[p] = (rowok && w0 + 2 * p + half < W) ? t : 0.f;
+                }
+            }
             const float* gp = gys + (ld * C1M_EH + lh) * C1M_EW + toff;
 #pragma unroll
             for (int p = 0; p < 16; ++p) {
@@ -347,11 +360,14 @@
 constexpr int C1F_MT = (C1F_NV + 31) / 32;
 constexpr int C1F_WGS = 512;
 
+template <bool BN>
 __global__ __launch_bounds__(C1_THREADS) void conv_c1_fwd_mfma_kernel(const float* __restrict__ x,
                                                                       const float* __restrict__ w,
                                                                       const float* __restrict__ res,
                                                                       float* __restrict__ out, int B, int D, int H, int W,
-                                                                      int nHt, int nWt, int ncols) {
+                                                                      int nHt, int nWt, int ncols,
+                                                                      const float* __restrict__ scale,
+                                                                      const float* __restrict__ shift) {
     STX_DYN_SMEM(smem);
     float* Ps = reinterpret_cast<float*>(smem);
     const int tid = threadIdx.x, lane = tid & 63, wave = __builtin_amdgcn_readfirstlane(tid >> 6);
@@ -359,6 +375,11 @@
     float wreg[16];
 #pragma unroll
     for (int s_ = 0; s_ < 16; ++s_) wreg[s_] = (i < 27) ? w[(size_t)(16 * half + s_) * 27 + i] : 0.f;
+    float4 bsc[BN ? 4 : 1], bsh[BN ? 4 : 1];
+    if constexpr (BN) {
+#pragma unroll
+        for (int q = 0; q < 4; ++q) { bsc[q] = stx_ld4(scale + 16 * half + 4 * q); bsh[q] = stx_ld4(shift + 16 * half + 4 * q); }
+    }
     const int lh = tid / C1F_TW, lw = tid % C1F_TW;
 
     constexpr int MTW = (C1F_MT + 3) / 4;
@@ -411,6 +432,16 @@
                 for (int t = 0; t < MTW; ++t) {
                     const int m = wave + 4 * t;
                     if (m < C1F_MT) {
+                        if constexpr (BN) {
+                            const bool vin = voff[t] != STX_BUF_OOB;
+#pragma unroll
+                            for (int q = 0; q < 4; ++q) {
+                                cur[t][q].x = vin ? c1_bn_relu(cur[t][q].x, bsc[q].x, bsh[q].x) : 0.f;
+                                cur[t][q].y = vin ? c1_bn_relu(cur[t][q].y, bsc[q].y, bsh[q].y) : 0.f;
+                                cur[t][q].z = vin ? c1_bn_relu(cur[t][q].z, bsc[q].z, bsh[q].z) : 0.f;
+                                cur[t][q].w = vin ? c1_bn_relu(cur[t][q].w, bsc[q].w, bsh[q].w) : 0.f;
+                            }
+                        }
                         f32x16 acc;
 #pragma unroll
                         for (int r = 0; r < 16; ++r) acc[r] = 0.f;
@@ -458,23 +489,32 @@
 
 }
 
+static bool c1_fwd_mfma_ok(int B, int D, int H, int W, int Cin) {
+    return Cin == 32 && B > 0 && D > 0 && H > 0 && W > 0 && (long long)H * W * 128 < (1ll << 31);
+}
+
+template <bool BN>
+static int c1_fwd_mfma_launch(const float* x, const float* w, const float* residual, float* out, int B, int D, int H, int W,
+                              const float* scale, const float* shift, void* stream, const char* what) {
+    const int nHt = stx_cdiv(H, C1F_TH), nWt = stx_cdiv(W, C1F_TW);
+    const long long ncols = (long long)B * nHt * nWt, units = ncols * D;
+    STX_REQUIRE(units < (1ll << 31), "%s: volume too large", what);
+    long long g = C1F_WGS;
+    if (g > units / 4) g = units / 4 > 0 ? units / 4 : 1;
+    const size_t lds = (size_t)2 * C1F_NV * 27 * 4;
+    if (int rc = stx_lds_require((const void*)conv_c1_fwd_mfma_kernel<BN>, lds, what)) return rc;
+    hipLaunchKernelGGL(conv_c1_fwd_mfma_kernel<BN>, dim3((unsigned)g), dim3(C1_THREADS), lds, (hipStream_t)stream, x, w,
+                       residual, out, B, D, H, W, nHt, nWt, (int)ncols, scale, shift);
+    return stx_check_launch(what);
+}
+
 extern "C" int stx_conv3d_c1_fwd(const float* x, const float* w, const float* residual, float* out, int B, int D,
                                  int H, int W, int Cin, void* stream) {
     stx_begin();
     STX_REQUIRE(x && w && out && B > 0 && D > 0 && H > 0 && W > 0, "conv3d_c1_fwd: bad shape");
     STX_REQUIRE(Cin % C1_CK == 0, "conv3d_c1_fwd: Cin=%d must be a multiple of %d", Cin, C1_CK);
-    if (Cin == 32 && (long long)H * W * 128 < (1ll << 31)) {
-        const int nHt = stx_cdiv(H, C1F_TH), nWt = stx_cdiv(W, C1F_TW);
-        const long long ncols = (long long)B * nHt * nWt, units = ncols * D;
-        STX_REQUIRE(units < (1ll << 31), "conv3d_c1_fwd: volume too large");
-        long long g = C1F_WGS;
-        if (g > units / 4) g = units / 4 > 0 ? units / 4 : 1;
-        const size_t lds = (size_t)2 * C1F_NV * 27 * 4;
-        if (int rc = stx_lds_require((const void*)conv_c1_fwd_mfma_kernel, lds, "conv3d_c1_fwd(mfma)")) return rc;
-        hipLaunchKernelGGL(conv_c1_fwd_mfma_kernel, dim3((unsigned)g), dim3(C1_THREADS), lds, (hipStream_t)stream, x, w,
-                           residual, out, B, D, H, W, nHt, nWt, (int)ncols);
-        return stx_check_launch("conv3d_c1_fwd(mfma)");
-    }
+    if (c1_fwd_mfma_ok(B, D, H, W, Cin))
+        return c1_fwd_mfma_launch<false>(x, w, residual, out, B, D, H, W, nullptr, nullptr, stream, "conv3d_c1_fwd(mfma)");
     C1Args a;
     a.x = x; a.w = w; a.gy = nullptr; a.res = residual; a.out = out;
     a.B = B; a.D = D; a.H = H; a.W = W; a.Cin = Cin;
@@ -485,10 +525,42 @@
     return stx_check_launch("conv3d_c1_fwd");
 }
 
+extern "C" int stx_conv3d_c1_bn_supported(int B, int D, int H, int W, int Cin) {
+    if (!c1_fwd_mfma_ok(B, D, H, W, Cin)) return 0;
+    const long long units = (long long)B * stx_cdiv(H, C1F_TH) * stx_cdiv(W, C1F_TW) * D;
+    const long long nt = (long long)B * stx_cdiv(D, C1M_TD) * stx_cdiv(H, C1M_TH) * stx_cdiv(W, C1M_TW);
+    return units < (1ll << 31) && nt < (1ll << 31);
+}
+
+extern "C" int stx_conv3d_c1_fwd_bn(const float* z, const float* scale, const float* shift, const float* w,
+                                    const float* residual, float* out, int B, int D, int H, int W, int Cin, void* stream) {
+    stx_begin();
+    STX_REQUIRE(z && scale && shift && w && out, "conv3d_c1_fwd_bn: null operand");
+    STX_REQUIRE(stx_conv3d_c1_bn_supported(B, D, H, W, Cin), "conv3d_c1_fwd_bn: shape %dx%dx%dx%dx%d is not served", B, D, H,
+                W, Cin);
+    return c1_fwd_mfma_launch<true>(z, w, residual, out, B, D, H, W, scale, shift, stream, "conv3d_c1_fwd_bn");
+}
+
 extern "C" long long stx_conv3d_c1_wgrad_workspace_floats(int Cin) {
     const long long valu = (long long)C1_WGRAD_BLOCKS * Cin * 27;
     const long long mfma = (long long)C1M_BLOCKS * 1024 * ((Cin + 31) / 32);
     return valu > mfma ? valu : mfma;
+}
+
+template <bool BN>
+static int c1_wgrad_mfma_launch(const float* x, const float* gy, float* dw, float* workspace, int B, int D, int H, int W,
+                                int Cin, const float* scale, const float* shift, void* stream, const char* what) {
+    const int nDt = stx_cdiv(D, C1M_TD), nHt = stx_cdiv(H, C1M_TH), nWt = stx_cdiv(W, C1M_TW);
+    const long long nt = (long long)B * nDt * nHt * nWt;
+    STX_REQUIRE(nt < (1ll << 31), "%s: volume too large", what);
+    const int nblk = nt < C1M_BLOCKS ? (int)nt : C1M_BLOCKS;
+    hipStream_t st = (hipStream_t)stream;
+    hipLaunchKernelGGL(conv_c1_wgrad_mfma_kernel<BN>, dim3(nblk, Cin / 32), dim3(C1_THREADS), 0, st, x, gy, workspace, B,
+                       D, H, W, Cin, nDt, nHt, nWt, (int)nt, scale, shift);
+    int rc = stx_check_launch(what);
+    if (rc) return rc;
+    hipLaunchKernelGGL(c1m_reduce_kernel, dim3(Cin * 27), dim3(C1_THREADS), 0, st, workspace, nblk, dw);
+    return stx_check_launch("conv3d_c1_wgrad(reduce)");
 }
 
 extern "C" int stx_conv3d_c1_wgrad(const float* x, const float* gy, float* dw, float* workspace, int B, int D, int H,
@@ -496,19 +568,9 @@
     stx_begin();
     STX_REQUIRE(x && gy && dw && workspace && B > 0, "conv3d_c1_wgrad: null operand");
     STX_REQUIRE(Cin % C1_CK == 0 && Cin <= 4 * C1_CK, "conv3d_c1_wgrad: Cin=%d must be 16..64 in steps of 16", Cin);
-    if (Cin % 32 == 0) {
-        const int nDt = stx_cdiv(D, C1M_TD), nHt = stx_cdiv(H, C1M_TH), nWt = stx_cdiv(W, C1M_TW);
-        const long long nt = (long long)B * nDt * nHt * nWt;
-        STX_REQUIRE(nt < (1ll << 31), "conv3d_c1_wgrad: volume too large");
-        const int nblk = nt < C1M_BLOCKS ? (int)nt : C1M_BLOCKS;
-        hipStream_t st = (hipStream_t)stream;
-        hipLaunchKernelGGL(conv_c1_wgrad_mfma_kernel, dim3(nblk, Cin / 32), dim3(C1_THREADS), 0, st, x, gy, workspace, B,
-                           D, H, W, Cin, nDt, nHt, nWt, (int)nt);
-        int rc = stx_check_launch("conv3d_c1_wgrad(mfma)");
-        if (rc) return rc;
-        hipLaunchKernelGGL(c1m_reduce_kernel, dim3(Cin * 27), dim3(C1_THREADS), 0, st, workspace, nblk, dw);
-        return stx_check_launch("conv3d_c1_wgrad(reduce)");
-    }
+    if (Cin % 32 == 0)
+        return c1_wgrad_mfma_launch<false>(x, gy, dw, workspace, B, D, H, W, Cin, nullptr, nullptr, stream,
+                                           "conv3d_c1_wgrad(mfma)");
     C1Args a;
     a.x = x; a.w = nullptr; a.gy = gy; a.res = nullptr; a.out = workspace;
     a.B = B; a.D = D; a.H = H; a.W = W; a.Cin = Cin;
@@ -524,6 +586,15 @@
     return stx_check_launch("conv3d_c1_colsum");
 }
 
+extern "C" int stx_conv3d_c1_wgrad_bn(const float* z, const float* scale, const float* shift, const float* gy, float* dw,
+                                      float* workspace, int B, int D, int H, int W, int Cin, void* stream) {
+    stx_begin();
+    STX_REQUIRE(z && scale && shift && gy && dw && workspace, "conv3d_c1_wgrad_bn: null operand");
+    STX_REQUIRE(stx_conv3d_c1_bn_supported(B, D, H, W, Cin), "conv3d_c1_wgrad_bn: shape %dx%dx%dx%dx%d is not served", B, D,
+                H, W, Cin);
+    return c1_wgrad_mfma_launch<true>(z, gy, dw, workspace, B, D, H, W, Cin, scale, shift, stream, "conv3d_c1_wgrad_bn");
+}
+
 extern "C" int stx_conv3d_c1_dgrad(const float* gy, const float* w, float* gx, int B, int D, int H, int W, int Cin,
                                    void* stream) {
     stx_begin();
diff --git a/stereo_toolbox_amd/models/GwcNet/gwcnet.py b/stereo_toolbox_amd/models/GwcNet/gwcnet.py
--- a/stereo_toolbox_amd/models/GwcNet/gwcnet.py
+++ b/stereo_toolbox_amd/models/GwcNet/gwcnet.py
@@ -2,7 +2,7 @@
 import torch.nn as nn
 
 from ... import ops
-from ...aggregation import conv_block, convbn_block, deferred_bn_counters, shared_input_convs
+from ...aggregation import classifier_tail, convbn_block, deferred_bn_counters, shared_input_convs, skip_input_conv
 from ..features2d import ResTrunk, cat_features, channels_last_weights_, convbn, init_reference_style, run_head2d, run_pair
 from .submodule import convbn_3d
 
@@ -60,8 +60,7 @@
 
 
 def run_classifier(seq, x, add=None, raw=None):
-    h = convbn_block(x, seq[0], relu=True, raw=raw)
-    cost = conv_block(h, seq[2], residual=None if add is None else add.unsqueeze(-1))
+    cost = classifier_tail(x, seq[0], seq[2], add=None if add is None else add.unsqueeze(-1), raw=raw)
     return cost.squeeze(-1)
 
 
@@ -101,8 +100,9 @@
                               fr.get("concat_feature"), self.maxdisp // 4, self.num_groups, mask_left=True)
         cost0 = convbn_block(vol, self.dres0[0], relu=True)
         cost0 = convbn_block(cost0, self.dres0[2], relu=True)
-        t = convbn_block(cost0, self.dres1[0], relu=True)
-        cost0 = convbn_block(t, self.dres1[2], relu=False, residual=cost0)
+        raw, skip = skip_input_conv(cost0, self.dres1[0])
+        t = convbn_block(cost0, self.dres1[0], relu=True, raw=raw)
+        cost0 = convbn_block(t, self.dres1[2], relu=False, residual=skip)
         if self.training:
             out1, r0 = self.dres2(cost0, also=self.classif0[0])
             out2, r1 = self.dres3(out1, also=self.classif1[0])
diff --git a/stereo_toolbox_amd/models/PSMNet/stackhourglass.py b/stereo_toolbox_amd/models/PSMNet/stackhourglass.py
--- a/stereo_toolbox_amd/models/PSMNet/stackhourglass.py
+++ b/stereo_toolbox_amd/models/PSMNet/stackhourglass.py
@@ -1,7 +1,7 @@
 import torch.nn as nn
 
 from ... import ops
-from ...aggregation import conv_block, convbn_block, deferred_bn_counters
+from ...aggregation import classifier_tail, convbn_block, deferred_bn_counters
 from ..features2d import channels_last_weights_, init_reference_style, run_pair
 from .submodule import convbn_3d, feature_extraction
 
@@ -36,8 +36,7 @@
 
 
 def _run_classifier(seq, x, add=None):
-    h = convbn_block(x, seq[0], relu=True)
-    cost = conv_block(h, seq[2], residual=None if add is None else add.unsqueeze(-1))
+    cost = classifier_tail(x, seq[0], seq[2], add=None if add is None else add.unsqueeze(-1))
     return cost.squeeze(-1)
 
 
diff --git a/stereo_toolbox_amd/ops.py b/stereo_toolbox_amd/ops.py
--- a/stereo_toolbox_amd/ops.py
+++ b/stereo_toolbox_amd/ops.py
@@ -311,11 +311,105 @@
     return dw
 
 
+def conv3d_c1_bn_supported(B, D, H, W, Cin):
+    return bool(get_lib().raw("stx_conv3d_c1_bn_supported")(B, D, H, W, Cin))
+
+
+def conv3d_c1_forward_bn(z, scale, shift, w, residual=None):
+    _chk(z, "z", 5)
+    _chk(w, "weight", 5)
+    _chk(residual, "add", 5)
+    B, D, H, W, Cin = z.shape
+    out = torch.empty(B, D, H, W, 1, dtype=torch.float32, device=z.device)
+    _call("stx_conv3d_c1_fwd_bn", _p(z), _p(scale), _p(shift), _p(w), _p(residual), _p(out), B, D, H, W, Cin)
+    return out
+
+
+def conv3d_c1_wgrad_bn(z, scale, shift, gy):
+    B, D, H, W, Cin = z.shape
+    ws = _WS.get("c1wgrad", get_lib().raw("stx_conv3d_c1_wgrad_workspace_floats")(Cin), z.device)
+    dw = torch.empty(1, Cin, 3, 3, 3, dtype=torch.float32, device=z.device)
+    _call("stx_conv3d_c1_wgrad_bn", _p(z), _p(scale), _p(shift), _p(gy), _p(dw), _p(ws), B, D, H, W, Cin)
+    return dw
+
+
 def conv3d_c1_dgrad(gy, w, Cin):
     B, D, H, W, _ = gy.shape
     gx = torch.empty(B, D, H, W, Cin, dtype=torch.float32, device=gy.device)
     _call("stx_conv3d_c1_dgrad", _p(gy), _p(w), _p(gx), B, D, H, W, Cin)
     return gx
+
+
+def _conv_raw_backward(ctx, gz, skip=None):
+    x, w = ctx.saved_tensors
+    ks, stride, transposed = ctx.cfg
+    pend = _take_pending_bn(gz)
+    gx = gw = None
+    B, D, H, W, Cin = x.shape
+    if pend is not None:
+        if (ctx.needs_input_grad[1] and not transposed and ks == 3 and stride == 1 and ctx.cin_true is None
+                and get_lib().raw("stx_conv3d_wgrad_bn_supported")(B, D, H, W, Cin, w.shape[0])):
+            gw_pre, gz = conv3d_wgrad_bn(x, gz, pend)
+            gw_pre = gw_pre.reshape(w.shape)
+        else:
+            gw_pre, gz = None, pend.materialize()
+    else:
+        gw_pre = None
+    gz = gz.contiguous()
+    if transposed:
+        Ci, Co = w.shape[0], w.shape[1]
+        if ctx.needs_input_grad[0]:
+            gx, _ = conv3d_forward(gz, pack_weight(w, 0), Ci, 3, 2)
+        if ctx.needs_input_grad[1]:
+            gz_w = gz if Co % 32 == 0 else _pad_channels(gz, (Co + 31) // 32 * 32)
+            x_w = x if Ci % 32 == 0 else _pad_channels(x, (Ci + 31) // 32 * 32)
+            gw = conv3d_wgrad(gz_w, x_w, 3, 2)[:Ci, :Co].reshape(w.shape)
+    else:
+        Co, Ci = w.shape[0], w.shape[1]
+        c1 = _is_c1(w, ks, stride, transposed)
+        gz_k, w_k = gz, w
+        if Co % 8 != 0 and not c1:
+            Cp = (Co + 7) // 8 * 8
+            gz_k = _pad_channels(gz, Cp)
+            w_k = w.new_zeros(Cp, *w.shape[1:])
+            w_k[:Co] = w
+        if ctx.needs_input_grad[0]:
+            if c1:
+                gx = conv3d_c1_dgrad(gz, w.contiguous(), Ci)
+            elif stride == 1 and Ci > 128:
+                parts = []
+                for lo in range(0, Ci, 128):
+                    hi = min(Ci, lo + 128)
+                    g, _ = conv3d_forward(gz_k, pack_weight(w_k[:, lo:hi].contiguous(), 1), hi - lo, ks, 1)
+                    parts.append(g)
+                gx = torch.cat(parts, -1)
+            elif stride == 1:
+                gx, _ = conv3d_forward(gz_k, pack_weight(w_k, 1), Ci, ks, 1, residual=skip)
+                skip = None
+            else:
+                if Co % 32:
+                    Cp = (Co + 31) // 32 * 32
+                    gz_k = _pad_channels(gz, Cp)
+                    w_k = w.new_zeros(Cp, *w.shape[1:])
+                    w_k[:Co] = w
+                gx, _ = deconv3d_forward(gz_k, pack_weight(w_k, 2), Ci, out_dims=(D, H, W))
+        if gw_pre is not None:
+            gw = gw_pre
+        elif ctx.needs_input_grad[1]:
+            if c1:
+                gw = conv3d_c1_wgrad(x, gz)
+            else:
+                gz_w = gz if Co % 32 == 0 else _pad_channels(gz, (Co + 31) // 32 * 32)
+                x_w = x if Ci % 32 == 0 else _pad_channels(x, (Ci + 31) // 32 * 32)
+                gw = conv3d_wgrad(x_w, gz_w, ks, stride)[:Co, :Ci].reshape(w.shape)
+    if skip is not None and ctx.needs_input_grad[0]:
+        raise StxError("conv backward: a skip gradient on a layer whose data gradient cannot take it")
+    if ctx.cin_true is not None:
+        if gx is not None and not ctx.x_prepadded:
+            gx = gx[..., :ctx.cin_true].contiguous()
+        if gw is not None:
+            gw = gw[:, :ctx.cin_true].contiguous()
+    return gx, gw
 
 
 class ConvRawFn(torch.autograd.Function):
@@ -350,72 +444,28 @@
 
     @staticmethod
     def backward(ctx, gz, _gstats):
-        x, w = ctx.saved_tensors
-        ks, stride, transposed = ctx.cfg
-        pend = _take_pending_bn(gz)
-        gx = gw = None
-        B, D, H, W, Cin = x.shape
-        if pend is not None:
-            if (ctx.needs_input_grad[1] and not transposed and ks == 3 and stride == 1 and ctx.cin_true is None
-                    and get_lib().raw("stx_conv3d_wgrad_bn_supported")(B, D, H, W, Cin, w.shape[0])):
-                gw_pre, gz = conv3d_wgrad_bn(x, gz, pend)
-                gw_pre = gw_pre.reshape(w.shape)
-            else:
-                gw_pre, gz = None, pend.materialize()
+        return (*_conv_raw_backward(ctx, gz), None, None, None, None)
+
+
+class ConvRawSkipFn(torch.autograd.Function):
+
+    @staticmethod
+    def forward(ctx, x, w, want_stats):
+        if (x.shape[-1] != w.shape[1] or w.shape[1] % 8 or w.shape[0] % 8 or w.shape[1] > 128 or tuple(w.shape[2:]) != (3, 3, 3)
+                or _is_c1(w, 3, 1, False)):
+            raise StxError(f"ConvRawSkipFn: weight {tuple(w.shape)} on an input of {x.shape[-1]} channels")
+        z, stats = ConvRawFn.forward(ctx, x, w, 3, 1, False, want_stats)
+        return z, stats, x.view_as(x)
+
+    @staticmethod
+    def backward(ctx, gz, _gstats, gskip):
+        if gz is None:
+            return gskip, None, None
+        if gskip is not None and ctx.needs_input_grad[0]:
+            gskip = gskip.contiguous()
         else:
-            gw_pre = None
-        gz = gz.contiguous()
-        if transposed:
-            Ci, Co = w.shape[0], w.shape[1]
-            if ctx.needs_input_grad[0]:
-                gx, _ = conv3d_forward(gz, pack_weight(w, 0), Ci, 3, 2)
-            if ctx.needs_input_grad[1]:
-                gz_w = gz if Co % 32 == 0 else _pad_channels(gz, (Co + 31) // 32 * 32)
-                x_w = x if Ci % 32 == 0 else _pad_channels(x, (Ci + 31) // 32 * 32)
-                gw = conv3d_wgrad(gz_w, x_w, 3, 2)[:Ci, :Co].reshape(w.shape)
-        else:
-            Co, Ci = w.shape[0], w.shape[1]
-            c1 = _is_c1(w, ks, stride, transposed)
-            gz_k, w_k = gz, w
-            if Co % 8 != 0 and not c1:
-                Cp = (Co + 7) // 8 * 8
-                gz_k = _pad_channels(gz, Cp)
-                w_k = w.new_zeros(Cp, *w.shape[1:])
-                w_k[:Co] = w
-            if ctx.needs_input_grad[0]:
-                if c1:
-                    gx = conv3d_c1_dgrad(gz, w.contiguous(), Ci)
-                elif stride == 1 and Ci > 128:
-                    parts = []
-                    for lo in range(0, Ci, 128):
-                        hi = min(Ci, lo + 128)
-                        g, _ = conv3d_forward(gz_k, pack_weight(w_k[:, lo:hi].contiguous(), 1), hi - lo, ks, 1)
-                        parts.append(g)
-                    gx = torch.cat(parts, -1)
-                elif stride == 1:
-                    gx, _ = conv3d_forward(gz_k, pack_weight(w_k, 1), Ci, ks, 1)
-                else:
-                    if Co % 32:
-                        Cp = (Co + 31) // 32 * 32
-                        gz_k = _pad_channels(gz, Cp)
-                        w_k = w.new_zeros(Cp, *w.shape[1:])
-                        w_k[:Co] = w
-                    gx, _ = deconv3d_forward(gz_k, pack_weight(w_k, 2), Ci, out_dims=(D, H, W))
-            if gw_pre is not None:
-                gw = gw_pre
-            elif ctx.needs_input_grad[1]:
-                if c1:
-                    gw = conv3d_c1_wgrad(x, gz)
-                else:
-                    gz_w = gz if Co % 32 == 0 else _pad_channels(gz, (Co + 31) // 32 * 32)
-                    x_w = x if Ci % 32 == 0 else _pad_channels(x, (Ci + 31) // 32 * 32)
-                    gw = conv3d_wgrad(x_w, gz_w, ks, stride)[:Co, :Ci].reshape(w.shape)
-        if ctx.cin_true is not None:
-            if gx is not None and not ctx.x_prepadded:
-                gx = gx[..., :ctx.cin_true].contiguous()
-            if gw is not None:
-                gw = gw[:, :ctx.cin_true].contiguous()
-        return gx, gw, None, None, None, None
+            gskip = None
+        return (*_conv_raw_backward(ctx, gz, gskip), None)
 
 
 AXIAL_MAX_CHANNELS = 192
@@ -1167,36 +1217,85 @@
     return out
 
 
+def _bn_act_backward(ctx, saved, gy, need_z1):
+    z1, gamma1, m1, i1, z2, gamma2, m2, i2, y, sc1, sh1, sc2, sh2 = saved
+    gy = gy.contiguous()
+    G = ctx.groups
+    C = z1.shape[-1]
+    nvox = z1.numel() // C // G
+    lib = get_lib()
+    NB = lib.raw("stx_bn_reduce_blocks")()
+    part = _WS.get("bnred", G * NB * 3 * C, z1.device)
+    sums_all = torch.empty(G + (1 if G > 1 else 0), 3, C, dtype=torch.float32, device=z1.device)
+    sums = sums_all[:G]
+    _call("stx_bn_bwd_reduce2", _p(gy), _p(y), _p(z1), _p(m1), _p(i1), _p(z2) if ctx.two else None,
+          _p(m2) if ctx.two else None, _p(i2) if ctx.two else None, _p(sc1), _p(sh1), _p(sc2), _p(sh2), _p(part),
+          _p(sums_all), nvox, C, int(ctx.relu), G)
+    if not need_z1 and not ctx.two and not ctx.has_res:
+        tot = sums_all[G] if G > 1 else sums_all[0]
+        return (None, tot[1], tot[0], None, None, None, None, None, None, None, None, None)
+    if (ctx.defer and not ctx.two and not ctx.has_res and ctx.relu in (0, 1) and ctx.train1 and not ctx.sync and G == 1
+            and (not ctx.relu or ctx.remask)):
+        alias = gy.view_as(gy)
+        pend = _PendingBn()
+        pend.g, pend.z, pend.scale, pend.shift, pend.mean, pend.invstd = alias, z1, sc1, sh1, m1, i1
+        pend.gamma, pend.sums, pend.inv_n, pend.act = gamma1, sums, 1.0 / nvox, int(ctx.relu)
+        if pend.scale is None:
+            pend.scale = pend.shift = m1
+        _defer_pending_bn(alias, pend)
+        tot = sums_all[0]
+        return (alias, tot[1], tot[0], None, None, None, None, None, None, None, None, None)
+    dz1 = torch.empty_like(z1)
+    dz2 = torch.empty_like(z2) if ctx.two else None
+    gres = torch.empty_like(z1) if (ctx.has_res and ctx.relu) else None
+    use = sums
+    if ctx.sync:
+        import torch.distributed as dist
+        use = sums.clone()
+        dist.all_reduce(use, group=ctx.sync[0])
+        use /= ctx.sync[1]
+    if not ctx.train1 or (ctx.two and not ctx.train2):
+        use = torch.zeros_like(sums)
+    _call("stx_bn_bwd_apply2", _p(gy), _p(y), _p(z1), _p(m1), _p(i1), _p(gamma1), _p(z2) if ctx.two else None,
+          _p(m2) if ctx.two else None, _p(i2) if ctx.two else None, _p(gamma2) if ctx.two else None, _p(sc1), _p(sh1),
+          _p(sc2), _p(sh2), _p(use), _p(dz1), _p(dz2), _p(gres), nvox, C, int(ctx.relu), G)
+    if ctx.has_res and not ctx.relu:
+        gres = gy
+    tot = sums_all[G] if G > 1 else sums_all[0]
+    return (dz1, tot[1], tot[0], dz2, tot[2] if ctx.two else None, tot[0].clone() if ctx.two else None, gres,
+            None, None, None, None, None)
+
+
+def _bn_affine(gamma, beta, bn, G=1):
+    if bn["training"]:
+        partials, count = bn["partials"], bn["count"]
+        if bn.get("sync"):
+            if G > 1:
+                raise StxError("BnActFn: SyncBatchNorm with groups is not wired (SyncBN runs the views separately)")
+            partials, count = _sync_bn_partials(partials, count, *bn["sync"])
+        return bn_finalize(partials, count, gamma, beta, bn["running_mean"], bn["running_var"], bn["momentum"],
+                           bn["eps"], G)
+    invstd = torch.rsqrt(bn["running_var"] + bn["eps"])
+    scale = gamma * invstd
+    res = (scale, beta - bn["running_mean"] * scale, bn["running_mean"].clone(), invstd)
+    return res if G == 1 else [t.unsqueeze(0).expand(G, -1).contiguous() for t in res]
+
+
 class BnActFn(torch.autograd.Function):
 
     @staticmethod
     def forward(ctx, z1, gamma1, beta1, z2, gamma2, beta2, residual, relu, bn1, bn2, groups=1, defer=False):
         G = int(groups)
         ctx.defer = bool(defer)
-
-        def affine(gamma, beta, bn):
-            if bn["training"]:
-                partials, count = bn["partials"], bn["count"]
-                if bn.get("sync"):
-                    if G > 1:
-                        raise StxError("BnActFn: SyncBatchNorm with groups is not wired (SyncBN runs the views separately)")
-                    partials, count = _sync_bn_partials(partials, count, *bn["sync"])
-                return bn_finalize(partials, count, gamma, beta, bn["running_mean"], bn["running_var"], bn["momentum"],
-                                   bn["eps"], G)
-            invstd = torch.rsqrt(bn["running_var"] + bn["eps"])
-            scale = gamma * invstd
-            res = (scale, beta - bn["running_mean"] * scale, bn["running_mean"].clone(), invstd)
-            return res if G == 1 else [t.unsqueeze(0).expand(G, -1).contiguous() for t in res]
-
         relu = int(relu)
         if relu == 2 and residual is not None:
             raise StxError("BnActFn: Mish with a plain residual is not wired (no model of the family uses it)")
         if G < 1 or z1.shape[0] % G:
             raise StxError(f"BnActFn: leading axis {z1.shape[0]} does not split into {G} groups")
-        sc1, sh1, m1, i1 = affine(gamma1, beta1, bn1)
+        sc1, sh1, m1, i1 = _bn_affine(gamma1, beta1, bn1, G)
         two = z2 is not None
         if two:
-            sc2, sh2, m2, i2 = affine(gamma2, beta2, bn2)
+            sc2, sh2, m2, i2 = _bn_affine(gamma2, beta2, bn2, G)
             y = bn_apply(z1, sc1, sh1, z2, sc2, sh2, relu, G)
         else:
             sc2 = sh2 = m2 = i2 = None
@@ -1214,52 +1313,34 @@
 
     @staticmethod
     def backward(ctx, gy):
-        z1, gamma1, m1, i1, z2, gamma2, m2, i2, y, sc1, sh1, sc2, sh2 = ctx.saved_tensors
-        gy = gy.contiguous()
-        G = ctx.groups
-        C = z1.shape[-1]
-        nvox = z1.numel() // C // G
-        lib = get_lib()
-        NB = lib.raw("stx_bn_reduce_blocks")()
-        part = _WS.get("bnred", G * NB * 3 * C, z1.device)
-        sums_all = torch.empty(G + (1 if G > 1 else 0), 3, C, dtype=torch.float32, device=z1.device)
-        sums = sums_all[:G]
-        _call("stx_bn_bwd_reduce2", _p(gy), _p(y), _p(z1), _p(m1), _p(i1), _p(z2) if ctx.two else None,
-              _p(m2) if ctx.two else None, _p(i2) if ctx.two else None, _p(sc1), _p(sh1), _p(sc2), _p(sh2), _p(part),
-              _p(sums_all), nvox, C, int(ctx.relu), G)
-        if not ctx.needs_input_grad[0] and not ctx.two and not ctx.has_res:
-            tot = sums_all[G] if G > 1 else sums_all[0]
-            return (None, tot[1], tot[0], None, None, None, None, None, None, None, None, None)
-        if (ctx.defer and not ctx.two and not ctx.has_res and ctx.relu in (0, 1) and ctx.train1 and not ctx.sync and G == 1
-                and (not ctx.relu or ctx.remask)):
-            alias = gy.view_as(gy)
-            pend = _PendingBn()
-            pend.g, pend.z, pend.scale, pend.shift, pend.mean, pend.invstd = alias, z1, sc1, sh1, m1, i1
-            pend.gamma, pend.sums, pend.inv_n, pend.act = gamma1, sums, 1.0 / nvox, int(ctx.relu)
-            if pend.scale is None:
-                pend.scale = pend.shift = m1
-            _defer_pending_bn(alias, pend)
-            tot = sums_all[0]
-            return (alias, tot[1], tot[0], None, None, None, None, None, None, None, None, None)
-        dz1 = torch.empty_like(z1)
-        dz2 = torch.empty_like(z2) if ctx.two else None
-        gres = torch.empty_like(z1) if (ctx.has_res and ctx.relu) else None
-        use = sums
-        if ctx.sync:
-            import torch.distributed as dist
-            use = sums.clone()
-            dist.all_reduce(use, group=ctx.sync[0])
-            use /= ctx.sync[1]
-        if not ctx.train1 or (ctx.two and not ctx.train2):
-            use = torch.zeros_like(sums)
-        _call("stx_bn_bwd_apply2", _p(gy), _p(y), _p(z1), _p(m1), _p(i1), _p(gamma1), _p(z2) if ctx.two else None,
-              _p(m2) if ctx.two else None, _p(i2) if ctx.two else None, _p(gamma2) if ctx.two else None, _p(sc1), _p(sh1),
-              _p(sc2), _p(sh2), _p(use), _p(dz1), _p(dz2), _p(gres), nvox, C, int(ctx.relu), G)
-        if ctx.has_res and not ctx.relu:
-            gres = gy
-        tot = sums_all[G] if G > 1 else sums_all[0]
-        return (dz1, tot[1], tot[0], dz2, tot[2] if ctx.two else None, tot[0].clone() if ctx.two else None, gres,
-                None, None, None, None, None)
+        return _bn_act_backward(ctx, ctx.saved_tensors, gy, ctx.needs_input_grad[0])
+
+
+class BnReluC1Fn(torch.autograd.Function):
+
+    @staticmethod
+    def forward(ctx, z, gamma, beta, w, add, bn, defer):
+        if not bn["training"]:
+            raise StxError("BnReluC1Fn: train-mode BatchNorm only (running statistics take the materialised path)")
+        sc, sh, m, i = _bn_affine(gamma, beta, bn)
+        cost = conv3d_c1_forward_bn(z, sc, sh, w.contiguous(), add)
+        ctx.relu, ctx.two, ctx.has_res, ctx.groups = 1, False, False, 1
+        ctx.train1, ctx.train2, ctx.sync, ctx.remask, ctx.defer = True, False, bn.get("sync"), True, bool(defer)
+        ctx.save_for_backward(z, gamma, m, i, sc, sh, w)
+        return cost
+
+    @staticmethod
+    def backward(ctx, gcost):
+        z, gamma, m, i, sc, sh, w = ctx.saved_tensors
+        gcost = gcost.contiguous()
+        gz = ggamma = gbeta = gw = None
+        if any(ctx.needs_input_grad[:3]):
+            gh = conv3d_c1_dgrad(gcost, w.contiguous(), z.shape[-1])
+            gz, ggamma, gbeta = _bn_act_backward(ctx, (z, gamma, m, i, None, None, None, None, None, sc, sh, None, None), gh,
+                                                 ctx.needs_input_grad[0])[:3]
+        if ctx.needs_input_grad[3]:
+            gw = conv3d_c1_wgrad_bn(z, sc, sh, gcost)
+        return gz, ggamma, gbeta, gw, (gcost if ctx.needs_input_grad[4] else None), None, None
 
 
 class MishFn(torch.autograd.Function):
```

Result: no change. 0.1786 pairs/s (-0.1%).
